# mryab/learning-at-home

Measured on NVIDIA H100. Metric: DMoE training samples/sec (whole job, device-timed, max over ranks), higher is better.
Workload: dtype bf16

## Files before the change

learning-at-home_b200/csrc/adam.cu:

```cuda
#include "sm90.cuh"

namespace lah {

struct AdamArgs {
    float* p; float* g; float* m; float* v; float* vmax; bf16* p_bf16;
    int num_segs; long long seg_start[13]; long long seg_n[12]; long long total;
    const int* step;
    const int* group_rows;
    int step_scalar;
    float lr, beta1, beta2, eps, weight_decay;
    int amsgrad, zero_mask;
    int world; long long peer_grad_off; char* peer_base[8]; float grad_scale;
    int G_active; const int* shadow_of; long long shadow_g_off; int me;
    int num_ranges; long long r_start[6]; long long r_cum[7];
    int dead_mask;
    const int* poison;
    float decay;
    const float* lr_dev;
};

template <bool DECOUPLED, bool DEV_LR>
__global__ void __launch_bounds__(256) adam_kernel(AdamArgs a) {
    if (a.poison && (*a.poison & 1)) return;
    float dev_lr = 0.f, dev_decay = 1.f;
    if constexpr (DEV_LR) {
        dev_lr = a.lr_dev[0];
        if constexpr (DECOUPLED) dev_decay = a.lr_dev[1];
    }
    const long long stride = static_cast<long long>(gridDim.x) * blockDim.x * 4;
    const long long span = a.num_ranges ? a.r_cum[a.num_ranges] : a.total;
    for (long long j = (static_cast<long long>(blockIdx.x) * blockDim.x + threadIdx.x) * 4; j < span; j += stride) {
        long long i = j;
        if (a.num_ranges) {
            int r = 0;
#pragma unroll
            for (int t = 1; t < 6; ++t)
                if (t < a.num_ranges && j >= a.r_cum[t]) r = t;
            i = a.r_start[r] + (j - a.r_cum[r]);
        }
        int sg = 0;
#pragma unroll
        for (int t = 1; t < 12; ++t)
            if (t < a.num_segs && i >= a.seg_start[t]) sg = t;
        const int g = static_cast<int>((i - a.seg_start[sg]) / a.seg_n[sg]);
        if (g >= a.G_active) continue;
        if (a.group_rows && a.group_rows[g] <= 0) continue;
        const int step = a.step ? a.step[g] : a.step_scalar;
        const float bc1 = 1.f - powf(a.beta1, static_cast<float>(step));
        const float bc2 = 1.f - powf(a.beta2, static_cast<float>(step));
        const float step_size = (DEV_LR ? dev_lr : a.lr) / bc1;
        const float inv_sqrt_bc2 = rsqrtf(bc2);
        float4 gr;
        if (a.peer_grad_off >= 0) {
            gr = make_float4(0.f, 0.f, 0.f, 0.f);
            for (int r = 0; r < a.world; ++r) {
                if ((a.dead_mask >> r) & 1) continue;
                const float4 t = *reinterpret_cast<const float4*>(
                    reinterpret_cast<const float*>(a.peer_base[r] + a.peer_grad_off) + i);
                gr.x += t.x; gr.y += t.y; gr.z += t.z; gr.w += t.w;
            }
            gr.x *= a.grad_scale; gr.y *= a.grad_scale; gr.z *= a.grad_scale; gr.w *= a.grad_scale;
        } else if (a.shadow_of && a.shadow_of[2 * g] >= 0) {
            const int slot = a.shadow_of[2 * g], mask = a.shadow_of[2 * g + 1];
            gr = ((mask >> a.me) & 1) ? *reinterpret_cast<const float4*>(a.g + i) : make_float4(0.f, 0.f, 0.f, 0.f);
            const long long pi = i + (a.G_active + slot - g) * a.seg_n[sg];
            for (int r = 0; r < a.world; ++r) {
                if (r == a.me || !((mask >> r) & 1)) continue;
                const float4 t = *reinterpret_cast<const float4*>(
                    reinterpret_cast<const float*>(a.peer_base[r] + a.shadow_g_off) + pi);
                gr.x += t.x; gr.y += t.y; gr.z += t.z; gr.w += t.w;
            }
        } else {
            gr = *reinterpret_cast<const float4*>(a.g + i);
        }
        float4 p = *reinterpret_cast<const float4*>(a.p + i);
        float4 m = *reinterpret_cast<const float4*>(a.m + i);
        float4 v = *reinterpret_cast<const float4*>(a.v + i);
        float4 vm = a.amsgrad ? *reinterpret_cast<const float4*>(a.vmax + i) : make_float4(0.f, 0.f, 0.f, 0.f);
        float* pp = &p.x; float* mp = &m.x; float* vp = &v.x; float* vmp = &vm.x; float* gp = &gr.x;
#pragma unroll
        for (int t = 0; t < 4; ++t) {
            float grad = gp[t];
            if constexpr (DECOUPLED) pp[t] = __fmul_rn(pp[t], DEV_LR ? dev_decay : a.decay);
            else if (a.weight_decay != 0.f) grad += a.weight_decay * pp[t];
            mp[t] = mp[t] + (1.f - a.beta1) * (grad - mp[t]);
            vp[t] = vp[t] * a.beta2 + (1.f - a.beta2) * grad * grad;
            float denom;
            if (a.amsgrad) {
                vmp[t] = fmaxf(vmp[t], vp[t]);
                denom = sqrtf(vmp[t]) * inv_sqrt_bc2 + a.eps;
            } else {
                denom = sqrtf(vp[t]) * inv_sqrt_bc2 + a.eps;
            }
            pp[t] -= step_size * (mp[t] / denom);
        }
        *reinterpret_cast<float4*>(a.p + i) = p;
        *reinterpret_cast<float4*>(a.m + i) = m;
        *reinterpret_cast<float4*>(a.v + i) = v;
        if (a.amsgrad) *reinterpret_cast<float4*>(a.vmax + i) = vm;
        if (a.p_bf16) {
            uint2 q;
            q.x = pack_bf16x2(p.x, p.y);
            q.y = pack_bf16x2(p.z, p.w);
            *reinterpret_cast<uint2*>(a.p_bf16 + i) = q;
        }
        if (((a.zero_mask >> sg) & 1) && a.peer_grad_off < 0)
            *reinterpret_cast<float4*>(a.g + i) = make_float4(0.f, 0.f, 0.f, 0.f);
    }
}

__global__ void bump_steps_kernel(int* step, const int* group_rows, int G) {
    const int g = blockIdx.x * blockDim.x + threadIdx.x;
    if (g < G && group_rows[g] > 0) step[g] += 1;
}

__global__ void cast_bf16_kernel(const float* __restrict__ src, bf16* __restrict__ dst, long long n) {
    const long long stride = static_cast<long long>(gridDim.x) * blockDim.x * 4;
    for (long long i = (static_cast<long long>(blockIdx.x) * blockDim.x + threadIdx.x) * 4; i < n; i += stride) {
        const float4 p = *reinterpret_cast<const float4*>(src + i);
        uint2 q;
        q.x = pack_bf16x2(p.x, p.y);
        q.y = pack_bf16x2(p.z, p.w);
        *reinterpret_cast<uint2*>(dst + i) = q;
    }
}

}

using namespace lah;

extern "C" const int* lah_get_poison_word();

extern "C" {

int lah_adam_step(float* p, float* g, float* m, float* v, float* vmax, void* p_bf16, int num_segs, const long long* seg_n,
                  int G, const int* step, const int* group_rows, int step_scalar, float lr, const float* lr_dev, float beta1,
                  float beta2, float eps, float weight_decay, int amsgrad, int zero_mask, int world, long long peer_grad_off,
                  const unsigned long long* peer_bases, float grad_scale, int G_active, const int* shadow_of,
                  long long shadow_g_off, int me, int seg_mask, int dead_mask, float decay, int decoupled, cudaStream_t st) {
    if (num_segs < 1 || num_segs > 12) return -2;
    if (decoupled && weight_decay != 0.f) return -2;
    AdamArgs a;
    a.num_segs = num_segs;
    long long off = 0;
    for (int s = 0; s < 12; ++s) {
        a.seg_start[s] = off;
        a.seg_n[s] = s < num_segs ? seg_n[s] : 1;
        if (s < num_segs) {
            if (seg_n[s] % 4) return -2;
            off += seg_n[s] * G;
        }
    }
    a.seg_start[12] = off;
    a.p = p; a.g = g; a.m = m; a.v = v; a.vmax = vmax; a.p_bf16 = (bf16*)p_bf16;
    a.total = off; a.step = step; a.group_rows = group_rows; a.step_scalar = step_scalar; a.lr = lr;
    a.beta1 = beta1; a.beta2 = beta2; a.eps = eps; a.weight_decay = weight_decay; a.amsgrad = amsgrad;
    a.zero_mask = zero_mask; a.world = world; a.peer_grad_off = peer_grad_off; a.grad_scale = grad_scale;
    a.G_active = G_active > 0 ? G_active : G; a.shadow_of = shadow_of; a.shadow_g_off = shadow_g_off; a.me = me;
    for (int i = 0; i < 8; ++i) a.peer_base[i] = (peer_bases && i < world) ? (char*)peer_bases[i] : nullptr;
    a.poison = lah_get_poison_word();
    a.dead_mask = dead_mask;
    a.decay = decay;
    a.lr_dev = lr_dev;
    a.num_ranges = 0;
    a.r_cum[0] = 0;
    if (seg_mask) {
        for (int s = 0; s < num_segs; ++s) {
            if (!((seg_mask >> s) & 1)) continue;
            const long long len = seg_n[s] * G;
            if (a.num_ranges && a.r_start[a.num_ranges - 1] + (a.r_cum[a.num_ranges] - a.r_cum[a.num_ranges - 1]) == a.seg_start[s]) {
                a.r_cum[a.num_ranges] += len;
            } else {
                if (a.num_ranges == 6) return -2;
                a.r_start[a.num_ranges] = a.seg_start[s];
                a.r_cum[a.num_ranges + 1] = a.r_cum[a.num_ranges] + len;
                ++a.num_ranges;
            }
        }
        if (!a.num_ranges) return 0;
    }
    const long long span = a.num_ranges ? a.r_cum[a.num_ranges] : a.total;
    if (span <= 0) return 0;
    long long blocks = (span / 4 + 255) / 256;
    if (blocks > 132 * 16) blocks = 132 * 16;
    if (lr_dev) {
        if (decoupled)
            adam_kernel<true, true><<<(int)blocks, 256, 0, st>>>(a);
        else
            adam_kernel<false, true><<<(int)blocks, 256, 0, st>>>(a);
    } else if (decoupled) {
        adam_kernel<true, false><<<(int)blocks, 256, 0, st>>>(a);
    } else {
        adam_kernel<false, false><<<(int)blocks, 256, 0, st>>>(a);
    }
    return -(int)cudaGetLastError();
}

int lah_bump_steps(int* step, const int* group_rows, int G, cudaStream_t st) {
    bump_steps_kernel<<<(G + 255) / 256, 256, 0, st>>>(step, group_rows, G);
    return -(int)cudaGetLastError();
}

int lah_cast_bf16(const float* src, void* dst, long long n, cudaStream_t st) {
    if (n % 4) return -2;
    if (n <= 0) return 0;
    long long blocks = (n / 4 + 255) / 256;
    if (blocks > 132 * 16) blocks = 132 * 16;
    cast_bf16_kernel<<<(int)blocks, 256, 0, st>>>(src, (bf16*)dst, n);
    return -(int)cudaGetLastError();
}

}
```

learning-at-home_b200/csrc/sm90.cuh:

```cuda
#pragma once

#include <cuda.h>
#include <cuda_runtime.h>
#include <cuda_bf16.h>
#include <stdint.h>

namespace lah {

typedef __nv_bfloat16 bf16;

__device__ __forceinline__ uint32_t smem_u32(const void* p) {
    return static_cast<uint32_t>(__cvta_generic_to_shared(p));
}

__device__ __forceinline__ uint32_t elect_one_sync() {
    uint32_t pred = 0;
    asm volatile(
        "{\n"
        ".reg .pred P1;\n"
        "elect.sync _|P1, 0xffffffff;\n"
        "selp.b32 %0, 1, 0, P1;\n"
        "}\n"
        : "=r"(pred));
    return pred;
}

__device__ __forceinline__ void mbar_init(uint64_t* bar, uint32_t count) {
    asm volatile("mbarrier.init.shared::cta.b64 [%0], %1;" ::"r"(smem_u32(bar)), "r"(count) : "memory");
}
__device__ __forceinline__ void fence_mbar_init() {
    asm volatile("fence.mbarrier_init.release.cluster;" ::: "memory");
}
__device__ __forceinline__ void fence_proxy_async_smem() {
    asm volatile("fence.proxy.async.shared::cta;" ::: "memory");
}
__device__ __forceinline__ void mbar_arrive_expect_tx(uint64_t* bar, uint32_t bytes) {
    asm volatile("mbarrier.arrive.expect_tx.shared::cta.b64 _, [%0], %1;" ::"r"(smem_u32(bar)), "r"(bytes)
                 : "memory");
}
__device__ __forceinline__ void mbar_arrive(uint64_t* bar) {
    asm volatile("mbarrier.arrive.shared::cta.b64 _, [%0];" ::"r"(smem_u32(bar)) : "memory");
}
__device__ __forceinline__ uint32_t mbar_try_wait(uint64_t* bar, uint32_t parity) {
    uint32_t ok;
    asm volatile(
        "{\n"
        ".reg .pred p;\n"
        "mbarrier.try_wait.parity.shared::cta.b64 p, [%1], %2;\n"
        "selp.b32 %0, 1, 0, p;\n"
        "}\n"
        : "=r"(ok)
        : "r"(smem_u32(bar)), "r"(parity)
        : "memory");
    return ok;
}
__device__ __forceinline__ void mbar_wait(uint64_t* bar, uint32_t parity) {
    while (!mbar_try_wait(bar, parity)) {
    }
}

__device__ __forceinline__ void tma_prefetch_desc(const CUtensorMap* tm) {
    asm volatile("prefetch.tensormap [%0];" ::"l"(reinterpret_cast<uint64_t>(tm)) : "memory");
}
__device__ __forceinline__ void tma_load_2d(void* smem_dst, const CUtensorMap* tm, uint64_t* bar, int c0, int c1) {
    asm volatile(
        "cp.async.bulk.tensor.2d.shared::cluster.global.mbarrier::complete_tx::bytes [%0], [%1, {%3, %4}], [%2];"
        ::"r"(smem_u32(smem_dst)), "l"(reinterpret_cast<uint64_t>(tm)), "r"(smem_u32(bar)), "r"(c0), "r"(c1)
        : "memory");
}
__device__ __forceinline__ void tma_load_3d(void* smem_dst, const CUtensorMap* tm, uint64_t* bar, int c0, int c1,
                                            int c2) {
    asm volatile(
        "cp.async.bulk.tensor.3d.shared::cluster.global.mbarrier::complete_tx::bytes [%0], [%1, {%3, %4, %5}], [%2];"
        ::"r"(smem_u32(smem_dst)), "l"(reinterpret_cast<uint64_t>(tm)), "r"(smem_u32(bar)), "r"(c0), "r"(c1), "r"(c2)
        : "memory");
}
__device__ __forceinline__ void tma_store_2d(const CUtensorMap* tm, const void* smem_src, int c0, int c1) {
    asm volatile("cp.async.bulk.tensor.2d.global.shared::cta.bulk_group [%0, {%2, %3}], [%1];" ::"l"(
                     reinterpret_cast<uint64_t>(tm)),
                 "r"(smem_u32(smem_src)), "r"(c0), "r"(c1)
                 : "memory");
}
__device__ __forceinline__ void tma_store_3d(const CUtensorMap* tm, const void* smem_src, int c0, int c1, int c2) {
    asm volatile("cp.async.bulk.tensor.3d.global.shared::cta.bulk_group [%0, {%2, %3, %4}], [%1];" ::"l"(
                     reinterpret_cast<uint64_t>(tm)),
                 "r"(smem_u32(smem_src)), "r"(c0), "r"(c1), "r"(c2)
                 : "memory");
}
__device__ __forceinline__ void tma_store_commit() { asm volatile("cp.async.bulk.commit_group;" ::: "memory"); }
template <int N>
__device__ __forceinline__ void tma_store_wait_read() {
    asm volatile("cp.async.bulk.wait_group.read %0;" ::"n"(N) : "memory");
}
template <int N>
__device__ __forceinline__ void tma_store_wait() {
    asm volatile("cp.async.bulk.wait_group %0;" ::"n"(N) : "memory");
}

__device__ __forceinline__ void wgmma_fence() { asm volatile("wgmma.fence.sync.aligned;" ::: "memory"); }
__device__ __forceinline__ void wgmma_commit() { asm volatile("wgmma.commit_group.sync.aligned;" ::: "memory"); }
template <int N>
__device__ __forceinline__ void wgmma_wait() {
    asm volatile("wgmma.wait_group.sync.aligned %0;" ::"n"(N) : "memory");
}
template <int R>
__device__ __forceinline__ void wgmma_fence_regs(float (&d)[R]) {
#pragma unroll
    for (int i = 0; i < R; ++i) asm volatile("" : "+f"(d[i])::"memory");
}

template <int TA, int TB>
__device__ __forceinline__ void wgmma_bf16_n16(float (&d)[8], uint64_t da, uint64_t db, uint32_t accumulate) {
    asm volatile(
        "{\n.reg .pred p;\nsetp.ne.b32 p, %10, 0;\n"
        "wgmma.mma_async.sync.aligned.m64n16k16.f32.bf16.bf16 {%0, %1, %2, %3, %4, %5, %6, %7}, %8, %9, p, 1, 1, %11, %12;\n}\n"
        : "+f"(d[0]), "+f"(d[1]), "+f"(d[2]), "+f"(d[3]), "+f"(d[4]), "+f"(d[5]), "+f"(d[6]), "+f"(d[7])
        : "l"(da), "l"(db), "r"(accumulate), "n"(TA), "n"(TB));
}

template <int TA, int TB>
__device__ __forceinline__ void wgmma_bf16_n32(float (&d)[16], uint64_t da, uint64_t db, uint32_t accumulate) {
    asm volatile(
        "{\n.reg .pred p;\nsetp.ne.b32 p, %18, 0;\n"
        "wgmma.mma_async.sync.aligned.m64n32k16.f32.bf16.bf16 {%0, %1, %2, %3, %4, %5, %6, %7, %8, %9, %10, %11, %12, %13, %14, %15}, %16, %17, p, 1, 1, %19, %20;\n}\n"
        : "+f"(d[0]), "+f"(d[1]), "+f"(d[2]), "+f"(d[3]), "+f"(d[4]), "+f"(d[5]), "+f"(d[6]), "+f"(d[7]), "+f"(d[8]), "+f"(d[9]), "+f"(d[10]), "+f"(d[11]), "+f"(d[12]), "+f"(d[13]), "+f"(d[14]), "+f"(d[15])
        : "l"(da), "l"(db), "r"(accumulate), "n"(TA), "n"(TB));
}

template <int TA, int TB>
__device__ __forceinline__ void wgmma_bf16_n64(float (&d)[32], uint64_t da, uint64_t db, uint32_t accumulate) {
    asm volatile(
        "{\n.reg .pred p;\nsetp.ne.b32 p, %34, 0;\n"
        "wgmma.mma_async.sync.aligned.m64n64k16.f32.bf16.bf16 {%0, %1, %2, %3, %4, %5, %6, %7, %8, %9, %10, %11, %12, %13, %14, %15, %16, %17, %18, %19, %20, %21, %22, %23, %24, %25, %26, %27, %28, %29, %30, %31}, %32, %33, p, 1, 1, %35, %36;\n}\n"
        : "+f"(d[0]), "+f"(d[1]), "+f"(d[2]), "+f"(d[3]), "+f"(d[4]), "+f"(d[5]), "+f"(d[6]), "+f"(d[7]), "+f"(d[8]), "+f"(d[9]), "+f"(d[10]), "+f"(d[11]), "+f"(d[12]), "+f"(d[13]), "+f"(d[14]), "+f"(d[15]), "+f"(d[16]), "+f"(d[17]), "+f"(d[18]), "+f"(d[19]), "+f"(d[20]), "+f"(d[21]), "+f"(d[22]), "+f"(d[23]), "+f"(d[24]), "+f"(d[25]), "+f"(d[26]), "+f"(d[27]), "+f"(d[28]), "+f"(d[29]), "+f"(d[30]), "+f"(d[31])
        : "l"(da), "l"(db), "r"(accumulate), "n"(TA), "n"(TB));
}

template <int TA, int TB>
__device__ __forceinline__ void wgmma_bf16_n128(float (&d)[64], uint64_t da, uint64_t db, uint32_t accumulate) {
    asm volatile(
        "{\n.reg .pred p;\nsetp.ne.b32 p, %66, 0;\n"
        "wgmma.mma_async.sync.aligned.m64n128k16.f32.bf16.bf16 {%0, %1, %2, %3, %4, %5, %6, %7, %8, %9, %10, %11, %12, %13, %14, %15, %16, %17, %18, %19, %20, %21, %22, %23, %24, %25, %26, %27, %28, %29, %30, %31, %32, %33, %34, %35, %36, %37, %38, %39, %40, %41, %42, %43, %44, %45, %46, %47, %48, %49, %50, %51, %52, %53, %54, %55, %56, %57, %58, %59, %60, %61, %62, %63}, %64, %65, p, 1, 1, %67, %68;\n}\n"
        : "+f"(d[0]), "+f"(d[1]), "+f"(d[2]), "+f"(d[3]), "+f"(d[4]), "+f"(d[5]), "+f"(d[6]), "+f"(d[7]), "+f"(d[8]), "+f"(d[9]), "+f"(d[10]), "+f"(d[11]), "+f"(d[12]), "+f"(d[13]), "+f"(d[14]), "+f"(d[15]), "+f"(d[16]), "+f"(d[17]), "+f"(d[18]), "+f"(d[19]), "+f"(d[20]), "+f"(d[21]), "+f"(d[22]), "+f"(d[23]), "+f"(d[24]), "+f"(d[25]), "+f"(d[26]), "+f"(d[27]), "+f"(d[28]), "+f"(d[29]), "+f"(d[30]), "+f"(d[31]), "+f"(d[32]), "+f"(d[33]), "+f"(d[34]), "+f"(d[35]), "+f"(d[36]), "+f"(d[37]), "+f"(d[38]), "+f"(d[39]), "+f"(d[40]), "+f"(d[41]), "+f"(d[42]), "+f"(d[43]), "+f"(d[44]), "+f"(d[45]), "+f"(d[46]), "+f"(d[47]), "+f"(d[48]), "+f"(d[49]), "+f"(d[50]), "+f"(d[51]), "+f"(d[52]), "+f"(d[53]), "+f"(d[54]), "+f"(d[55]), "+f"(d[56]), "+f"(d[57]), "+f"(d[58]), "+f"(d[59]), "+f"(d[60]), "+f"(d[61]), "+f"(d[62]), "+f"(d[63])
        : "l"(da), "l"(db), "r"(accumulate), "n"(TA), "n"(TB));
}

template <int TA, int TB>
__device__ __forceinline__ void wgmma_bf16_n256(float (&d)[128], uint64_t da, uint64_t db, uint32_t accumulate) {
    asm volatile(
        "{\n.reg .pred p;\nsetp.ne.b32 p, %130, 0;\n"
        "wgmma.mma_async.sync.aligned.m64n256k16.f32.bf16.bf16 {%0, %1, %2, %3, %4, %5, %6, %7, %8, %9, %10, %11, %12, %13, %14, %15, %16, %17, %18, %19, %20, %21, %22, %23, %24, %25, %26, %27, %28, %29, %30, %31, %32, %33, %34, %35, %36, %37, %38, %39, %40, %41, %42, %43, %44, %45, %46, %47, %48, %49, %50, %51, %52, %53, %54, %55, %56, %57, %58, %59, %60, %61, %62, %63, %64, %65, %66, %67, %68, %69, %70, %71, %72, %73, %74, %75, %76, %77, %78, %79, %80, %81, %82, %83, %84, %85, %86, %87, %88, %89, %90, %91, %92, %93, %94, %95, %96, %97, %98, %99, %100, %101, %102, %103, %104, %105, %106, %107, %108, %109, %110, %111, %112, %113, %114, %115, %116, %117, %118, %119, %120, %121, %122, %123, %124, %125, %126, %127}, %128, %129, p, 1, 1, %131, %132;\n}\n"
        : "+f"(d[0]), "+f"(d[1]), "+f"(d[2]), "+f"(d[3]), "+f"(d[4]), "+f"(d[5]), "+f"(d[6]), "+f"(d[7]), "+f"(d[8]), "+f"(d[9]), "+f"(d[10]), "+f"(d[11]), "+f"(d[12]), "+f"(d[13]), "+f"(d[14]), "+f"(d[15]), "+f"(d[16]), "+f"(d[17]), "+f"(d[18]), "+f"(d[19]), "+f"(d[20]), "+f"(d[21]), "+f"(d[22]), "+f"(d[23]), "+f"(d[24]), "+f"(d[25]), "+f"(d[26]), "+f"(d[27]), "+f"(d[28]), "+f"(d[29]), "+f"(d[30]), "+f"(d[31]), "+f"(d[32]), "+f"(d[33]), "+f"(d[34]), "+f"(d[35]), "+f"(d[36]), "+f"(d[37]), "+f"(d[38]), "+f"(d[39]), "+f"(d[40]), "+f"(d[41]), "+f"(d[42]), "+f"(d[43]), "+f"(d[44]), "+f"(d[45]), "+f"(d[46]), "+f"(d[47]), "+f"(d[48]), "+f"(d[49]), "+f"(d[50]), "+f"(d[51]), "+f"(d[52]), "+f"(d[53]), "+f"(d[54]), "+f"(d[55]), "+f"(d[56]), "+f"(d[57]), "+f"(d[58]), "+f"(d[59]), "+f"(d[60]), "+f"(d[61]), "+f"(d[62]), "+f"(d[63]), "+f"(d[64]), "+f"(d[65]), "+f"(d[66]), "+f"(d[67]), "+f"(d[68]), "+f"(d[69]), "+f"(d[70]), "+f"(d[71]), "+f"(d[72]), "+f"(d[73]), "+f"(d[74]), "+f"(d[75]), "+f"(d[76]), "+f"(d[77]), "+f"(d[78]), "+f"(d[79]), "+f"(d[80]), "+f"(d[81]), "+f"(d[82]), "+f"(d[83]), "+f"(d[84]), "+f"(d[85]), "+f"(d[86]), "+f"(d[87]), "+f"(d[88]), "+f"(d[89]), "+f"(d[90]), "+f"(d[91]), "+f"(d[92]), "+f"(d[93]), "+f"(d[94]), "+f"(d[95]), "+f"(d[96]), "+f"(d[97]), "+f"(d[98]), "+f"(d[99]), "+f"(d[100]), "+f"(d[101]), "+f"(d[102]), "+f"(d[103]), "+f"(d[104]), "+f"(d[105]), "+f"(d[106]), "+f"(d[107]), "+f"(d[108]), "+f"(d[109]), "+f"(d[110]), "+f"(d[111]), "+f"(d[112]), "+f"(d[113]), "+f"(d[114]), "+f"(d[115]), "+f"(d[116]), "+f"(d[117]), "+f"(d[118]), "+f"(d[119]), "+f"(d[120]), "+f"(d[121]), "+f"(d[122]), "+f"(d[123]), "+f"(d[124]), "+f"(d[125]), "+f"(d[126]), "+f"(d[127])
        : "l"(da), "l"(db), "r"(accumulate), "n"(TA), "n"(TB));
}

template <int TB>
__device__ __forceinline__ void wgmma_bf16_rs_n32(float (&d)[16], const uint32_t (&a)[4], uint64_t db, uint32_t accumulate) {
    asm volatile(
        "{\n.reg .pred p;\nsetp.ne.b32 p, %21, 0;\n"
        "wgmma.mma_async.sync.aligned.m64n32k16.f32.bf16.bf16 {%0, %1, %2, %3, %4, %5, %6, %7, %8, %9, %10, %11, %12, %13, %14, %15}, {%16, %17, %18, %19}, %20, p, 1, 1, %22;\n}\n"
        : "+f"(d[0]), "+f"(d[1]), "+f"(d[2]), "+f"(d[3]), "+f"(d[4]), "+f"(d[5]), "+f"(d[6]), "+f"(d[7]), "+f"(d[8]), "+f"(d[9]), "+f"(d[10]), "+f"(d[11]), "+f"(d[12]), "+f"(d[13]), "+f"(d[14]), "+f"(d[15])
        : "r"(a[0]), "r"(a[1]), "r"(a[2]), "r"(a[3]), "l"(db), "r"(accumulate), "n"(TB));
}

template <int TB>
__device__ __forceinline__ void wgmma_bf16_rs_n64(float (&d)[32], const uint32_t (&a)[4], uint64_t db, uint32_t accumulate) {
    asm volatile(
        "{\n.reg .pred p;\nsetp.ne.b32 p, %37, 0;\n"
        "wgmma.mma_async.sync.aligned.m64n64k16.f32.bf16.bf16 {%0, %1, %2, %3, %4, %5, %6, %7, %8, %9, %10, %11, %12, %13, %14, %15, %16, %17, %18, %19, %20, %21, %22, %23, %24, %25, %26, %27, %28, %29, %30, %31}, {%32, %33, %34, %35}, %36, p, 1, 1, %38;\n}\n"
        : "+f"(d[0]), "+f"(d[1]), "+f"(d[2]), "+f"(d[3]), "+f"(d[4]), "+f"(d[5]), "+f"(d[6]), "+f"(d[7]), "+f"(d[8]), "+f"(d[9]), "+f"(d[10]), "+f"(d[11]), "+f"(d[12]), "+f"(d[13]), "+f"(d[14]), "+f"(d[15]), "+f"(d[16]), "+f"(d[17]), "+f"(d[18]), "+f"(d[19]), "+f"(d[20]), "+f"(d[21]), "+f"(d[22]), "+f"(d[23]), "+f"(d[24]), "+f"(d[25]), "+f"(d[26]), "+f"(d[27]), "+f"(d[28]), "+f"(d[29]), "+f"(d[30]), "+f"(d[31])
        : "r"(a[0]), "r"(a[1]), "r"(a[2]), "r"(a[3]), "l"(db), "r"(accumulate), "n"(TB));
}

template <int TB>
__device__ __forceinline__ void wgmma_bf16_rs_n128(float (&d)[64], const uint32_t (&a)[4], uint64_t db, uint32_t accumulate) {
    asm volatile(
        "{\n.reg .pred p;\nsetp.ne.b32 p, %69, 0;\n"
        "wgmma.mma_async.sync.aligned.m64n128k16.f32.bf16.bf16 {%0, %1, %2, %3, %4, %5, %6, %7, %8, %9, %10, %11, %12, %13, %14, %15, %16, %17, %18, %19, %20, %21, %22, %23, %24, %25, %26, %27, %28, %29, %30, %31, %32, %33, %34, %35, %36, %37, %38, %39, %40, %41, %42, %43, %44, %45, %46, %47, %48, %49, %50, %51, %52, %53, %54, %55, %56, %57, %58, %59, %60, %61, %62, %63}, {%64, %65, %66, %67}, %68, p, 1, 1, %70;\n}\n"
        : "+f"(d[0]), "+f"(d[1]), "+f"(d[2]), "+f"(d[3]), "+f"(d[4]), "+f"(d[5]), "+f"(d[6]), "+f"(d[7]), "+f"(d[8]), "+f"(d[9]), "+f"(d[10]), "+f"(d[11]), "+f"(d[12]), "+f"(d[13]), "+f"(d[14]), "+f"(d[15]), "+f"(d[16]), "+f"(d[17]), "+f"(d[18]), "+f"(d[19]), "+f"(d[20]), "+f"(d[21]), "+f"(d[22]), "+f"(d[23]), "+f"(d[24]), "+f"(d[25]), "+f"(d[26]), "+f"(d[27]), "+f"(d[28]), "+f"(d[29]), "+f"(d[30]), "+f"(d[31]), "+f"(d[32]), "+f"(d[33]), "+f"(d[34]), "+f"(d[35]), "+f"(d[36]), "+f"(d[37]), "+f"(d[38]), "+f"(d[39]), "+f"(d[40]), "+f"(d[41]), "+f"(d[42]), "+f"(d[43]), "+f"(d[44]), "+f"(d[45]), "+f"(d[46]), "+f"(d[47]), "+f"(d[48]), "+f"(d[49]), "+f"(d[50]), "+f"(d[51]), "+f"(d[52]), "+f"(d[53]), "+f"(d[54]), "+f"(d[55]), "+f"(d[56]), "+f"(d[57]), "+f"(d[58]), "+f"(d[59]), "+f"(d[60]), "+f"(d[61]), "+f"(d[62]), "+f"(d[63])
        : "r"(a[0]), "r"(a[1]), "r"(a[2]), "r"(a[3]), "l"(db), "r"(accumulate), "n"(TB));
}

template <int N, int TA, int TB>
__device__ __forceinline__ void wgmma_bf16_ss(float (&d)[N / 2], uint64_t da, uint64_t db, uint32_t accumulate) {
    static_assert(N == 32 || N == 64 || N == 128, "N");
    if constexpr (N == 32) wgmma_bf16_n32<TA, TB>(d, da, db, accumulate);
    else if constexpr (N == 64) wgmma_bf16_n64<TA, TB>(d, da, db, accumulate);
    else wgmma_bf16_n128<TA, TB>(d, da, db, accumulate);
}
template <int N, int TB>
__device__ __forceinline__ void wgmma_bf16_rs(float (&d)[N / 2], const uint32_t (&a)[4], uint64_t db, uint32_t accumulate) {
    static_assert(N == 32 || N == 64 || N == 128, "N");
    if constexpr (N == 32) wgmma_bf16_rs_n32<TB>(d, a, db, accumulate);
    else if constexpr (N == 64) wgmma_bf16_rs_n64<TB>(d, a, db, accumulate);
    else wgmma_bf16_rs_n128<TB>(d, a, db, accumulate);
}

__device__ __forceinline__ uint64_t make_smem_desc_sw128(uint32_t saddr, uint32_t lbo_bytes, uint32_t sbo_bytes) {
    uint64_t d = 0;
    d |= static_cast<uint64_t>((saddr & 0x3FFFFu) >> 4);
    d |= static_cast<uint64_t>((lbo_bytes >> 4) & 0x3FFFu) << 16;
    d |= static_cast<uint64_t>((sbo_bytes >> 4) & 0x3FFFu) << 32;
    d |= static_cast<uint64_t>(1) << 62;
    return d;
}

__device__ __forceinline__ uint64_t make_smem_desc_sw64(uint32_t saddr, uint32_t lbo_bytes, uint32_t sbo_bytes) {
    uint64_t d = 0;
    d |= static_cast<uint64_t>((saddr & 0x3FFFFu) >> 4);
    d |= static_cast<uint64_t>((lbo_bytes >> 4) & 0x3FFFu) << 16;
    d |= static_cast<uint64_t>((sbo_bytes >> 4) & 0x3FFFu) << 32;
    d |= static_cast<uint64_t>(2) << 62;
    return d;
}

template <int COLS>
__device__ __forceinline__ uint64_t make_smem_desc_cols(uint32_t saddr, uint32_t lbo_bytes) {
    static_assert(COLS == 32 || COLS == 64, "atoms are 32 or 64 bf16 columns wide");
    if constexpr (COLS == 32) return make_smem_desc_sw64(saddr, lbo_bytes, 512);
    else return make_smem_desc_sw128(saddr, lbo_bytes, 1024);
}

__device__ __forceinline__ void named_bar_sync(int id, int threads) {
    asm volatile("bar.sync %0, %1;" ::"r"(id), "r"(threads) : "memory");
}

__device__ __forceinline__ void st_release_sys(int* p, int v) {
    asm volatile("st.release.sys.global.s32 [%0], %1;" ::"l"(p), "r"(v) : "memory");
}
__device__ __forceinline__ int ld_acquire_sys(const int* p) {
    int v;
    asm volatile("ld.acquire.sys.global.s32 %0, [%1];" : "=r"(v) : "l"(p) : "memory");
    return v;
}
__device__ __forceinline__ void red_add_release_sys(int* p, int v) {
    asm volatile("red.release.sys.global.add.s32 [%0], %1;" ::"l"(p), "r"(v) : "memory");
}
__device__ __forceinline__ int ld_acquire_gpu(const int* p) {
    int v;
    asm volatile("ld.acquire.gpu.global.s32 %0, [%1];" : "=r"(v) : "l"(p) : "memory");
    return v;
}
__device__ __forceinline__ int4 ld_nc_v4(const int4* p) {
    int4 r;
    asm volatile("ld.global.nc.L1::no_allocate.v4.s32 {%0, %1, %2, %3}, [%4];"
                 : "=r"(r.x), "=r"(r.y), "=r"(r.z), "=r"(r.w)
                 : "l"(p));
    return r;
}
__device__ __forceinline__ int4 ld_v4(const int4* p) {
    int4 r;
    asm volatile("ld.global.v4.s32 {%0, %1, %2, %3}, [%4];" : "=r"(r.x), "=r"(r.y), "=r"(r.z), "=r"(r.w) : "l"(p));
    return r;
}
__device__ __forceinline__ void st_v4(int4* p, const int4& v) {
    asm volatile("st.global.v4.s32 [%0], {%1, %2, %3, %4};" ::"l"(p), "r"(v.x), "r"(v.y), "r"(v.z), "r"(v.w)
                 : "memory");
}

__device__ __forceinline__ bool spin_flag_ge(const int* flag, int epoch) {
    const long long t0 = clock64();
    while (ld_acquire_sys(flag) < epoch) {
        if (clock64() - t0 > 20000000000ll) return false;
    }
    return true;
}
__device__ __forceinline__ bool spin_flag_ft(const int* flag, int epoch, int* status, int rank, int timeout_ms) {
    if (status) {
        const volatile int* vs = status;
        if ((vs[1] >> rank) & 1) return false;
        if (vs[0] & 1) return false;
    }
    const long long t0 = clock64();
    const long long limit = timeout_ms > 0 ? static_cast<long long>(timeout_ms) * 2000000ll : 20000000000ll;
    while (ld_acquire_sys(flag) < epoch) {
        if (clock64() - t0 > limit) {
            if (status) atomicOr(status, 1);
            return false;
        }
    }
    return true;
}
__device__ __forceinline__ unsigned long long globaltimer_ns() {
    unsigned long long t;
    asm volatile("mov.u64 %0, %%globaltimer;" : "=l"(t));
    return t;
}
__device__ __forceinline__ void fence_proxy_async_global() { asm volatile("fence.proxy.async.global;" ::: "memory"); }

__device__ __forceinline__ uint32_t pack_bf16x2(float lo, float hi) {
    __nv_bfloat162 v = __floats2bfloat162_rn(lo, hi);
    return *reinterpret_cast<uint32_t*>(&v);
}
__device__ __forceinline__ float2 unpack_bf16x2(uint32_t u) {
    __nv_bfloat162 v = *reinterpret_cast<__nv_bfloat162*>(&u);
    return __bfloat1622float2(v);
}
__device__ __forceinline__ float warp_sum(float v) {
#pragma unroll
    for (int o = 16; o > 0; o >>= 1) v += __shfl_xor_sync(0xffffffffu, v, o);
    return v;
}
__device__ __forceinline__ float warp_max(float v) {
#pragma unroll
    for (int o = 16; o > 0; o >>= 1) v = fmaxf(v, __shfl_xor_sync(0xffffffffu, v, o));
    return v;
}

inline int make_tmap(CUtensorMap* tm, CUtensorMapDataType dtype, int rank, const void* ptr, const uint64_t* dims,
                     const uint64_t* strides_bytes, const uint32_t* box,
                     CUtensorMapSwizzle swizzle = CU_TENSOR_MAP_SWIZZLE_128B) {
    typedef CUresult (*EncodeTiled)(CUtensorMap*, CUtensorMapDataType, cuuint32_t, void*, const cuuint64_t*,
                                    const cuuint64_t*, const cuuint32_t*, const cuuint32_t*, CUtensorMapInterleave,
                                    CUtensorMapSwizzle, CUtensorMapL2promotion, CUtensorMapFloatOOBfill);
    static const EncodeTiled encode = [] {
        void* fn = nullptr;
        cudaDriverEntryPointQueryResult qres;
        if (cudaGetDriverEntryPoint("cuTensorMapEncodeTiled", &fn, cudaEnableDefault, &qres) != cudaSuccess) fn = nullptr;
        return reinterpret_cast<EncodeTiled>(fn);
    }();
    if (!encode) return -100;
    cuuint64_t gdims[3], gstr[2];
    cuuint32_t gbox[3], estr[3] = {1, 1, 1};
    for (int i = 0; i < rank; ++i) {
        gdims[i] = dims[i];
        gbox[i] = box[i];
    }
    for (int i = 0; i < rank - 1; ++i) gstr[i] = strides_bytes[i];
    const CUresult r = encode(tm, dtype, rank, const_cast<void*>(ptr), gdims, gstr, gbox, estr, CU_TENSOR_MAP_INTERLEAVE_NONE,
                              swizzle, CU_TENSOR_MAP_L2_PROMOTION_L2_256B, CU_TENSOR_MAP_FLOAT_OOB_FILL_NONE);
    return r == CUDA_SUCCESS ? 0 : -1000 - static_cast<int>(r);
}

inline int num_sms() {
    static const int sms = [] {
        int dev = 0, n = 0;
        cudaGetDevice(&dev);
        cudaDeviceGetAttribute(&n, cudaDevAttrMultiProcessorCount, dev);
        return n;
    }();
    return sms;
}

inline int persistent_grid(long long total_tiles, int max_ctas) {
    int grid = num_sms();
    if (max_ctas > 0 && max_ctas < grid) grid = max_ctas;
    if (total_tiles < grid) grid = static_cast<int>(total_tiles);
    return grid;
}

template <auto Kernel>
inline int set_max_dynamic_smem(int bytes) {
    static bool done = false;
    if (!done) {
        const cudaError_t e = cudaFuncSetAttribute(Kernel, cudaFuncAttributeMaxDynamicSharedMemorySize, bytes);
        if (e != cudaSuccess) return -static_cast<int>(e);
        done = true;
    }
    return 0;
}

}
```

learning-at-home_b200/csrc/small_m.cu:

```cuda
#include "sm90.cuh"
#include <climits>

namespace lah {
namespace smallm {

constexpr int BM = 128;
constexpr int BK = 64;
constexpr int MMA_K = 16;
constexpr int BN_MAX = 128;
constexpr int NUM_THREADS = 288;

namespace sab {

constexpr int STAGES = 6;
constexpr int A_BYTES = BM * BK * 2;
constexpr int B_BYTES = BN_MAX * BK * 2;
constexpr int STAGE_BYTES = A_BYTES + B_BYTES;
constexpr int BAR_OFFSET = STAGES * STAGE_BYTES;
constexpr int QD = 4;
constexpr int MAX_G = 1023;
constexpr int CUM_OFFSET = BAR_OFFSET + (2 * STAGES + 2 * QD) * 8 + QD * 4 + 16;
constexpr int SMEM_TOTAL = CUM_OFFSET + (MAX_G + 1) * 4 + 1024;
static_assert(SMEM_TOTAL <= 232448, "shared memory budget");

struct Params {
    int G, M_out, K;
    const int* group_off;
    const int* group_rows;
    bf16* out;
    long long ldo;
    const float* bias;
    const bf16* residual;
    long long ldr;
    const int* wait_flags;
    int wait_count, wait_epoch;
    const int* epoch_base;
    int* status;
    int* tile_counter;
};

__device__ __forceinline__ int box_rows_of(int nn) { return nn <= 16 ? 16 : (nn <= 32 ? 32 : (nn <= 64 ? 64 : 128)); }

__device__ __forceinline__ int find_group(const int* cum, int G, int gc) {
    int lo = 0, hi = G - 1;
    while (lo < hi) {
        const int mid = (lo + hi + 1) >> 1;
        if (cum[mid] <= gc) lo = mid; else hi = mid - 1;
    }
    return lo;
}

template <int NB, bool A_MN>
__device__ __forceinline__ void sab_tile(const Params& p, uint8_t* smem, uint64_t* full_bar, uint64_t* empty_bar, int& stage,
                                         uint32_t& phase, int num_kb, int wg, int warp, int lane, int g, int ms, int row0,
                                         int nn) {
    float acc[NB / 2];
    constexpr uint32_t A_KSTEP = A_MN ? MMA_K * 128 : MMA_K * 2;
    int prev_stage = -1;
    for (int kb = 0; kb < num_kb; ++kb) {
        mbar_wait(&full_bar[stage], phase);
        const uint32_t sa = smem_u32(smem + stage * STAGE_BYTES) + wg * (A_MN ? BK * 128 : 64 * 128);
        const uint32_t sb = smem_u32(smem + stage * STAGE_BYTES + A_BYTES);
        wgmma_fence();
#pragma unroll
        for (int k = 0; k < BK / MMA_K; ++k) {
            const uint64_t da = make_smem_desc_sw128(sa + k * A_KSTEP, BK * 128, 1024);
            const uint64_t db = make_smem_desc_sw128(sb + k * (MMA_K * 2), 0, 1024);
            const uint32_t accum = (kb > 0 || k > 0) ? 1u : 0u;
            if constexpr (NB == 16) wgmma_bf16_n16<A_MN, 0>(acc, da, db, accum);
            if constexpr (NB == 32) wgmma_bf16_n32<A_MN, 0>(acc, da, db, accum);
            if constexpr (NB == 64) wgmma_bf16_n64<A_MN, 0>(acc, da, db, accum);
            if constexpr (NB == 128) wgmma_bf16_n128<A_MN, 0>(acc, da, db, accum);
        }
        wgmma_commit();
        wgmma_wait<1>();
        if (prev_stage >= 0) {
            __syncwarp();
            if (lane == 0) mbar_arrive(&empty_bar[prev_stage]);
        }
        prev_stage = stage;
        if (++stage == STAGES) {
            stage = 0;
            phase ^= 1;
        }
    }
    wgmma_wait<0>();
    wgmma_fence_regs(acc);
    __syncwarp();
    if (lane == 0 && prev_stage >= 0) mbar_arrive(&empty_bar[prev_stage]);

    const int n16 = (nn + 15) & ~15;
#pragma unroll
    for (int h = 0; h < 2; ++h) {
        const int feat = ms * BM + wg * 64 + (warp & 3) * 16 + (lane >> 2) + 8 * h;
        const float bias = p.bias ? __ldg(p.bias + static_cast<long long>(g) * p.M_out + feat) : 0.f;
#pragma unroll
        for (int j = 0; j < NB / 8; ++j) {
#pragma unroll
            for (int e = 0; e < 2; ++e) {
                const int n = 8 * j + 2 * (lane & 3) + e;
                if (n < n16) {
                    const long long row = row0 + n;
                    float v = acc[4 * j + 2 * h + e] + bias;
                    if (p.residual) v += __bfloat162float(p.residual[row * p.ldr + feat]);
                    p.out[row * p.ldo + feat] = __float2bfloat16(v);
                }
            }
        }
    }
}

template <bool A_MN>
__global__ void __launch_bounds__(NUM_THREADS, 1)
swapab_kernel(const Params p, const __grid_constant__ CUtensorMap tmA, const __grid_constant__ CUtensorMap tmB16,
              const __grid_constant__ CUtensorMap tmB32, const __grid_constant__ CUtensorMap tmB64,
              const __grid_constant__ CUtensorMap tmB128) {
    extern __shared__ uint8_t smem_raw[];
    uint8_t* smem = reinterpret_cast<uint8_t*>((reinterpret_cast<uintptr_t>(smem_raw) + 1023) & ~uintptr_t(1023));
    uint64_t* full_bar = reinterpret_cast<uint64_t*>(smem + BAR_OFFSET);
    uint64_t* empty_bar = full_bar + STAGES;
    uint64_t* q_full = empty_bar + STAGES;
    uint64_t* q_empty = q_full + QD;
    volatile int* q_tile = reinterpret_cast<volatile int*>(q_empty + QD);
    int* cum = reinterpret_cast<int*>(smem + CUM_OFFSET);

    const int warp = threadIdx.x >> 5;
    const int lane = threadIdx.x & 31;

    if (warp == 0) {
        int carry = 0;
        for (int base = 0; base < p.G; base += 32) {
            const int g = base + lane;
            int x = g < p.G ? (__ldg(p.group_rows + g) + BN_MAX - 1) / BN_MAX : 0;
#pragma unroll
            for (int d = 1; d < 32; d <<= 1) {
                const int y = __shfl_up_sync(0xffffffffu, x, d);
                if (lane >= d) x += y;
            }
            if (g < p.G) cum[g + 1] = carry + x;
            carry += __shfl_sync(0xffffffffu, x, 31);
        }
        if (lane == 0) cum[0] = 0;
    }
    if (warp == 8 && lane == 0) {
        tma_prefetch_desc(&tmA);
        tma_prefetch_desc(&tmB16);
        tma_prefetch_desc(&tmB32);
        tma_prefetch_desc(&tmB64);
        tma_prefetch_desc(&tmB128);
        for (int i = 0; i < STAGES; ++i) {
            mbar_init(&full_bar[i], 1);
            mbar_init(&empty_bar[i], 8);
        }
        for (int i = 0; i < QD; ++i) {
            mbar_init(&q_full[i], 1);
            mbar_init(&q_empty[i], 8);
        }
        fence_mbar_init();
    }
    __syncthreads();

    const int m_slices = p.M_out / BM;
    const int total = cum[p.G] * m_slices;
    const int num_kb = p.K / BK;

    if (warp == 8) {
        if (lane != 0) return;
        if (p.wait_flags) {
            const int epoch = p.wait_epoch + (p.epoch_base ? *p.epoch_base : 0);
            const unsigned long long t_wait = globaltimer_ns();
            for (int sidx = 0; sidx < p.wait_count; ++sidx)
                spin_flag_ft(p.wait_flags + sidx, epoch, p.status, sidx, p.epoch_base ? p.epoch_base[1] : 0);
            if (blockIdx.x == 0) atomicAdd(reinterpret_cast<unsigned long long*>(p.status + 2), globaltimer_ns() - t_wait);
            fence_proxy_async_global();
        }
        int stage = 0, qi = 0;
        uint32_t phase = 0, qphase = 0;
        while (true) {
            const int tile = atomicAdd(p.tile_counter, 1);
            mbar_wait(&q_empty[qi], qphase ^ 1);
            q_tile[qi] = tile;
            mbar_arrive(&q_full[qi]);
            if (++qi == QD) {
                qi = 0;
                qphase ^= 1;
            }
            if (tile >= total) break;
            const int gc = tile / m_slices, ms = tile - gc * m_slices;
            const int g = find_group(cum, p.G, gc);
            const int n0 = (gc - cum[g]) * BN_MAX;
            const int rows = __ldg(p.group_rows + g);
            const int off = __ldg(p.group_off + g);
            const int box = box_rows_of(min(rows - n0, BN_MAX));
            const CUtensorMap* tmB = box == 16 ? &tmB16 : (box == 32 ? &tmB32 : (box == 64 ? &tmB64 : &tmB128));
            for (int kb = 0; kb < num_kb; ++kb) {
                mbar_wait(&empty_bar[stage], phase ^ 1);
                uint8_t* sa = smem + stage * STAGE_BYTES;
                uint8_t* sb = sa + A_BYTES;
                const int k = kb * BK;
                mbar_arrive_expect_tx(&full_bar[stage], A_BYTES + box * 128);
                if (!A_MN) {
                    tma_load_3d(sa, &tmA, &full_bar[stage], k, ms * BM, g);
                } else {
#pragma unroll
                    for (int i = 0; i < BM / 64; ++i)
                        tma_load_3d(sa + i * (BK * 128), &tmA, &full_bar[stage], ms * BM + i * 64, k, g);
                }
                tma_load_2d(sb, tmB, &full_bar[stage], k, off + n0);
                if (++stage == STAGES) {
                    stage = 0;
                    phase ^= 1;
                }
            }
        }
        return;
    }

    const int wg = warp >> 2;
    int stage = 0, qi = 0;
    uint32_t phase = 0, qphase = 0;
    while (true) {
        mbar_wait(&q_full[qi], qphase);
        const int tile = q_tile[qi];
        __syncwarp();
        if (lane == 0) mbar_arrive(&q_empty[qi]);
        if (++qi == QD) {
            qi = 0;
            qphase ^= 1;
        }
        if (tile >= total) break;
        const int gc = tile / m_slices, ms = tile - gc * m_slices;
        const int g = find_group(cum, p.G, gc);
        const int n0 = (gc - cum[g]) * BN_MAX;
        const int nn = min(__ldg(p.group_rows + g) - n0, BN_MAX);
        const int row0 = __ldg(p.group_off + g) + n0;
        switch (box_rows_of(nn)) {
            case 16: sab_tile<16, A_MN>(p, smem, full_bar, empty_bar, stage, phase, num_kb, wg, warp, lane, g, ms, row0, nn); break;
            case 32: sab_tile<32, A_MN>(p, smem, full_bar, empty_bar, stage, phase, num_kb, wg, warp, lane, g, ms, row0, nn); break;
            case 64: sab_tile<64, A_MN>(p, smem, full_bar, empty_bar, stage, phase, num_kb, wg, warp, lane, g, ms, row0, nn); break;
            default: sab_tile<128, A_MN>(p, smem, full_bar, empty_bar, stage, phase, num_kb, wg, warp, lane, g, ms, row0, nn); break;
        }
    }
}

}

namespace wa {

constexpr int WBK = 32;
constexpr int OP_STAGES = 2;
constexpr int OP_STAGE_BYTES = 2 * (WBK * BM * 2);
constexpr int OP_BYTES = OP_STAGES * OP_STAGE_BYTES;
constexpr int BAND_ROWS = 4;
constexpr int CHUNKS = 16 / BAND_ROWS;
constexpr int SUB_COLS = 32;
constexpr int SUB_BYTES = BM / CHUNKS * SUB_COLS * 4;
constexpr int ARR_BYTES = (BN_MAX / SUB_COLS) * SUB_BYTES;
constexpr int ST_STAGES = 3;
constexpr int ST_STAGE_BYTES = 4 * ARR_BYTES;
constexpr int ST_OFFSET = OP_BYTES;
constexpr int BAR_OFFSET = ST_OFFSET + ST_STAGES * ST_STAGE_BYTES;
constexpr int QD = 4;
constexpr int SMEM_TOTAL = BAR_OFFSET + (2 * OP_STAGES + 2 * ST_STAGES + 2 * QD) * 8 + QD * 4 + 16 + 1024;
static_assert(ST_STAGES <= CHUNKS, "the producer issues a tile's first ST_STAGES chunks before its remaining k-blocks");
static_assert(OP_STAGE_BYTES % 1024 == 0 && SUB_BYTES % 1024 == 0, "128-B swizzle atoms need 1 KB alignment");
static_assert(SMEM_TOTAL <= 232448, "shared memory budget");

struct Params {
    int G, N, K;
    const int* group_off;
    const int* group_rows;
    const int* skip;
    const int* step;
    float* p;
    float* m;
    float* v;
    float* vmax;
    bf16* p_bf16;
    float lr, beta1, beta2, eps;
    int amsgrad;
    float wd;
    int* tile_counter;
    const int* poison;
};
static_assert(sizeof(Params) == 128 && sizeof(Params) % alignof(CUtensorMap) == 0, "Params layout");

constexpr int WD_NONE = 0, WD_L2 = 1, WD_DECOUPLED = 2;

struct Tile {
    int g, mt, nt;
};

struct StateMaps {
    CUtensorMap a[4];
};

__device__ __forceinline__ void state_chunk_tma(const StateMaps& tm, int n_arr, uint8_t* ss, uint64_t* bar, int col0, int srow,
                                                int c) {
    for (int a = 0; a < n_arr; ++a)
#pragma unroll
        for (int q = 0; q < BN_MAX / SUB_COLS; ++q) {
            uint8_t* s = ss + a * ARR_BYTES + q * SUB_BYTES;
            if (bar) tma_load_3d(s, &tm.a[a], bar, col0 + q * SUB_COLS, BAND_ROWS * c, srow / 16);
            else tma_store_3d(&tm.a[a], s, col0 + q * SUB_COLS, BAND_ROWS * c, srow / 16);
        }
}

template <int WD, bool DEV_LR>
__global__ void __launch_bounds__(NUM_THREADS, 1)
wgrad_adam_kernel(const Params p, const __grid_constant__ CUtensorMap tmDY, const __grid_constant__ CUtensorMap tmX,
                  const __grid_constant__ StateMaps tmS, const float* __restrict__ lr_dev) {
    extern __shared__ uint8_t smem_raw[];
    uint8_t* smem = reinterpret_cast<uint8_t*>((reinterpret_cast<uintptr_t>(smem_raw) + 1023) & ~uintptr_t(1023));
    uint8_t* st_smem = smem + ST_OFFSET;
    uint64_t* op_full = reinterpret_cast<uint64_t*>(smem + BAR_OFFSET);
    uint64_t* op_empty = op_full + OP_STAGES;
    uint64_t* st_full = op_empty + OP_STAGES;
    uint64_t* st_empty = st_full + ST_STAGES;
    uint64_t* q_full = st_empty + ST_STAGES;
    uint64_t* q_empty = q_full + QD;
    volatile int* q_tile = reinterpret_cast<volatile int*>(q_empty + QD);

    const int warp = threadIdx.x >> 5;
    const int lane = threadIdx.x & 31;
    if (p.poison && (*p.poison & 1)) return;
    const int n_arr = p.amsgrad ? 4 : 3;

    if (warp == 8 && lane == 0) {
        tma_prefetch_desc(&tmDY);
        tma_prefetch_desc(&tmX);
        for (int a = 0; a < n_arr; ++a) tma_prefetch_desc(&tmS.a[a]);
        for (int i = 0; i < OP_STAGES; ++i) {
            mbar_init(&op_full[i], 1);
            mbar_init(&op_empty[i], 8);
        }
        for (int i = 0; i < ST_STAGES; ++i) {
            mbar_init(&st_full[i], 1);
            mbar_init(&st_empty[i], 1);
        }
        for (int i = 0; i < QD; ++i) {
            mbar_init(&q_full[i], 1);
            mbar_init(&q_empty[i], 8);
        }
        fence_mbar_init();
    }
    __syncthreads();

    const int n_tiles = p.K / BN_MAX;
    const int tiles_per_group = (p.N / BM) * n_tiles;
    const int total = p.G * tiles_per_group;
    auto decode = [&](int tile) {
        Tile t;
        t.g = tile / tiles_per_group;
        const int r = tile - t.g * tiles_per_group;
        t.mt = r / n_tiles;
        t.nt = r - t.mt * n_tiles;
        return t;
    };

    if (warp == 8) {
        if (lane != 0) return;
        uint32_t phase = 0, qphase = 0, sphase = 0;
        int qi = 0, stage = 0, sstage = 0;
        while (true) {
            int tile;
            while (true) {
                tile = atomicAdd(p.tile_counter, 1);
                if (tile >= total) break;
                const int g = tile / tiles_per_group;
                if (__ldg(p.group_rows + g) > 0 && !(p.skip && __ldg(p.skip + 2 * g) >= 0)) break;
                atomicMax(p.tile_counter, (g + 1) * tiles_per_group);
            }
            mbar_wait(&q_empty[qi], qphase ^ 1);
            q_tile[qi] = tile;
            mbar_arrive(&q_full[qi]);
            if (++qi == QD) {
                qi = 0;
                qphase ^= 1;
            }
            if (tile >= total) break;
            const Tile t = decode(tile);
            const int off = __ldg(p.group_off + t.g), rows = __ldg(p.group_rows + t.g);
            const int srow = t.g * p.N + t.mt * BM;
            auto load_chunk = [&](int c) {
                mbar_wait(&st_empty[sstage], sphase ^ 1);
                mbar_arrive_expect_tx(&st_full[sstage], n_arr * ARR_BYTES);
                state_chunk_tma(tmS, n_arr, st_smem + sstage * ST_STAGE_BYTES, &st_full[sstage], t.nt * BN_MAX, srow, c);
                if (++sstage == ST_STAGES) {
                    sstage = 0;
                    sphase ^= 1;
                }
            };
            for (int t0 = 0; t0 < rows; t0 += WBK) {
                mbar_wait(&op_empty[stage], phase ^ 1);
                mbar_arrive_expect_tx(&op_full[stage], OP_STAGE_BYTES);
                uint8_t* sa = smem + stage * OP_STAGE_BYTES;
                uint8_t* sb = sa + WBK * BM * 2;
#pragma unroll
                for (int i = 0; i < BM / 64; ++i)
                    tma_load_2d(sa + i * (WBK * 128), &tmDY, &op_full[stage], t.mt * BM + i * 64, off + t0);
#pragma unroll
                for (int i = 0; i < BN_MAX / 64; ++i)
                    tma_load_2d(sb + i * (WBK * 128), &tmX, &op_full[stage], t.nt * BN_MAX + i * 64, off + t0);
                if (++stage == OP_STAGES) {
                    stage = 0;
                    phase ^= 1;
                }
                if (t0 == 0)
                    for (int c = 0; c < ST_STAGES; ++c) load_chunk(c);
            }
            for (int c = ST_STAGES; c < CHUNKS; ++c) load_chunk(c);
        }
        return;
    }

    float lr = p.lr, wd = p.wd;
    if constexpr (DEV_LR) {
        lr = lr_dev[0];
        if constexpr (WD == WD_DECOUPLED) wd = lr_dev[1];
    }
    const int wg = warp >> 2;
    int qi = 0, stage = 0, sstage = 0;
    uint32_t phase = 0, qphase = 0, sphase = 0;
    float acc[BN_MAX / 2];
    float xg[BN_MAX / 8];
    const int lrow = wg * 64 + (warp & 3) * 16 + (lane >> 2);
    const int brow = (lane >> 2) & 3;
    const int R = warp * BAND_ROWS + brow;
    const int jflip = 2 * (brow & 1);
    while (true) {
        mbar_wait(&q_full[qi], qphase);
        const int tile = q_tile[qi];
        __syncwarp();
        if (lane == 0) mbar_arrive(&q_empty[qi]);
        if (++qi == QD) {
            qi = 0;
            qphase ^= 1;
        }
        if (tile >= total) break;
        const Tile t = decode(tile);
        const int rows = __ldg(p.group_rows + t.g);
        int prev_stage = -1;
        for (int t0 = 0; t0 < rows; t0 += WBK) {
            mbar_wait(&op_full[stage], phase);
            const uint32_t sa = smem_u32(smem + stage * OP_STAGE_BYTES) + wg * (WBK * 128);
            const uint32_t sb = smem_u32(smem + stage * OP_STAGE_BYTES + WBK * BM * 2);
            const int ksteps = min(WBK / MMA_K, (rows - t0 + MMA_K - 1) / MMA_K);
            wgmma_fence();
            for (int k = 0; k < ksteps; ++k) {
                const uint64_t da = make_smem_desc_sw128(sa + k * (MMA_K * 128), WBK * 128, 1024);
                const uint64_t db = make_smem_desc_sw128(sb + k * (MMA_K * 128), WBK * 128, 1024);
                wgmma_bf16_n128<1, 1>(acc, da, db, (t0 > 0 || k > 0) ? 1u : 0u);
            }
            wgmma_commit();
            wgmma_wait<1>();
            if (prev_stage >= 0) {
                __syncwarp();
                if (lane == 0) mbar_arrive(&op_empty[prev_stage]);
            }
            prev_stage = stage;
            if (++stage == OP_STAGES) {
                stage = 0;
                phase ^= 1;
            }
        }
        wgmma_wait<0>();
        wgmma_fence_regs(acc);
        __syncwarp();
        if (lane == 0 && prev_stage >= 0) mbar_arrive(&op_empty[prev_stage]);

        const float st = static_cast<float>(__ldg(p.step + t.g));
        const float step_size = lr / (1.f - powf(p.beta1, st));
        const float inv_sqrt_bc2 = rsqrtf(1.f - powf(p.beta2, st));
        const int srow = t.g * p.N + t.mt * BM;
        const int col_base = t.nt * BN_MAX + 2 * (lane & 3);
#pragma unroll
        for (int c = 0; c < CHUNKS; ++c) {
            mbar_wait(&st_full[sstage], sphase);
            uint8_t* ss = st_smem + sstage * ST_STAGE_BYTES;
            if ((c & 1) == 0) {
#pragma unroll
                for (int i = 0; i < BN_MAX / 8; ++i) xg[i] = __shfl_xor_sync(0xffffffffu, acc[4 * (BN_MAX / 16 + i / 2) + i % 2], 16);
            }
            const bool own = (lane >> 4) == (c & 1);
            const long long o_row = (static_cast<long long>(srow) + (own ? lrow : lrow ^ 4) + 8 * (c >> 1)) * p.K + col_base;
            const int jbase = own ? 0 : BN_MAX / 16;
#pragma unroll
            for (int k = 0; k < BN_MAX / 16; ++k) {
                const int j = jbase + (k ^ jflip);
                const int so = (j >> 2) * SUB_BYTES + R * 128 + (((2 * (j & 3) + ((lane & 3) >> 1)) ^ (R & 7)) << 4) +
                               8 * (lane & 1);
                float2* sp = reinterpret_cast<float2*>(ss + so);
                float2* sm = reinterpret_cast<float2*>(ss + ARR_BYTES + so);
                float2* sv = reinterpret_cast<float2*>(ss + 2 * ARR_BYTES + so);
                float2* svm = reinterpret_cast<float2*>(ss + 3 * ARR_BYTES + so);
                float2 pw = *sp, m = *sm, v = *sv;
                float2 vm = p.amsgrad ? *svm : make_float2(0.f, 0.f);
                float* pp = &pw.x; float* mp = &m.x; float* vp = &v.x; float* vmp = &vm.x;
#pragma unroll
                for (int e = 0; e < 2; ++e) {
                    float grad = own ? (jflip ? acc[4 * (k ^ 2) + e] : acc[4 * k + e])
                                     : (jflip ? xg[2 * (k ^ 2) + e] : xg[2 * k + e]);
                    if constexpr (WD == WD_L2) grad += wd * pp[e];
                    if constexpr (WD == WD_DECOUPLED) pp[e] = __fmul_rn(pp[e], wd);
                    mp[e] = mp[e] + (1.f - p.beta1) * (grad - mp[e]);
                    vp[e] = vp[e] * p.beta2 + (1.f - p.beta2) * grad * grad;
                    float denom;
                    if (p.amsgrad) {
                        vmp[e] = fmaxf(vmp[e], vp[e]);
                        denom = sqrtf(vmp[e]) * inv_sqrt_bc2 + p.eps;
                    } else {
                        denom = sqrtf(vp[e]) * inv_sqrt_bc2 + p.eps;
                    }
                    pp[e] -= step_size * (mp[e] / denom);
                }
                *sp = pw;
                *sm = m;
                *sv = v;
                if (p.amsgrad) *svm = vm;
                *reinterpret_cast<uint32_t*>(p.p_bf16 + o_row + 8 * j) = pack_bf16x2(pw.x, pw.y);
            }
            fence_proxy_async_smem();
            named_bar_sync(1, 256);
            if (threadIdx.x == 0) {
                state_chunk_tma(tmS, n_arr, ss, nullptr, t.nt * BN_MAX, srow, c);
                tma_store_commit();
                tma_store_wait_read<0>();
                mbar_arrive(&st_empty[sstage]);
            }
            if (++sstage == ST_STAGES) {
                sstage = 0;
                sphase ^= 1;
            }
            if (c == 1) {
#pragma unroll
                for (int j = 0; j < BN_MAX / 8; ++j) {
                    acc[4 * j] = acc[4 * j + 2];
                    acc[4 * j + 1] = acc[4 * j + 3];
                }
            }
        }
    }
    if (threadIdx.x == 0) tma_store_wait<0>();
}

}
}
}

using namespace lah;
using namespace lah::smallm;

extern "C" const int* lah_get_epoch_base();

static int* tile_counter() {
    static int* ctr = nullptr;
    if (!ctr) {
        if (cudaMalloc(&ctr, 256) != cudaSuccess) return nullptr;
        cudaMemset(ctr, 0, 256);
    }
    return ctr;
}
static const int* g_poison = nullptr;

extern "C" {

int lah_set_poison_word(const int* status) {
    g_poison = status;
    return 0;
}
const int* lah_get_poison_word() { return g_poison; }

int lah_swapab_linear(const void* x, long long ldx, int x_rows, const void* W, int G, int M_out, int K, int a_mn,
                      void* out, long long ldo, const int* group_off, const int* group_rows, const float* bias,
                      const void* residual, long long ldr, const int* wait_flags, int wait_count, int wait_epoch,
                      int* status, int max_ctas, cudaStream_t st) {
    if ((K % BK) || (M_out % BM) || (ldx % 8) || G > sab::MAX_G) return -2;
    CUtensorMap tmA, tmB[4];
    if (!a_mn) {
        uint64_t dims[3] = {(uint64_t)K, (uint64_t)M_out, (uint64_t)G};
        uint64_t str[2] = {(uint64_t)K * 2, (uint64_t)M_out * K * 2};
        uint32_t box[3] = {BK, BM, 1};
        int r = make_tmap(&tmA, CU_TENSOR_MAP_DATA_TYPE_BFLOAT16, 3, W, dims, str, box);
        if (r) return r;
    } else {
        uint64_t dims[3] = {(uint64_t)M_out, (uint64_t)K, (uint64_t)G};
        uint64_t str[2] = {(uint64_t)M_out * 2, (uint64_t)M_out * K * 2};
        uint32_t box[3] = {64, BK, 1};
        int r = make_tmap(&tmA, CU_TENSOR_MAP_DATA_TYPE_BFLOAT16, 3, W, dims, str, box);
        if (r) return r;
    }
    const uint32_t boxes[4] = {16, 32, 64, 128};
    for (int i = 0; i < 4; ++i) {
        uint64_t dims[2] = {(uint64_t)K, (uint64_t)x_rows};
        uint64_t str[1] = {(uint64_t)ldx * 2};
        uint32_t box[2] = {BK, boxes[i]};
        int r = make_tmap(&tmB[i], CU_TENSOR_MAP_DATA_TYPE_BFLOAT16, 2, x, dims, str, box);
        if (r) return r;
    }
    sab::Params p;
    p.G = G; p.M_out = M_out; p.K = K; p.group_off = group_off; p.group_rows = group_rows; p.out = (bf16*)out; p.ldo = ldo;
    p.bias = bias; p.residual = (const bf16*)residual; p.ldr = ldr; p.wait_flags = wait_flags; p.wait_count = wait_count;
    p.wait_epoch = wait_epoch; p.epoch_base = lah_get_epoch_base(); p.status = status;
    p.tile_counter = tile_counter();
    if (!p.tile_counter) return -3;
    const long long total = 1ll * (M_out / BM) * (G + x_rows / BN_MAX);
    if (total <= 0 || G <= 0) return 0;
    if (cudaMemsetAsync(p.tile_counter, 0, sizeof(int), st) != cudaSuccess) return -4;
    const int ctas = persistent_grid(total, max_ctas);
    if (!a_mn) {
        if (int e = set_max_dynamic_smem<sab::swapab_kernel<false>>(sab::SMEM_TOTAL)) return e;
        sab::swapab_kernel<false><<<ctas, NUM_THREADS, sab::SMEM_TOTAL, st>>>(p, tmA, tmB[0], tmB[1], tmB[2], tmB[3]);
    } else {
        if (int e = set_max_dynamic_smem<sab::swapab_kernel<true>>(sab::SMEM_TOTAL)) return e;
        sab::swapab_kernel<true><<<ctas, NUM_THREADS, sab::SMEM_TOTAL, st>>>(p, tmA, tmB[0], tmB[1], tmB[2], tmB[3]);
    }
    return -(int)cudaGetLastError();
}

}

template <int WD, bool DEV_LR>
static int launch_wgrad_adam(const wa::Params& a, const CUtensorMap& tmDY, const CUtensorMap& tmX, const wa::StateMaps& tmS,
                             const float* lr_dev, int ctas, cudaStream_t st) {
    if (int e = set_max_dynamic_smem<wa::wgrad_adam_kernel<WD, DEV_LR>>(wa::SMEM_TOTAL)) return e;
    wa::wgrad_adam_kernel<WD, DEV_LR><<<ctas, NUM_THREADS, wa::SMEM_TOTAL, st>>>(a, tmDY, tmX, tmS, lr_dev);
    return -(int)cudaGetLastError();
}

extern "C" {

int lah_wgrad_adam(const void* dy, long long lddy, const void* x, long long ldx, int total_rows, int G, int N, int K,
                   const int* group_off, const int* group_rows, const int* skip, const int* step, float* p, float* m,
                   float* v, float* vmax, void* p_bf16, float lr, const float* lr_dev, float beta1, float beta2, float eps,
                   int amsgrad, float weight_decay, float decay, int decoupled, int max_ctas, cudaStream_t st) {
    if ((N % BM) || (K % BN_MAX) || (lddy % 8) || (ldx % 8) || 1ll * G * N > INT_MAX) return -2;
    if (decoupled && weight_decay != 0.f) return -2;
    if (amsgrad && !vmax) return -2;
    CUtensorMap tmDY, tmX;
    wa::StateMaps tmS;
    {
        float* arrs[4] = {p, m, v, amsgrad ? vmax : p};
        uint64_t dims[3] = {(uint64_t)K, 16, (uint64_t)G * N / 16};
        uint64_t str[2] = {(uint64_t)K * 4, (uint64_t)K * 64};
        uint32_t box[3] = {wa::SUB_COLS, wa::BAND_ROWS, BM / 16};
        for (int a = 0; a < 4; ++a) {
            int r = make_tmap(&tmS.a[a], CU_TENSOR_MAP_DATA_TYPE_FLOAT32, 3, arrs[a], dims, str, box);
            if (r) return r;
        }
    }
    {
        uint64_t dims[2] = {(uint64_t)N, (uint64_t)total_rows};
        uint64_t str[1] = {(uint64_t)lddy * 2};
        uint32_t box[2] = {64, wa::WBK};
        int r = make_tmap(&tmDY, CU_TENSOR_MAP_DATA_TYPE_BFLOAT16, 2, dy, dims, str, box);
        if (r) return r;
    }
    {
        uint64_t dims[2] = {(uint64_t)K, (uint64_t)total_rows};
        uint64_t str[1] = {(uint64_t)ldx * 2};
        uint32_t box[2] = {64, wa::WBK};
        int r = make_tmap(&tmX, CU_TENSOR_MAP_DATA_TYPE_BFLOAT16, 2, x, dims, str, box);
        if (r) return r;
    }
    wa::Params a;
    a.G = G; a.N = N; a.K = K; a.group_off = group_off; a.group_rows = group_rows; a.skip = skip; a.step = step;
    a.p = p; a.m = m; a.v = v; a.vmax = vmax; a.p_bf16 = (bf16*)p_bf16; a.lr = lr; a.beta1 = beta1; a.beta2 = beta2; a.eps = eps; a.amsgrad = amsgrad;
    a.wd = decoupled ? decay : weight_decay;
    a.tile_counter = tile_counter() ? tile_counter() + 16 : nullptr;
    a.poison = g_poison;
    if (!a.tile_counter) return -3;
    const long long total = 1ll * G * (N / BM) * (K / BN_MAX);
    if (total <= 0) return 0;
    if (cudaMemsetAsync(a.tile_counter, 0, sizeof(int), st) != cudaSuccess) return -4;
    const int ctas = persistent_grid(total, max_ctas);
    if (lr_dev) {
        if (decoupled) return launch_wgrad_adam<wa::WD_DECOUPLED, true>(a, tmDY, tmX, tmS, lr_dev, ctas, st);
        if (weight_decay != 0.f) return launch_wgrad_adam<wa::WD_L2, true>(a, tmDY, tmX, tmS, lr_dev, ctas, st);
        return launch_wgrad_adam<wa::WD_NONE, true>(a, tmDY, tmX, tmS, lr_dev, ctas, st);
    }
    if (decoupled) return launch_wgrad_adam<wa::WD_DECOUPLED, false>(a, tmDY, tmX, tmS, nullptr, ctas, st);
    if (weight_decay != 0.f) return launch_wgrad_adam<wa::WD_L2, false>(a, tmDY, tmX, tmS, nullptr, ctas, st);
    return launch_wgrad_adam<wa::WD_NONE, false>(a, tmDY, tmX, tmS, nullptr, ctas, st);
}

}
```

learning-at-home_b200/ops/kernels.py:

```python
import ctypes
import math

import torch
import torch.nn.functional as F

from . import native
from .native import c_void_p, c_int, c_ll, c_float, ptr, stream_ptr

c_ull = ctypes.c_ulonglong
_configured = False

SLOT_COUNTS, SLOT_DISPATCH, SLOT_OUTPUT, SLOT_GRAD, SLOT_DINPUT, SLOT_TRAINER, SLOT_BARRIER, SLOT_SHADOW = range(8)
NUM_SLOTS = 8
MAX_WORLD = 8
STATUS_TIMEOUT, STATUS_OVERFLOW = 1, 2


def _lib():
    global _configured
    lib = native.cuda_lib()
    if _configured:
        return lib
    P, I, L, Fl = c_void_p, c_int, c_ll, c_float
    sigs = {
        "lah_ln_relu_fwd": [P, P, P, P, P, P, P, I, I, I, I, P],
        "lah_ln_relu_bwd": [P, P, P, P, P, P, P, P, P, P, P, P, I, I, I, I, P, P],
        "lah_grouped_colsum": [P, L, P, P, I, P, I, I, P],
        "lah_set_step_counters": [P],
        "lah_set_multicast": [c_ull],
        "lah_set_poison_word": [P],
        "lah_nvls_allreduce": [L, L, Fl, P],
        "lah_heartbeat": [L, I, I, L, P],
        "lah_alive_from_heartbeats": [P, P, I, L, L, P],
        "lah_set_spin_timeout_ms": [I],
        "lah_step_begin": [I, L, P],
        "lah_swapab_linear": [P, L, I, P, I, I, I, I, P, L, P, P, P, P, L, P, I, I, P, I, P],
        "lah_wgrad_adam": [P, L, P, L, I, I, I, I, P, P, P, P, P, P, P, P, P, Fl, P, Fl, Fl, Fl, I, Fl, Fl, I, I, P],
        "lah_ln_relu_fwd_q": [P, P, P, P, P, P, P, I, I, I, P, P, P],
        "lah_set_peers": [P, I, I],
        "lah_set_wait_counter": [P],
        "lah_gate_topk": [P, I, P, I, I, P, Fl, c_ull, L, P, P, P, P, P],
        "lah_layout_exchange": [L, L, I, I, I, I, I, I, I, P, P, P, P, P, P, P, I, Fl, I, P, P, P, P, P],
        "lah_scatter_rows": [P, P, P, P, P, P, L, L, I, I, I, I, I, I, I, I, P, P, P, P, P, I, P],
        "lah_pull_shadow": [P, I, I, L, L, I, P, I, P],
        "lah_zero_slots": [P, I, P, I, I, I, I, P],
        "lah_signal_wait": [L, I, I, I, I, P, P],
        "lah_combine_rows": [L, P, P, P, P, I, I, I, I, L, I, I, I, I, P, P, P],
        "lah_gate_bwd": [L, P, P, P, P, P, I, I, I, I, P, I, P, P],
        "lah_router_loss_fwd": [P, I, P, I, P, P, I, P, P, P, P, P, P, P],
        "lah_router_loss_bwd": [P, I, P, I, P, P, P, P, Fl, Fl, P, P],
        "lah_adam_step": [P, P, P, P, P, P, I, P, I, P, P, I, Fl, P, Fl, Fl, Fl, Fl, I, I, I, L, P, Fl, I, P, L, I, I, I, Fl,
                          I, P],
        "lah_bump_steps": [P, P, I, P],
        "lah_cast_bf16": [P, P, L, P],
        "lah_attention_fwd": [P, P, P, L, I, I, I, c_ull, I, Fl, P, P],
        "lah_attention_bwd": [P, P, P, P, P, P, P, L, I, I, I, c_ull, I, Fl, P, P],
        "lah_attention_fwd_causal": [P, P, P, L, I, I, I, c_ull, I, Fl, P],
        "lah_attention_bwd_causal": [P, P, P, P, P, P, P, L, I, I, I, c_ull, I, Fl, P],
        "lah_pack_key_mask": [P, P, L, I, P],
        "lah_dropout_mask": [P, I, I, I, I, I, c_ull, I, P],
        "lah_dropout_ew": [I, P, P, P, L, I, c_ull, I, I, Fl, P],
        "lah_rms_norm_fwd": [P, P, P, P, I, I, Fl, P, I, P],
        "lah_rms_norm_bwd": [P, P, P, P, P, P, P, I, I, I, P, P, P],
        "lah_swiglu_fwd": [P, P, L, I, P],
        "lah_swiglu_bwd": [P, P, P, L, I, P],
        "lah_symm_alloc": [c_ull, ctypes.POINTER(c_void_p)],
        "lah_symm_free": [P],
        "lah_symm_get_handle": [P, ctypes.c_char_p],
        "lah_symm_open_handle": [ctypes.c_char_p, ctypes.POINTER(c_void_p)],
        "lah_symm_close_handle": [P],
        "lah_device_sync": [],
    }
    for name, argtypes in sigs.items():
        fn = getattr(lib, name)
        fn.restype = c_int
        fn.argtypes = argtypes
    _configured = True
    return lib


def _grid_array(grid_size):
    return (c_int * len(grid_size))(*[int(g) for g in grid_size])


def _check_ln_width(C, what, max_width=None):
    if max_width is None and not ln_width_ok(C):
        raise ValueError(f"{what}: width {C} is not a multiple of {LN_WIDTH_STEP} in [{LN_WIDTH_STEP}, {LN_MAX_WIDTH}]")
    if max_width is not None and (C <= 0 or C % LN_WIDTH_STEP):
        raise ValueError(f"{what}: width {C} is not a positive multiple of {LN_WIDTH_STEP}")


def ln_relu_fwd(h, gamma, beta, tile_group, *, out, mean, rstd, relu=True, quant=None, tile_rows=128):
    rows, C = h.shape
    _check_ln_width(C, "ln_relu_fwd")
    assert h.is_contiguous() and gamma.dtype == torch.float32 and (out is None or out.is_contiguous())
    if quant is not None:
        assert quant.K == C and quant.groups == 1 and quant.rows_per_group >= rows and quant.tile_rows == 128
        native.check(_lib().lah_ln_relu_fwd_q(ptr(h), ptr(out), ptr(mean), ptr(rstd), ptr(gamma), ptr(beta),
                                              ptr(tile_group), rows, C, int(relu), ptr(quant.q), ptr(quant.sf),
                                              stream_ptr()), "lah_ln_relu_fwd_q")
    else:
        native.check(_lib().lah_ln_relu_fwd(ptr(h), ptr(out), ptr(mean), ptr(rstd), ptr(gamma), ptr(beta),
                                            ptr(tile_group), rows, C, int(relu), int(tile_rows), stream_ptr()),
                     "lah_ln_relu_fwd")
    native.count_launch()
    return out


def ln_relu_bwd(da, h, mean, rstd, gamma, beta, tile_group, *, dh, dgamma, dbeta, dbias, relu=True, tile_rows=128,
                dres=None):
    rows, C = h.shape
    _check_ln_width(C, "ln_relu_bwd")
    assert da.is_contiguous() and h.is_contiguous() and dh.is_contiguous()
    assert dres is None or (dres.shape == h.shape and dres.dtype == torch.bfloat16 and dres.is_contiguous())
    part = torch.empty((rows + tile_rows - 1) // tile_rows, 3, C, device=h.device, dtype=torch.float32)
    native.check(_lib().lah_ln_relu_bwd(ptr(da), ptr(h), ptr(mean), ptr(rstd), ptr(gamma), ptr(beta), ptr(dh),
                                        ptr(dgamma), ptr(dbeta), ptr(dbias), ptr(part), ptr(tile_group), rows, C,
                                        int(relu), int(tile_rows), ptr(dres), stream_ptr()), "lah_ln_relu_bwd")
    native.count_launch(2)
    return dh


def _bf16_rows(t, what, shape):
    if t.dtype != torch.bfloat16 or not t.is_contiguous() or tuple(t.shape) != tuple(shape):
        raise ValueError(f"{what}: expected a contiguous bf16 tensor of shape {tuple(shape)}, got {t.dtype} "
                         f"{tuple(t.shape)}{'' if t.is_contiguous() else ' (not contiguous)'}")


def _f32_vec(t, what, n):
    if t.dtype != torch.float32 or not t.is_contiguous() or t.numel() != n:
        raise ValueError(f"{what}: expected a contiguous float32 tensor of {n} elements, got {t.dtype} {tuple(t.shape)}")


def _check_rms_groups(what, gamma, tile_group, tile_rows, rows, C):
    if tile_rows < 8 or tile_rows & (tile_rows - 1):
        raise ValueError(f"{what}: tile_rows must be a power of two >= 8, got {tile_rows}")
    if tile_group is None:
        return 1
    tiles = (rows + tile_rows - 1) // tile_rows
    if tile_group.dtype != torch.int32 or not tile_group.is_contiguous() or tile_group.numel() < tiles:
        raise ValueError(f"{what}: tile_group must be a contiguous int32 tensor of >= {tiles} entries, got "
                         f"{tile_group.dtype} {tuple(tile_group.shape)}")
    if gamma.numel() % C or gamma.numel() == 0:
        raise ValueError(f"{what}: grouped gamma must be [G, {C}], got {tuple(gamma.shape)}")
    return gamma.numel() // C


def rms_norm_fwd(x, gamma, eps, *, out, rstd, tile_group=None, tile_rows=16):
    if x.dim() != 2:
        raise ValueError(f"rms_norm_fwd: x must be [rows, C], got {tuple(x.shape)}")
    rows, C = x.shape
    _check_ln_width(C, "rms_norm_fwd")
    _bf16_rows(x, "rms_norm_fwd x", (rows, C))
    _bf16_rows(out, "rms_norm_fwd out", (rows, C))
    G = _check_rms_groups("rms_norm_fwd", gamma, tile_group, tile_rows, rows, C)
    _f32_vec(gamma, "rms_norm_fwd gamma", G * C)
    _f32_vec(rstd, "rms_norm_fwd rstd", rows)
    if not eps > 0:
        raise ValueError(f"rms_norm_fwd: eps must be > 0, got {eps}")
    native.check(_lib().lah_rms_norm_fwd(ptr(x), ptr(out), ptr(rstd), ptr(gamma), rows, C, float(eps), ptr(tile_group),
                                         int(tile_rows), stream_ptr()), "lah_rms_norm_fwd")
    native.count_launch()
    return out


def rms_norm_bwd(dn, x, rstd, gamma, *, dx, dgamma, dres=None, tile_rows=16, tile_group=None):
    if x.dim() != 2:
        raise ValueError(f"rms_norm_bwd: x must be [rows, C], got {tuple(x.shape)}")
    rows, C = x.shape
    _check_ln_width(C, "rms_norm_bwd")
    for t, what in ((dn, "dn"), (x, "x"), (dx, "dx")) + (((dres, "dres"),) if dres is not None else ()):
        _bf16_rows(t, f"rms_norm_bwd {what}", (rows, C))
    G = _check_rms_groups("rms_norm_bwd", gamma, tile_group, tile_rows, rows, C)
    _f32_vec(gamma, "rms_norm_bwd gamma", G * C)
    _f32_vec(dgamma, "rms_norm_bwd dgamma", G * C)
    _f32_vec(rstd, "rms_norm_bwd rstd", rows)
    part = torch.empty((rows + tile_rows - 1) // tile_rows, C, device=x.device, dtype=torch.float32)
    native.check(_lib().lah_rms_norm_bwd(ptr(dn), ptr(x), ptr(rstd), ptr(gamma), ptr(dx), ptr(dgamma), ptr(part), rows, C,
                                         int(tile_rows), ptr(dres), ptr(tile_group), stream_ptr()), "lah_rms_norm_bwd")
    native.count_launch(2)
    return dx


def _tile_rows_of(tile_group, tile_rows, rows):
    return tile_group.long().repeat_interleave(tile_rows)[:rows]


def rms_norm_grouped_fwd_ref(x, gamma, eps, tile_group, tile_rows):
    xf = x if x.dtype == torch.float64 else x.float()
    g = _tile_rows_of(tile_group.cpu(), tile_rows, x.shape[0]).to(x.device)
    live = (g >= 0)[:, None]
    gam = gamma.reshape(-1, x.shape[1]).to(xf.dtype)[g.clamp(min=0)]
    n, rstd = rms_norm_fwd_ref(xf, torch.ones(x.shape[1], dtype=xf.dtype, device=x.device), eps)
    return torch.where(live, n * gam, torch.zeros_like(n)), rstd


def rms_norm_grouped_bwd_ref(dn, x, gamma, eps, tile_group, tile_rows, dres=None):
    xf = x if x.dtype == torch.float64 else x.float()
    C = x.shape[1]
    gam = gamma.reshape(-1, C).to(xf.dtype)
    g = _tile_rows_of(tile_group.cpu(), tile_rows, x.shape[0]).to(x.device)
    live = g >= 0
    d = dn.to(xf.dtype) * live[:, None]
    gr = gam[g.clamp(min=0)]
    rstd = torch.rsqrt(xf.pow(2).mean(-1, keepdim=True) + eps)
    dx = rstd * (gr * d - xf * (gr * d * xf).mean(-1, keepdim=True) * rstd * rstd)
    if dres is not None:
        dx = dx + dres.to(xf.dtype)
    dx = dx * live[:, None]
    dgamma = torch.zeros_like(gam).index_add_(0, g[live], (d * xf * rstd)[live])
    return dx, dgamma


def rms_norm_fwd_ref(x, gamma, eps):
    xf = x if x.dtype == torch.float64 else x.float()
    rstd = torch.rsqrt(xf.pow(2).mean(-1) + eps)
    return xf * rstd[:, None] * gamma.to(xf.dtype), rstd


def rms_norm_bwd_ref(dn, x, gamma, eps, dres=None):
    xf = x if x.dtype == torch.float64 else x.float()
    d, g = dn.to(xf.dtype), gamma.to(xf.dtype)
    rstd = torch.rsqrt(xf.pow(2).mean(-1, keepdim=True) + eps)
    dx = rstd * (g * d - xf * (g * d * xf).mean(-1, keepdim=True) * rstd * rstd)
    if dres is not None:
        dx = dx + dres.to(xf.dtype)
    return dx, (d * xf * rstd).sum(0)


def grouped_colsum(x, tile_group, *, out, tile_rows=128):
    rows, C = x.shape
    _check_ln_width(C, "grouped_colsum", max_width=0)
    part = torch.empty((rows + tile_rows - 1) // tile_rows, C, device=x.device, dtype=torch.float32)
    native.check(_lib().lah_grouped_colsum(ptr(x), x.stride(0), ptr(out), ptr(part), C, ptr(tile_group), rows,
                                           int(tile_rows), stream_ptr()), "lah_grouped_colsum")
    native.count_launch(2)
    return out


def set_peers(bases, me):
    arr = (c_ull * len(bases))(*[int(b) for b in bases])
    native.check(_lib().lah_set_peers(ctypes.cast(arr, c_void_p), len(bases), me), "lah_set_peers")


def set_wait_counter(counter):
    native.check(_lib().lah_set_wait_counter(ptr(counter)), "lah_set_wait_counter")


def set_multicast(mc_base):
    native.check(_lib().lah_set_multicast(int(mc_base)), "lah_set_multicast")


def nvls_allreduce(off, n, scale=1.0):
    native.check(_lib().lah_nvls_allreduce(int(off), int(n), float(scale), stream_ptr()), "lah_nvls_allreduce")
    native.count_launch()


def heartbeat(hb_off, first, count, now_ms):
    native.check(_lib().lah_heartbeat(int(hb_off), int(first), int(count), int(now_ms), stream_ptr()), "lah_heartbeat")
    native.count_launch()


def alive_from_heartbeats(hb, alive, now_ms, max_age_ms):
    native.check(_lib().lah_alive_from_heartbeats(ptr(hb), ptr(alive), alive.numel(), int(now_ms), int(max_age_ms),
                                                  stream_ptr()), "lah_alive_from_heartbeats")
    native.count_launch()


def set_poison_word(status):
    native.check(_lib().lah_set_poison_word(ptr(status)), "lah_set_poison_word")


def set_step_counters(ctr):
    native.check(_lib().lah_set_step_counters(ptr(ctr)), "lah_set_step_counters")


def step_begin(epoch_delta, token_delta=0):
    native.check(_lib().lah_step_begin(int(epoch_delta), int(token_delta), stream_ptr()), "lah_step_begin")
    native.count_launch()


def set_spin_timeout_ms(ms):
    native.check(_lib().lah_set_spin_timeout_ms(int(ms)), "lah_set_spin_timeout_ms")


def gate_topk(logits, grid_size, k, *, alive=None, failure_rate=0.0, seed=0, token_offset=0, idx, w, pos, counts):
    B = logits.shape[0]
    assert logits.dtype == torch.float32 and logits.is_contiguous() and logits.shape[1] == sum(grid_size)
    native.check(_lib().lah_gate_topk(ptr(logits), B, ctypes.cast(_grid_array(grid_size), c_void_p), len(grid_size), k,
                                      ptr(alive), float(failure_rate), int(seed) & (2 ** 64 - 1), int(token_offset),
                                      ptr(idx), ptr(w), ptr(pos), ptr(counts), stream_ptr()), "lah_gate_topk")
    native.count_launch(2)


def layout_exchange(cnt_all_off, flags_off, slot, epoch, E, E_loc, max_rows, *, align=128, tile_rows=None, counts, dst_row, group_off, group_rows,
                    tile_group, total_rows, status, shadow_slots=0, shadow_tol=1.1, min_shadow_rows=512, route_owner=None,
                    step_rows=None, shadow_info=None, owned_shadow=None):
    native.check(_lib().lah_layout_exchange(cnt_all_off, flags_off, slot, epoch, E, E_loc, max_rows, align,
                                            int(tile_rows or min(align, 128)), ptr(counts),
                                            ptr(dst_row), ptr(group_off), ptr(group_rows), ptr(tile_group),
                                            ptr(total_rows), ptr(status), int(shadow_slots), float(shadow_tol),
                                            int(min_shadow_rows), ptr(route_owner), ptr(step_rows), ptr(shadow_info),
                                            ptr(owned_shadow), stream_ptr()), "lah_layout_exchange")
    native.count_launch()


def pull_shadow(shadow_info, shadow_slots, E_loc, p_off, pbf16_off, seg_sizes, small_mask):
    segs = (c_ll * len(seg_sizes))(*[int(s) for s in seg_sizes])
    native.check(_lib().lah_pull_shadow(ptr(shadow_info), int(shadow_slots), E_loc, p_off, pbf16_off, len(seg_sizes),
                                        ctypes.cast(segs, c_void_p), int(small_mask), stream_ptr()), "lah_pull_shadow")
    native.count_launch()


def zero_slots(g, seg_sizes, slots, first_slot, num_slots, seg_mask):
    segs = (c_ll * len(seg_sizes))(*[int(s) for s in seg_sizes])
    native.check(_lib().lah_zero_slots(ptr(g), len(seg_sizes), ctypes.cast(segs, c_void_p), slots, first_slot, num_slots,
                                       int(seg_mask), stream_ptr()), "lah_zero_slots")
    native.count_launch()


def scatter_rows(src, scale, idx, pos, dst_row, pair_row, dst_off, flags_off, slot, epoch, k, E_loc, max_rows,
                 group_off, group_rows, done_counter, status, align=128, route_owner=None, num_groups=0):
    num_pairs = idx.numel()
    H = src.shape[1]
    assert src.is_contiguous() and src.dtype == torch.bfloat16
    native.check(_lib().lah_scatter_rows(ptr(src), ptr(scale), ptr(idx), ptr(pos), ptr(dst_row), ptr(pair_row), dst_off,
                                         flags_off, slot, epoch, num_pairs, k, H, E_loc, max_rows, align, ptr(group_off),
                                         ptr(group_rows), ptr(done_counter), ptr(status), ptr(route_owner),
                                         int(num_groups), stream_ptr()),
                 "lah_scatter_rows")
    native.count_launch()


def signal_wait(flags_off, slot, epoch, status, *, signal=True, wait=True):
    native.check(_lib().lah_signal_wait(flags_off, slot, epoch, int(signal), int(wait), ptr(status), stream_ptr()),
                 "lah_signal_wait")
    native.count_launch()


def combine_rows(src_off, idx, pair_row, w, out, k, E_loc, *, flags_off=0, slot=0, epoch=0, signal=False, wait=False,
                 status=None, route_owner=None):
    B, H = out.shape
    native.check(_lib().lah_combine_rows(src_off, ptr(idx), ptr(pair_row), ptr(w), ptr(out), B, k, H, E_loc, flags_off,
                                         slot, epoch, int(signal), int(wait), ptr(status), ptr(route_owner),
                                         stream_ptr()),
                 "lah_combine_rows")
    native.count_launch()
    return out


def gate_bwd(yo_off, grad, idx, pair_row, w, dlogits, k, E_loc, grid_size, route_owner=None):
    B, H = grad.shape
    assert grad.is_contiguous() and grad.dtype == torch.bfloat16 and dlogits.dtype == torch.float32
    native.check(_lib().lah_gate_bwd(yo_off, ptr(grad), ptr(idx), ptr(pair_row), ptr(w), ptr(dlogits), B, k, H, E_loc,
                                     ctypes.cast(_grid_array(grid_size), c_void_p), len(grid_size), ptr(route_owner),
                                     stream_ptr()),
                 "lah_gate_bwd")
    native.count_launch()
    return dlogits


MAX_GRID_DIMS = 4
LAYOUT_MAX_E = 4096
ROUTER_WARPS = 4


def check_router_grid(grid_size):
    grid = tuple(int(g) for g in grid_size)
    if not 1 <= len(grid) <= MAX_GRID_DIMS or min(grid) < 1 or sum(grid) > LAYOUT_MAX_E or math.prod(grid) > LAYOUT_MAX_E:
        raise ValueError(f"router losses: grid_size must have 1..{MAX_GRID_DIMS} positive sizes with at most "
                         f"{LAYOUT_MAX_E} experts, got {grid_size}")
    return grid


def _router_args(what, logits, grid_size, alive):
    grid = check_router_grid(grid_size)
    if logits.dtype != torch.float32 or logits.dim() != 2 or logits.shape[1] != sum(grid) or not logits.is_contiguous():
        raise ValueError(f"{what}: logits must be a contiguous float32 [B, {sum(grid)}] tensor, got {logits.dtype} "
                         f"{tuple(logits.shape)}")
    E = math.prod(grid)
    if alive is not None and (alive.dtype != torch.uint8 or alive.numel() != E or not alive.is_contiguous()):
        raise ValueError(f"{what}: alive must be a contiguous uint8 tensor of {E} entries, got {alive.dtype} "
                         f"{tuple(alive.shape)}")
    return grid, logits.shape[0], E


def router_loss_fwd(logits, grid_size, counts, *, alive=None, f, z, Fb, loss, partials=None, ticket=None):
    grid, B, E = _router_args("router_loss_fwd", logits, grid_size, alive)
    if counts.dtype != torch.int32 or counts.dim() != 2 or counts.shape[1] != E or not counts.is_contiguous() \
            or not 1 <= counts.shape[0] <= MAX_WORLD:
        raise ValueError(f"router_loss_fwd: counts must be a contiguous int32 [R <= {MAX_WORLD}, {E}] tensor, got "
                         f"{counts.dtype} {tuple(counts.shape)}")
    nblk = (B + ROUTER_WARPS - 1) // ROUTER_WARPS
    if partials is None:
        partials = torch.empty(max(1, 2 * nblk), dtype=torch.float32, device=logits.device)
    if ticket is None:
        ticket = torch.zeros(1, dtype=torch.int32, device=logits.device)
    _f32_vec(f, "router_loss_fwd: f", E + 1)
    _f32_vec(loss, "router_loss_fwd: loss", 2)
    for t, name, n in ((z, "z", B), (Fb, "Fb", B), (partials, "partials", 2 * nblk)):
        if t.dtype != torch.float32 or not t.is_contiguous() or t.numel() < n:
            raise ValueError(f"router_loss_fwd: {name} must be a contiguous float32 tensor of >= {n} entries, got "
                             f"{t.dtype} {tuple(t.shape)}")
    if ticket.dtype != torch.int32 or ticket.numel() < 1:
        raise ValueError("router_loss_fwd: ticket must be an int32 tensor")
    native.check(_lib().lah_router_loss_fwd(ptr(logits), B, ctypes.cast(_grid_array(grid), c_void_p), len(grid),
                                            ptr(alive), ptr(counts), counts.shape[0], ptr(f), ptr(z), ptr(Fb), ptr(loss),
                                            ptr(partials), ptr(ticket), stream_ptr()), "lah_router_loss_fwd")
    native.count_launch(2 if B > 0 else 1)
    return loss


def router_loss_bwd(logits, grid_size, *, alive=None, f, z, Fb, aux_coef, z_coef, dlogits):
    grid, B, E = _router_args("router_loss_bwd", logits, grid_size, alive)
    _f32_vec(f, "router_loss_bwd: f", E + 1)
    for t, name in ((z, "z"), (Fb, "Fb")):
        if t.dtype != torch.float32 or not t.is_contiguous() or t.numel() < B:
            raise ValueError(f"router_loss_bwd: {name} must be a contiguous float32 tensor of >= {B} entries")
    if dlogits.dtype != torch.float32 or tuple(dlogits.shape) != tuple(logits.shape) or not dlogits.is_contiguous():
        raise ValueError(f"router_loss_bwd: dlogits must be a contiguous float32 {tuple(logits.shape)} tensor, got "
                         f"{dlogits.dtype} {tuple(dlogits.shape)}")
    if not (math.isfinite(aux_coef) and math.isfinite(z_coef)):
        raise ValueError("router_loss_bwd: the coefficients must be finite")
    native.check(_lib().lah_router_loss_bwd(ptr(logits), B, ctypes.cast(_grid_array(grid), c_void_p), len(grid),
                                            ptr(alive), ptr(f), ptr(z), ptr(Fb), float(aux_coef), float(z_coef),
                                            ptr(dlogits), stream_ptr()), "lah_router_loss_bwd")
    if B > 0:
        native.count_launch()
    return dlogits


MAX_SEQ = 65536
HEAD_DIMS = (32, 64, 128)
LN_WIDTH_STEP = 128
LN_MAX_WIDTH = 4096
LN_WIDTHS = tuple(range(LN_WIDTH_STEP, LN_MAX_WIDTH + 1, LN_WIDTH_STEP))


def ln_width_ok(C) -> bool:
    return 0 < C <= LN_MAX_WIDTH and C % LN_WIDTH_STEP == 0


def pack_key_mask(pad):
    assert pad.is_cuda and pad.dtype == torch.bool and pad.dim() == 2 and pad.is_contiguous(), (pad.dtype, tuple(pad.shape))
    batch, seq_len = pad.shape
    assert 1 <= seq_len <= MAX_SEQ, seq_len
    words = torch.empty(batch, (seq_len + 31) // 32, dtype=torch.int32, device=pad.device)
    native.check(_lib().lah_pack_key_mask(ptr(pad), ptr(words), batch, seq_len, stream_ptr()), "lah_pack_key_mask")
    native.count_launch()
    return words


def pack_key_mask_ref(pad):
    batch, seq_len = pad.shape
    n = (seq_len + 31) // 32
    valid = torch.zeros(batch, n * 32, dtype=torch.int64)
    valid[:, :seq_len] = (~pad.cpu()).long()
    bits = (valid.view(batch, n, 32) << torch.arange(32)).sum(-1)
    return torch.where(bits >= 2 ** 31, bits - 2 ** 32, bits).to(torch.int32)


def _check_key_mask(key_mask, tokens, seq_len, device, causal):
    assert not (causal and key_mask is not None), "causal attention takes no key padding mask"
    if key_mask is not None:
        assert key_mask.dtype == torch.int32 and key_mask.is_contiguous() and key_mask.device == device
        assert key_mask.shape == (tokens // seq_len, (seq_len + 31) // 32), (tuple(key_mask.shape), tokens, seq_len)


def attention_fwd(qkv, num_heads, *, out=None, lse=None, dropout=None, seq_len=512, key_mask=None, causal=False):
    tokens, three_d = qkv.shape
    d_model = three_d // 3
    assert 1 <= seq_len <= MAX_SEQ and tokens % seq_len == 0, (tokens, seq_len)
    assert qkv.is_cuda and qkv.dtype == torch.bfloat16 and qkv.is_contiguous()
    assert num_heads > 0 and d_model % num_heads == 0 and d_model // num_heads in HEAD_DIMS, (d_model, num_heads)
    if out is None:
        out = torch.empty(tokens, d_model, dtype=torch.bfloat16, device=qkv.device)
    assert out.dtype == torch.bfloat16 and out.is_contiguous() and out.shape == (tokens, d_model)
    if lse is not None:
        assert lse.dtype == torch.float32 and lse.is_contiguous() and lse.numel() == tokens * num_heads
    _check_key_mask(key_mask, tokens, seq_len, qkv.device, causal)
    seed, thr, rescale = _dropout_args(dropout)
    args = (ptr(qkv), ptr(out), ptr(lse), tokens, int(seq_len), num_heads, d_model, seed, thr, rescale, stream_ptr())
    if causal:
        native.check(_lib().lah_attention_fwd_causal(*args), "lah_attention_fwd_causal")
    else:
        native.check(_lib().lah_attention_fwd(*args, ptr(key_mask)), "lah_attention_fwd")
    native.count_launch()
    return out


def attention_bwd(qkv, out, dout, lse, num_heads, *, dropout=None, seq_len=512, dqkv=None, key_mask=None, causal=False):
    tokens, three_d = qkv.shape
    d_model = three_d // 3
    assert 1 <= seq_len <= MAX_SEQ and tokens % seq_len == 0, (tokens, seq_len)
    assert dout.dtype == torch.bfloat16 and dout.is_contiguous() and out.is_contiguous() and lse.dtype == torch.float32
    assert out.dtype == torch.bfloat16 and qkv.is_contiguous()
    assert num_heads > 0 and d_model % num_heads == 0 and d_model // num_heads in HEAD_DIMS, (d_model, num_heads)
    delta = torch.empty(tokens, num_heads, dtype=torch.float32, device=qkv.device)
    if dqkv is None:
        dqkv = torch.empty_like(qkv)
    assert dqkv.dtype == torch.bfloat16 and dqkv.is_contiguous() and dqkv.shape == qkv.shape
    blocks = (seq_len + 127) // 128
    dq_part = torch.empty(blocks, tokens, d_model, dtype=torch.bfloat16, device=qkv.device)
    _check_key_mask(key_mask, tokens, seq_len, qkv.device, causal)
    args = (ptr(qkv), ptr(out), ptr(dout), ptr(lse), ptr(delta), ptr(dqkv), ptr(dq_part), tokens, int(seq_len), num_heads,
            d_model, *_dropout_args(dropout), stream_ptr())
    if causal:
        native.check(_lib().lah_attention_bwd_causal(*args), "lah_attention_bwd_causal")
    else:
        native.check(_lib().lah_attention_bwd(*args, ptr(key_mask)), "lah_attention_bwd")
    native.count_launch(3)
    return dqkv


def attention_ref(qkv, num_heads, seq_len=512, key_mask=None, causal=False):
    tokens, three_d = qkv.shape
    d = three_d // 3
    x = qkv if qkv.dtype == torch.float64 else qkv.float()
    q, k, v = x.view(tokens // seq_len, seq_len, 3, num_heads, d // num_heads).unbind(2)
    q, k, v = (t.transpose(1, 2) for t in (q, k, v))
    s = q @ k.transpose(-1, -2) / (d // num_heads) ** 0.5
    if causal:
        s = s.masked_fill(torch.ones(seq_len, seq_len, dtype=torch.bool, device=s.device).triu(1), float("-inf"))
    if key_mask is None:
        att = torch.softmax(s, dim=-1) @ v
    else:
        s = s.masked_fill(key_mask.to(s.device).view(tokens // seq_len, 1, 1, seq_len), float("-inf"))
        att = torch.softmax(s, dim=-1).nan_to_num(0.0) @ v
    return att.transpose(1, 2).reshape(tokens, d)


SITE_ATTN, SITE_OUT_PROJ, SITE_FF, SITE_LINEAR2 = range(4)


def dropout_threshold(p):
    assert 0.0 <= p < 1.0, p
    return min(65535, int(math.floor(p * 65536 + 0.5)))


def _dropout_args(dropout):
    if dropout is None or dropout[0] == 0:
        return 0, -1, 1.0
    p, seed = dropout[0], dropout[1]
    return int(seed) & (2 ** 64 - 1), dropout_threshold(p), 1.0 / (1.0 - p)


def dropout_mask(shape, p, seed, site, device=None):
    if site == SITE_ATTN:
        batch, heads, rows, cols = shape
    else:
        (rows, cols), batch, heads = shape, 1, 1
    out = torch.empty(*shape, dtype=torch.uint8, device=device or "cuda")
    native.check(_lib().lah_dropout_mask(ptr(out), int(site), batch, heads, rows, cols, int(seed) & (2 ** 64 - 1),
                                         dropout_threshold(p), stream_ptr()), "lah_dropout_mask")
    native.count_launch()
    return out.bool()


def _dropout_ew(op, x, f, p, seed, site, out):
    assert x.dtype == torch.bfloat16 and x.is_contiguous() and x.dim() == 2 and 1 <= site <= 3
    assert f is None or (f.shape == x.shape and f.dtype == torch.bfloat16 and f.is_contiguous())
    out = torch.empty_like(x) if out is None else out
    assert out.shape == x.shape and out.is_contiguous()
    rows, cols = x.shape
    native.check(_lib().lah_dropout_ew(op, ptr(x), ptr(f), ptr(out), rows, cols, int(seed) & (2 ** 64 - 1), int(site),
                                       dropout_threshold(p), 1.0 / (1.0 - p), stream_ptr()), "lah_dropout_ew")
    native.count_launch()
    return out


def dropout_apply(x, p, seed, site, *, out=None):
    return _dropout_ew(0, x, None, p, seed, site, out)


def gelu_dropout(f, p, seed, site, *, out=None):
    return _dropout_ew(1, f, None, p, seed, site, out)


def gelu_dropout_bwd(dg, f, p, seed, site, *, out=None):
    return _dropout_ew(2, dg, f, p, seed, site, out)


def relu_dropout(f, p, seed, site, *, out=None):
    return _dropout_ew(3, f, None, p, seed, site, out)


def relu_dropout_bwd(dg, f, p, seed, site, *, out=None):
    return _dropout_ew(4, dg, f, p, seed, site, out)


def relu_dropout_ref(f, mask, p):
    return mask.float() * F.relu(f.float()) / (1 - p)


def relu_dropout_bwd_ref(dg, f, mask, p):
    return (f.float() > 0).float() * mask.float() * dg.float() / (1 - p)


def _check_swiglu(h, what):
    if h.dim() != 2 or h.shape[1] % 256:
        raise ValueError(f"{what}: h must be [rows, 2 * inner] with inner a multiple of 128, got {tuple(h.shape)}")
    rows, inner = h.shape[0], h.shape[1] // 2
    _bf16_rows(h, f"{what} h", (rows, 2 * inner))
    return rows, inner


def swiglu_fwd(h, *, out=None):
    rows, inner = _check_swiglu(h, "swiglu_fwd")
    out = torch.empty(rows, inner, dtype=torch.bfloat16, device=h.device) if out is None else out
    _bf16_rows(out, "swiglu_fwd out", (rows, inner))
    native.check(_lib().lah_swiglu_fwd(ptr(h), ptr(out), rows, inner, stream_ptr()), "lah_swiglu_fwd")
    native.count_launch()
    return out


def swiglu_bwd(da, h, *, out=None):
    rows, inner = _check_swiglu(h, "swiglu_bwd")
    _bf16_rows(da, "swiglu_bwd da", (rows, inner))
    out = torch.empty_like(h) if out is None else out
    _bf16_rows(out, "swiglu_bwd out", (rows, 2 * inner))
    native.check(_lib().lah_swiglu_bwd(ptr(da), ptr(h), ptr(out), rows, inner, stream_ptr()), "lah_swiglu_bwd")
    native.count_launch()
    return out


def swiglu_ref(h):
    hf = h if h.dtype == torch.float64 else h.float()
    g, u = hf.chunk(2, dim=-1)
    return F.silu(g) * u


def swiglu_bwd_ref(da, h):
    hf = h if h.dtype == torch.float64 else h.float()
    g, u = hf.chunk(2, dim=-1)
    d = da.to(hf.dtype)
    s = torch.sigmoid(g)
    return torch.cat([d * u * s * (1 + g * (1 - s)), d * g * s], dim=-1)


_PHILOX_M0, _PHILOX_M1, _PHILOX_W0, _PHILOX_W1 = 0xD2511F53, 0xCD9E8D57, 0x9E3779B9, 0xBB67AE85
_U32 = 0xFFFFFFFF


def _mulhilo32(a, m):
    t1, t2 = (a & 0xFFFF) * m, (a >> 16) * m
    return (t2 + (t1 >> 16)) >> 16, (((t2 & 0xFFFF) << 16) + t1) & _U32


def philox4x32_10_ref(ctr, key):
    c = [torch.as_tensor(w, dtype=torch.int64) for w in ctr]
    c = list(torch.broadcast_tensors(*c))
    k0, k1 = int(key[0]) & _U32, int(key[1]) & _U32
    for _ in range(10):
        hi0, lo0 = _mulhilo32(c[0], _PHILOX_M0)
        hi1, lo1 = _mulhilo32(c[2], _PHILOX_M1)
        c = [hi1 ^ c[1] ^ k0, lo1, hi0 ^ c[3] ^ k1, lo0]
        k0, k1 = (k0 + _PHILOX_W0) & _U32, (k1 + _PHILOX_W1) & _U32
    return c


def dropout_counter_ref(site, *index):
    idx = torch.broadcast_tensors(*[torch.as_tensor(t, dtype=torch.int64) for t in index])
    zero = torch.zeros_like(idx[0])
    if site == SITE_ATTN:
        b, h, q, k = idx
        gq, gk = (q >> 4) * 4 + ((q >> 1) & 3), (k >> 4) * 4 + ((k >> 1) & 3)
        ctr = ((((gq & 127) * 128) + (gk & 127)) | ((q & 1) << 14), h, b, ((gq >> 7) << 8) | ((gk >> 7) << 20) | SITE_ATTN)
        lane = ((q >> 3) & 1) * 4 + ((k & 1) | (((k >> 3) & 1) << 1))
    else:
        r, n = idx
        gr, gn = (r >> 4) * 8 + (r & 7), (n >> 4) * 4 + ((n >> 1) & 3)
        ctr = (gn, gr, zero, zero + site)
        lane = ((r >> 3) & 1) * 4 + ((n & 1) | (((n >> 3) & 1) << 1))
    return ctr, lane


def dropout_keep_ref(p, seed, site, *index):
    ctr, lane = dropout_counter_ref(site, *index)
    seed = int(seed) & (2 ** 64 - 1)
    words = torch.stack(philox4x32_10_ref(ctr, (seed & _U32, seed >> 32)), dim=-1)
    w = words.gather(-1, (lane >> 1).unsqueeze(-1)).squeeze(-1)
    u16 = torch.where((lane & 1) == 1, w >> 16, w & 0xFFFF)
    return u16 >= dropout_threshold(p)


def dropout_mask_ref(shape, p, seed, site):
    grids = [torch.arange(n).view(*([1] * i), n, *([1] * (len(shape) - i - 1))) for i, n in enumerate(shape)]
    return dropout_keep_ref(p, seed, site, *grids)


def weight_decay_args(lr, weight_decay, decoupled):
    if decoupled:
        return 0.0, 1.0 - float(lr) * float(weight_decay)
    return float(weight_decay), 1.0


def lr_block_values(lr, weight_decay, decoupled):
    return float(lr), weight_decay_args(lr, weight_decay, decoupled)[1]


def _check_lr_dev(lr_dev):
    assert (lr_dev.is_cuda and lr_dev.dtype == torch.float32 and lr_dev.numel() == 2 and lr_dev.is_contiguous()), \
        "lr_dev: a contiguous float32 CUDA tensor [lr, decay] (lr_block_values)"


def segment_views(flat, shapes, slots=1):
    views, off = {}, 0
    for name, shape in shapes.items():
        n = slots * math.prod(shape)
        views[name] = flat[off: off + n].view(slots, *shape)
        off += n
    assert off == flat.numel(), (off, flat.numel())
    return views


def adam_step(p, g, m, v, vmax, p_bf16, seg_sizes, G, *, step=None, group_rows=None, step_scalar=0, lr=1e-3,
              betas=(0.9, 0.999), eps=1e-8, weight_decay=0.0, decoupled=False, amsgrad=True, zero_mask=0, world=1,
              peer_grad_off=-1, peer_bases=None, grad_scale=1.0, G_active=0, shadow_of=None, shadow_g_off=-1, me=0,
              seg_mask=0, dead_mask=0, lr_dev=None):
    arr = None
    if peer_bases is not None:
        arr = (c_ull * len(peer_bases))(*[int(b) for b in peer_bases])
    if isinstance(seg_sizes, int):
        seg_sizes = [seg_sizes]
    segs = (c_ll * len(seg_sizes))(*[int(s) for s in seg_sizes])
    if lr_dev is not None:
        _check_lr_dev(lr_dev)
    l2, decay = weight_decay_args(lr, weight_decay, decoupled)
    native.check(_lib().lah_adam_step(ptr(p), ptr(g), ptr(m), ptr(v), ptr(vmax), ptr(p_bf16), len(seg_sizes),
                                      ctypes.cast(segs, c_void_p), G, ptr(step), ptr(group_rows), int(step_scalar), lr,
                                      ptr(lr_dev), betas[0], betas[1], eps, l2, int(amsgrad), int(zero_mask), world,
                                      peer_grad_off, ctypes.cast(arr, c_void_p) if arr is not None else c_void_p(0),
                                      grad_scale, int(G_active), ptr(shadow_of), int(shadow_g_off), int(me), int(seg_mask),
                                      int(dead_mask), decay, int(bool(decoupled and weight_decay)), stream_ptr()),
                 "lah_adam_step")
    native.count_launch()


def swapab_linear(x, w, group_off, group_rows, *, out, bias=None, residual=None, w_is_kn=False, wait=None, max_ctas=0):
    assert x.dtype == torch.bfloat16 and w.dtype == torch.bfloat16 and out.dtype == torch.bfloat16 and w.is_contiguous()
    rows, K = x.shape
    G = w.shape[0]
    M_out = w.shape[2] if w_is_kn else w.shape[1]
    assert (w.shape[1] if w_is_kn else w.shape[2]) == K and x.stride(1) == 1 and out.stride(1) == 1
    wait_flags, wait_count, wait_epoch, wait_status = (wait[0], wait[0].numel(), wait[1], wait[2]) if wait else (None, 0, 0, None)
    native.check(_lib().lah_swapab_linear(ptr(x), x.stride(0), rows, ptr(w), G, M_out, K, int(w_is_kn), ptr(out),
                                          out.stride(0), ptr(group_off), ptr(group_rows), ptr(bias), ptr(residual),
                                          residual.stride(0) if residual is not None else 0, ptr(wait_flags), wait_count,
                                          wait_epoch, ptr(wait_status), int(max_ctas), stream_ptr()),
                 "lah_swapab_linear")
    native.count_launch()
    return out


def swapab_linear_ref(x, w, group_off, group_rows, *, bias=None, residual=None, w_is_kn=False):
    off, rows = group_off.tolist(), group_rows.tolist()
    M_out = w.shape[2] if w_is_kn else w.shape[1]
    out = torch.zeros(x.shape[0], M_out, dtype=torch.float32, device=x.device)
    for g, (o, r) in enumerate(zip(off, rows)):
        if r <= 0:
            continue
        wg = w[g].float()
        y = x[o:o + r].float() @ (wg if w_is_kn else wg.t())
        if bias is not None:
            y = y + bias.view(w.shape[0], M_out)[g]
        if residual is not None:
            y = y + residual[o:o + r].float()
        out[o:o + r] = y
    return out


def wgrad_adam(dy, x, group_off, group_rows, *, p, m, v, vmax, p_bf16, step, skip=None, lr=1e-3, betas=(0.9, 0.999),
               eps=1e-8, amsgrad=True, weight_decay=0.0, decoupled=False, max_ctas=0, lr_dev=None):
    G, N, Kd = p.shape
    assert dy.shape[1] == N and x.shape[1] == Kd and dy.shape[0] == x.shape[0] and p.is_contiguous()
    assert dy.dtype == torch.bfloat16 and x.dtype == torch.bfloat16 and p.dtype == torch.float32
    if amsgrad and vmax is None:
        raise ValueError("wgrad_adam: amsgrad needs a vmax tensor (vmax=None only with amsgrad=False)")
    if lr_dev is not None:
        _check_lr_dev(lr_dev)
    l2, decay = weight_decay_args(lr, weight_decay, decoupled)
    native.check(_lib().lah_wgrad_adam(ptr(dy), dy.stride(0), ptr(x), x.stride(0), dy.shape[0], G, N, Kd, ptr(group_off),
                                       ptr(group_rows), ptr(skip), ptr(step), ptr(p), ptr(m), ptr(v), ptr(vmax), ptr(p_bf16),
                                       lr, ptr(lr_dev), betas[0], betas[1], eps, int(amsgrad), l2, decay,
                                       int(bool(decoupled and weight_decay)), int(max_ctas), stream_ptr()),
                 "lah_wgrad_adam")
    native.count_launch()


def bump_steps(step, group_rows):
    native.check(_lib().lah_bump_steps(ptr(step), ptr(group_rows), step.numel(), stream_ptr()), "lah_bump_steps")
    native.count_launch()


def cast_bf16(src, dst):
    assert src.dtype == torch.float32 and dst.dtype == torch.bfloat16 and src.numel() == dst.numel()
    native.check(_lib().lah_cast_bf16(ptr(src), ptr(dst), src.numel(), stream_ptr()), "lah_cast_bf16")
    native.count_launch()


def product_key_scores(logits, grid_size):
    parts = torch.split(logits, list(grid_size), dim=-1)
    scores = parts[0]
    for part in parts[1:]:
        scores = (scores.unsqueeze(-1) + part.unsqueeze(-2)).flatten(-2)
    return scores


def gate_topk_ref(logits, grid_size, k, alive=None, fail_mask=None):
    scores = product_key_scores(logits.float(), grid_size)
    dead = torch.zeros_like(scores, dtype=torch.bool)
    if alive is not None:
        dead |= ~alive.bool().view(1, -1)
    if fail_mask is not None:
        dead |= fail_mask
    scores = scores.masked_fill(dead, float("-inf"))
    if scores.shape[-1] < k:
        scores = F.pad(scores, (0, k - scores.shape[-1]), value=float("-inf"))
    top_v, top_i = torch.sort(scores, dim=-1, descending=True, stable=True)
    top_v, top_i = top_v[..., :k], top_i[..., :k]
    valid = torch.isfinite(top_v)
    w = torch.softmax(top_v.masked_fill(~valid, float("-inf")), dim=-1)
    w = torch.where(valid, w, torch.zeros_like(w)).nan_to_num(0.0)
    return torch.where(valid, top_i, torch.full_like(top_i, -1)), w


def router_loss_ref(logits, grid_size, counts, alive=None):
    scores = product_key_scores(logits, grid_size)
    B, E = scores.shape
    live = torch.ones(E, dtype=torch.bool, device=scores.device) if alive is None else alive.bool().reshape(-1).to(scores.device)
    c = counts.reshape(-1, E).sum(0).to(scores.dtype).to(scores.device)
    f = (c / c.sum() if float(c.sum()) > 0 else torch.zeros_like(c)).detach()
    N = int(live.sum())
    masked = scores.masked_fill(~live.view(1, -1), float("-inf"))
    ok = torch.isfinite(masked).any(-1, keepdim=True)
    masked = torch.where(ok, masked, torch.zeros_like(masked))
    if N == 0 or B == 0:
        zero = scores.sum() * 0
        return zero, zero
    z = torch.logsumexp(masked, -1, keepdim=True)
    p = torch.where(live.view(1, -1) & ok, torch.exp(masked - z), torch.zeros_like(masked))
    z = torch.where(ok, z, torch.zeros_like(z)).squeeze(-1)
    return N * (p * f).sum() / B, (z * z).sum() / B


_SPLITMIX_GAMMA = 0x9E3779B97F4A7C15


def splitmix64_ref(x):
    import numpy as np
    x = np.array(x, dtype=np.uint64, ndmin=1) + np.uint64(_SPLITMIX_GAMMA)
    x = (x ^ (x >> np.uint64(30))) * np.uint64(0xBF58476D1CE4E5B9)
    x = (x ^ (x >> np.uint64(27))) * np.uint64(0x94D049BB133111EB)
    return x ^ (x >> np.uint64(31))


def gate_fail_mask_ref(B, E, rate, seed, token_offset):
    import numpy as np
    mask64 = 2 ** 64 - 1
    tok = (np.arange(B, dtype=np.uint64) + np.uint64(int(token_offset) & mask64)) * np.uint64(0x100000001B3)
    key = np.uint64(int(seed) & mask64) ^ (tok[:, None] + np.arange(E, dtype=np.uint64)[None, :])
    u = (splitmix64_ref(key) >> np.uint64(40)).astype(np.float64) / 2.0 ** 24
    return torch.from_numpy(u < float(np.float32(rate)))


def ln_relu_ref(h, gamma, beta, relu=True):
    y = F.layer_norm(h.float(), (h.shape[-1],), gamma.float(), beta.float(), 1e-5)
    return F.relu(y) if relu else y


def ln_relu_bwd_ref(da, h, gamma, beta, relu=True, dres=None):
    hf = h.float()
    mu = hf.mean(-1, keepdim=True)
    rstd = torch.rsqrt(hf.var(-1, unbiased=False, keepdim=True) + 1e-5)
    xhat = (hf - mu) * rstd
    g = da.float()
    if relu:
        g = g * (xhat * gamma.float() + beta.float() > 0)
    dxh = g * gamma.float()
    dh = rstd * (dxh - dxh.mean(-1, keepdim=True) - xhat * (dxh * xhat).mean(-1, keepdim=True))
    if dres is not None:
        dh = dh + dres.float()
    return dh, (g * xhat).sum(0), g.sum(0), dh.sum(0)


@torch.no_grad()
def adam_step_ref(p, g, m, v, vmax, seg_sizes, G, *, step, group_rows=None, lr=1e-3, betas=(0.9, 0.999), eps=1e-8,
                  amsgrad=True, zero_mask=0, weight_decay=0.0, decoupled=False):
    if isinstance(seg_sizes, int):
        seg_sizes = [seg_sizes]
    off = 0
    active = torch.ones(G, dtype=torch.bool, device=p.device) if group_rows is None else (group_rows > 0)
    idx = active.nonzero().squeeze(1)
    stepf = step.to(torch.float32).clamp(min=1)[idx]
    bc1 = (1 - betas[0] ** stepf).view(-1, 1)
    bc2 = (1 - betas[1] ** stepf).view(-1, 1)
    for s, size in enumerate(seg_sizes):
        sl = slice(off, off + size * G)
        off += size * G
        if idx.numel() == 0:
            continue
        P, Gr, M, V = p[sl].view(G, size), g[sl].view(G, size), m[sl].view(G, size), v[sl].view(G, size)
        grad = Gr[idx]
        if weight_decay and decoupled:
            P[idx] = P[idx] * (1 - lr * weight_decay)
        elif weight_decay:
            grad = grad + weight_decay * P[idx]
        m_new = M[idx] + (1 - betas[0]) * (grad - M[idx])
        v_new = V[idx] * betas[1] + (1 - betas[1]) * grad * grad
        if amsgrad:
            VM = vmax[sl].view(G, size)
            vm_new = torch.maximum(VM[idx], v_new)
            denom = vm_new.sqrt() / bc2.sqrt() + eps
            VM[idx] = vm_new
        else:
            denom = v_new.sqrt() / bc2.sqrt() + eps
        P[idx] = P[idx] - (lr / bc1) * (m_new / denom)
        M[idx] = m_new
        V[idx] = v_new
        if (zero_mask >> s) & 1:
            Gr[idx] = 0.0
```

learning-at-home_b200/parallel/engine.py:

```python
import math
from dataclasses import dataclass, field
from typing import Dict, List, Optional, Sequence, Tuple

import torch
import torch.nn as nn
import torch.nn.functional as F

from ..models.layers import FFN_SEG_KEYS as REF_KEYS, FFN_SEG_NAMES as SEG_NAMES, FFN_SMALL_SEG_MASK as SMALL_SEG_MASK
from ..models.layers import EXPERT_LAYOUTS, gated_inner_dim
from ..ops import fp8, gemm, kernels as K, native

GATED_EPS = 1e-6


@dataclass
class DMoEConfig:
    hidden: int = 512
    grid_size: Tuple[int, ...] = (8, 8)
    k: int = 4
    num_layers: int = 4
    in_features: int = 784
    num_classes: int = 10
    tokens_per_rank: int = 1024
    capacity_factor: float = 2.0
    failure_rate: float = 0.0
    lr: float = 1e-3
    betas: Tuple[float, float] = (0.9, 0.999)
    eps: float = 1e-8
    amsgrad: bool = True
    weight_decay: float = 0.0
    decoupled_weight_decay: bool = False
    seed: int = 1337
    uid_prefix: str = "expert"
    gate_mode: str = "product_key"
    shadow_experts: int = 8
    shadow_tol: float = 1.1
    shadow_min_rows: int = 1024
    expert_dtype: str = "bf16"
    expert_path: str = "auto"
    optimizer_ctas: int = -1
    update_every_inputs: int = 0
    update_every_steps: int = 0
    trainer_staleness: int = 0
    trainer_microbatches: int = 1
    peer_timeout_ms: int = 0
    expert: str = "ffn"
    inner_dim: int = 0
    router_aux_loss_coef: float = 0.0
    router_z_loss_coef: float = 0.0

    def __post_init__(self):
        if self.expert not in EXPERT_LAYOUTS:
            raise ValueError(f"DMoEConfig.expert must be one of {sorted(EXPERT_LAYOUTS)}, got {self.expert!r}")
        if self.expert == "ffn" and self.inner_dim:
            raise ValueError("DMoEConfig.inner_dim: FeedforwardBlock experts are 4 * hidden wide; inner_dim is for "
                             "expert='swiglu' only")
        if self.inner_dim < 0:
            raise ValueError(f"DMoEConfig.inner_dim must be >= 0, got {self.inner_dim}")
        if self.expert == "swiglu" and self.expert_dtype != "bf16":
            raise ValueError("expert='swiglu' runs bf16 expert GEMMs only (its RMSNorm and SwiGLU kernels do not emit "
                             f"MXFP8 operands); got expert_dtype={self.expert_dtype!r}")
        for name in ("router_aux_loss_coef", "router_z_loss_coef"):
            v = float(getattr(self, name))
            if not math.isfinite(v) or v < 0.0:
                raise ValueError(f"DMoEConfig.{name} must be a finite value >= 0, got {v}")
            if v > 0.0 and self.gate_mode == "emulator":
                raise ValueError(f"DMoEConfig.{name}: the emulator gate is frozen (not trained), so a router loss would "
                                 "train nothing; use gate_mode='product_key'")

    @property
    def router_losses(self) -> bool:
        return self.router_aux_loss_coef > 0.0 or self.router_z_loss_coef > 0.0

    def check_native_sizes(self):
        if self.expert == "swiglu" and (self.hidden % 128 or not 128 <= self.hidden <= K.LN_MAX_WIDTH or self.inner % 128):
            raise ValueError(f"expert='swiglu' on the GPU needs hidden a multiple of 128 in [128, {K.LN_MAX_WIDTH}] and "
                             f"an inner width that is a multiple of 128; got hidden={self.hidden}, inner={self.inner}")

    @property
    def layout(self):
        return EXPERT_LAYOUTS[self.expert]

    def gemm_widths(self) -> Tuple[int, ...]:
        H, I = self.hidden, self.inner
        return (2 * I, H, I) if self.expert == "swiglu" else (I, H)

    def resolved_path(self, world: int = 1) -> str:
        if self.accumulate:
            return "big"
        if self.expert_path != "auto":
            return self.expert_path
        rows_per_expert = self.tokens_per_rank * world * self.k / max(1, self.num_experts)
        experts_per_rank = -(-self.num_experts // max(1, world))
        return "small" if (rows_per_expert < 512 and self.expert_dtype == "bf16"
                           and all(n % 128 == 0 for n in self.gemm_widths())
                           and experts_per_rank <= 1023) else "big"

    @property
    def accumulate(self) -> bool:
        return self.update_every_inputs > 1 or self.update_every_steps > 1

    def update_thresholds(self) -> Tuple[int, int]:
        never = 2 ** 31 - 1
        return (self.update_every_inputs if self.update_every_inputs > 0 else never,
                self.update_every_steps if self.update_every_steps > 0 else never)

    @property
    def num_experts(self) -> int:
        return int(math.prod(self.grid_size))

    @property
    def inner(self) -> int:
        if self.expert == "swiglu":
            return self.inner_dim or gated_inner_dim(self.hidden)
        return 4 * self.hidden

    def adam_kwargs(self) -> Dict:
        return dict(lr=self.lr, betas=self.betas, eps=self.eps, amsgrad=self.amsgrad, weight_decay=self.weight_decay,
                    decoupled=self.decoupled_weight_decay)

    def seg_shapes(self) -> Dict[str, Tuple[int, ...]]:
        return self.layout.shapes(self.hidden, self.inner)


def refuse_router_losses(cfg: DMoEConfig, arm: str):
    if cfg.router_losses:
        raise ValueError(f"{arm} does not train router losses; set router_aux_loss_coef and router_z_loss_coef to 0 "
                         "(FusedDMoE / DMoETrainer train them)")


def expert_uid(cfg: DMoEConfig, e: int) -> str:
    parts = []
    for size in reversed(cfg.grid_size):
        parts.append(str(e % size))
        e //= size
    return ".".join([cfg.uid_prefix] + parts[::-1])


class EngineContext:

    def __init__(self, cfg: DMoEConfig, group=None, device=None, heap_bytes: Optional[int] = None):
        from .symmetric import SymmetricHeap
        import torch.distributed as dist
        cfg.check_native_sizes()
        self.cfg = cfg
        self.device = device or torch.device("cuda", torch.cuda.current_device())
        distributed = dist.is_available() and dist.is_initialized()
        self.world = dist.get_world_size(group) if distributed else 1
        self.rank = dist.get_rank(group) if distributed else 0
        assert cfg.num_experts % self.world == 0, "experts must divide evenly over ranks"
        self.E = cfg.num_experts
        self.E_loc = self.E // self.world
        pairs = cfg.tokens_per_rank * cfg.k
        cap = pairs if self.world == 1 else int(math.ceil(pairs * cfg.capacity_factor))
        self.small = cfg.resolved_path(self.world) == "small"
        if self.small:
            self.align = self.tile_rows = 16
            self.S = 0
        else:
            self.align = 256 if all(n % 256 == 0 for n in cfg.gemm_widths()) else 128
            self.tile_rows = 128
            self.S = min(int(cfg.shadow_experts), 2 * K.MAX_WORLD) if self.world > 1 else 0
        self.G_tot = self.E_loc + self.S
        self.max_rows = ((cap + self.align - 1) // self.align + self.G_tot) * self.align
        self.max_rows = (self.max_rows + 127) // 128 * 128
        self.max_tiles = self.max_rows // self.tile_rows
        H = cfg.hidden
        sym_rows_bytes = self.max_rows * H * 2
        need = (3 * cfg.num_layers + 2) * (sym_rows_bytes + 4096) + K.MAX_WORLD * self.E * 4 + (32 << 20)
        if self.S:
            rec = sum(int(math.prod(shape)) for shape in cfg.seg_shapes().values())
            need += cfg.num_layers * (self.G_tot * rec * 10 + (1 << 20))
        self.heap = SymmetricHeap(heap_bytes or need, group=group, device=self.device)
        self.flags, self.flags_off = self.heap.alloc((K.NUM_SLOTS, K.MAX_WORLD), torch.int32)
        self.cnt_all, self.cnt_all_off = self.heap.alloc((K.MAX_WORLD, self.E), torch.int32)
        i32 = dict(dtype=torch.int32, device=self.device)
        self.counts = torch.zeros(self.E, **i32)
        self.done_counter = torch.zeros(1, **i32)
        self._status_buf = torch.zeros(4, **i32)
        self.status = self._status_buf[:1]
        self.wait_ns = self._status_buf[2:4].view(torch.int64)
        K.set_wait_counter(self.wait_ns)
        self.step_ctr = torch.zeros(4, **i32)
        K.set_step_counters(self.step_ctr)
        K.set_spin_timeout_ms(cfg.peer_timeout_ms)
        self.step_ctr[1] = int(cfg.peer_timeout_ms)
        self.dead_mask = 0
        import os as _os
        octas = int(_os.environ.get("LAH_OPTIMIZER_CTAS", cfg.optimizer_ctas))
        sms = torch.cuda.get_device_properties(self.device).multi_processor_count
        if octas < 0:
            octas = sms * (17 if self.world == 1 else 18) // 28
        self.opt_ctas = octas if (self.small and 0 < octas < sms - 8) else 0
        self.chain_ctas = sms - self.opt_ctas if self.opt_ctas else 0
        self.opt_stream = torch.cuda.Stream(self.device) if self.opt_ctas else None
        self._opt_pending = False
        self.defer_join = False
        K.set_poison_word(self.status)
        self._lr_written = K.lr_block_values(cfg.lr, cfg.weight_decay, cfg.decoupled_weight_decay)
        self.lr_dev = torch.tensor(self._lr_written, dtype=torch.float32, device=self.device)
        assert 2 * cfg.num_layers + 4 < self.EPOCH_STRIDE
        self.alive = torch.ones(self.E, dtype=torch.uint8, device=self.device)
        self.hb, self.hb_off = self.heap.alloc((self.E,), torch.int64)
        self.hb.zero_()
        self._hb_stream = None
        self.epoch = 0
        self.token_counter = 0
        from .profiler import StageTimer
        self.timer = StageTimer(enabled=False)
        self.gyd, self.gyd_off = self.heap.alloc((self.max_rows, H), torch.bfloat16)
        self.dxd, self.dxd_off = self.heap.alloc((self.max_rows, H), torch.bfloat16)
        if cfg.router_losses:
            blocks = -(-cfg.tokens_per_rank // K.ROUTER_WARPS)
            self.router_partials = torch.zeros(2 * blocks, dtype=torch.float32, device=self.device)
            self.router_ticket = torch.zeros(1, dtype=torch.int32, device=self.device)
        bf = dict(dtype=torch.bfloat16, device=self.device)
        for name, width in cfg.layout.buffers(H, cfg.inner)["scratch"].items():
            setattr(self, name, torch.empty(self.max_rows, width, **bf))
        self.heap.barrier()

    EPOCH_STRIDE = 64

    def adam_kwargs(self) -> Dict:
        return dict(self.cfg.adam_kwargs(), lr_dev=self.lr_dev)

    def refresh_lr(self):
        cfg = self.cfg
        vals = K.lr_block_values(cfg.lr, cfg.weight_decay, cfg.decoupled_weight_decay)
        if vals == self._lr_written or torch.cuda.is_current_stream_capturing():
            return
        self.lr_dev[0].fill_(vals[0])
        self.lr_dev[1].fill_(vals[1])
        self._lr_written = vals

    def close(self):
        K.set_wait_counter(None)
        K.set_step_counters(None)
        K.set_poison_word(None)
        self.heap.close()

    def heartbeat(self, experts=None, now: Optional[float] = None):
        import time
        first, count = experts if experts is not None else (self.rank * self.E_loc, self.E_loc)
        now_ms = int((time.time() if now is None else now) * 1000)
        if self._hb_stream is None:
            self._hb_stream = torch.cuda.Stream(self.device)
        with torch.cuda.stream(self._hb_stream):
            K.heartbeat(self.hb_off, first, count, now_ms)

    def refresh_alive(self, heartbeat_expiration: float = 120.0, now: Optional[float] = None):
        import time
        now_ms = int((time.time() if now is None else now) * 1000)
        if self._hb_stream is None:
            self._hb_stream = torch.cuda.Stream(self.device)
        with torch.cuda.stream(self._hb_stream):
            K.alive_from_heartbeats(self.hb, self.alive, now_ms, int(heartbeat_expiration * 1000))
            self._apply_dead_mask()

    def step_failed(self) -> bool:
        return bool(int(self.status.item()) & K.STATUS_TIMEOUT)

    def clear_failure(self):
        self._status_buf[0] = 0

    def detect_dead_ranks(self, max_age: float, now: Optional[float] = None):
        ages = self.heartbeat_ages(now).view(self.world, self.E_loc)
        return [r for r in range(self.world) if r != self.rank and float(ages[r].min()) > max_age]

    def exclude_ranks(self, ranks):
        for r in ranks:
            self.dead_mask |= 1 << int(r)
        self._status_buf[1] = self.dead_mask
        self._apply_dead_mask()
        self.clear_failure()

    def readmit_ranks(self, ranks):
        for r in ranks:
            self.dead_mask &= ~(1 << int(r))
        self._status_buf[1] = self.dead_mask

    def _apply_dead_mask(self):
        if self.dead_mask:
            view = self.alive.view(self.world, self.E_loc)
            for r in range(self.world):
                if (self.dead_mask >> r) & 1:
                    view[r] = 0

    def heartbeat_ages(self, now: Optional[float] = None) -> torch.Tensor:
        import time
        if self._hb_stream is not None:
            self._hb_stream.synchronize()
        hb = self.hb.cpu().double()
        now_ms = (time.time() if now is None else now) * 1000
        return torch.where(hb > 0, (now_ms - hb) / 1000.0, torch.full_like(hb, float("inf")))

    def join_optimizer_stream(self):
        if self.opt_stream is not None and self._opt_pending:
            torch.cuda.current_stream(self.device).wait_stream(self.opt_stream)
            self._opt_pending = False

    def begin_step(self):
        K.step_begin(self.EPOCH_STRIDE, self.cfg.num_layers * self.cfg.tokens_per_rank)
        self.epoch = 0
        self.token_counter = 0

    def next_epoch(self) -> int:
        if self.epoch + 1 >= self.EPOCH_STRIDE:
            self.begin_step()
        self.epoch += 1
        return self.epoch

    def exposed_wait_ms(self, reset: bool = True) -> float:
        ms = float(self.wait_ns.item()) * 1e-6
        if reset:
            self.wait_ns.zero_()
        return ms

    def check_status(self):
        code = int(self.status.item())
        if code & K.STATUS_TIMEOUT:
            raise RuntimeError("DMoE engine: timed out waiting for a peer GPU (dead rank?)")
        if code & K.STATUS_OVERFLOW:
            raise RuntimeError("DMoE engine: expert receive buffer overflow; raise DMoEConfig.capacity_factor")


class ExpertShard:

    def __init__(self, cfg: DMoEConfig, E_loc: int, first_expert: int, device, layer_index: int = 0, ctx=None):
        self.cfg, self.E_loc, self.first_expert = cfg, E_loc, first_expert
        self.slots = slots = E_loc + (ctx.S if ctx is not None else 0)
        self.layout = cfg.layout
        shapes = cfg.seg_shapes()
        shapes = {n: shapes[n] for n in self.layout.names}
        self.seg_sizes = [int(math.prod(shape)) for shape in shapes.values()]
        total = sum(self.seg_sizes) * slots
        f32 = dict(dtype=torch.float32, device=device)
        self.p_off = self.g_off = self.pbf16_off = -1
        if ctx is not None and ctx.S > 0:
            self.p, self.p_off = ctx.heap.alloc((total,), torch.float32)
            self.g, self.g_off = ctx.heap.alloc((total,), torch.float32)
            self.p_bf16, self.pbf16_off = ctx.heap.alloc((total,), torch.bfloat16)
            self.p.zero_(), self.g.zero_(), self.p_bf16.zero_()
        else:
            self.p = torch.zeros(total, **f32)
            self.g = torch.zeros(total, **f32)
            self.p_bf16 = torch.zeros(total, dtype=torch.bfloat16, device=device)
        self.m = torch.zeros(total, **f32)
        self.v = torch.zeros(total, **f32)
        self.vmax = torch.zeros(total, **f32) if cfg.amsgrad else None
        self.step = torch.zeros(E_loc, dtype=torch.int32, device=device)
        self.views, self.grads, self.bf16, self.m_views, self.v_views = (
            K.segment_views(flat, shapes, slots) for flat in (self.p, self.g, self.p_bf16, self.m, self.v))
        self.vmax_views = K.segment_views(self.vmax, shapes, slots) if self.vmax is not None else {}
        self.pending_rows = torch.zeros(E_loc, dtype=torch.int32, device=device)
        self.pending_steps = torch.zeros(E_loc, dtype=torch.int32, device=device)
        self.fire = torch.zeros(E_loc, dtype=torch.int32, device=device)
        self.w8 = None
        self.w8_dirty = True
        if cfg.expert_dtype == "fp8" and ctx is not None:
            self.w8 = {n: fp8.MXFP8Tensor(shapes[n][0], slots, shapes[n][1], fp8.WEIGHT_TILE, device)
                       for n in ("w1", "w2", "w3")}
        self.reset_parameters(layer_index)

    @torch.no_grad()
    def reset_parameters(self, layer_index: int = 0):
        cfg = self.cfg
        dev = self.p.device
        for le in range(self.E_loc):
            gen = torch.Generator(device=dev)
            gen.manual_seed(cfg.seed * 1000003 + layer_index * 10007 + self.first_expert + le)
            for n in self.layout.names:
                t = self.views[n][le]
                if n.startswith("be"):
                    t.zero_()
                elif n.startswith("g"):
                    t.fill_(1.0)
                else:
                    fan_in = self.views["w" + n[1:]].shape[-1]
                    bound = 1.0 / math.sqrt(fan_in)
                    t.uniform_(-bound, bound, generator=gen)
        self.sync_bf16()

    def fp8_weights(self):
        if self.w8_dirty:
            for n, t in self.w8.items():
                fp8.quantize(self.bf16[n].view(-1, t.K), tile_rows=fp8.WEIGHT_TILE, groups=self.slots, out=t)
            self.w8_dirty = False
        return self.w8

    def sync_bf16(self):
        self.w8_dirty = True
        if self.p.is_cuda:
            K.cast_bf16(self.p, self.p_bf16)
        else:
            self.p_bf16.copy_(self.p)

    def _expert_tensors(self, views, le: int) -> Dict[str, torch.Tensor]:
        return self.layout.module_state({n: views[n][le] for n in self.layout.names})

    def expert_state_dict(self, le: int, prefix: str = "expert.") -> Dict[str, torch.Tensor]:
        return {prefix + k: t.detach().clone().cpu() for k, t in self._expert_tensors(self.views, le).items()}

    def expert_optimizer_state(self, le: int) -> Dict:
        step = torch.tensor(float(self.step[le].item()))
        moments = [("exp_avg", self.m_views), ("exp_avg_sq", self.v_views)]
        if self.vmax is not None:
            moments.append(("max_exp_avg_sq", self.vmax_views))
        per_key = {name: self._expert_tensors(views, le) for name, views in moments}
        state = {i: dict(step=step.clone(), **{name: per_key[name][k].clone().cpu() for name, _ in moments})
                 for i, k in enumerate(self.layout.params)}
        cfg = self.cfg
        group = dict(lr=cfg.lr, betas=cfg.betas, eps=cfg.eps, weight_decay=cfg.weight_decay, amsgrad=cfg.amsgrad,
                     decoupled_weight_decay=cfg.decoupled_weight_decay, params=list(range(len(self.layout.params))))
        return dict(state=state, param_groups=[group])

    def load_expert_state_dict(self, le: int, state: Dict[str, torch.Tensor], prefix: str = "expert."):
        with torch.no_grad():
            for n, t in self.layout.segment_state(state, prefix).items():
                self.views[n][le].copy_(t)
        self.sync_bf16()

    def load_expert_optimizer_state(self, le: int, opt_state: Dict):
        with torch.no_grad():
            for i, k in enumerate(self.layout.params):
                entry = opt_state["state"].get(i)
                if entry is None:
                    continue
                n, block, parts = self.layout.slices[k]
                for name, views in (("exp_avg", self.m_views), ("exp_avg_sq", self.v_views),
                                    ("max_exp_avg_sq", self.vmax_views if self.vmax is not None else None)):
                    if views is None or name not in entry:
                        continue
                    dst = views[n][le]
                    dst = dst.chunk(parts, 0)[block] if parts > 1 else dst
                    dst.copy_(entry[name].reshape(dst.shape))
                self.step[le] = int(entry["step"])


class LayerWorkspace:
    def __init__(self, ctx: EngineContext):
        cfg, dev, R = ctx.cfg, ctx.device, ctx.max_rows
        H, I = cfg.hidden, cfg.inner
        bf = dict(dtype=torch.bfloat16, device=dev)
        i32 = dict(dtype=torch.int32, device=dev)
        f32 = dict(dtype=torch.float32, device=dev)
        self.xd, self.xd_off = ctx.heap.alloc((R, H), torch.bfloat16)
        self.yo, self.yo_off = ctx.heap.alloc((R, H), torch.bfloat16)
        buffers = cfg.layout.buffers(H, I)
        for name, width in buffers["rows"].items():
            setattr(self, name, torch.empty(R, width, **bf))
        for name in buffers["stats"]:
            setattr(self, name, torch.empty(R, **f32))
        self.xq = self.aq = None
        if cfg.expert_dtype == "fp8":
            self.xq = fp8.MXFP8Tensor(R, 1, H, fp8.ACT_TILE, dev)
            self.aq = fp8.MXFP8Tensor(R, 1, I, fp8.ACT_TILE, dev)
        P = cfg.tokens_per_rank * cfg.k
        self.idx, self.pos, self.pair_row = torch.empty(P, **i32), torch.empty(P, **i32), torch.empty(P, **i32)
        self.w = torch.empty(P, **f32)
        self.dst_row = torch.empty(ctx.E, **i32)
        self.route_owner = torch.zeros(ctx.E, **i32)
        self.group_off = torch.zeros(ctx.G_tot + 1, **i32)
        self.group_rows = torch.zeros(ctx.G_tot, **i32)
        self.step_rows = torch.zeros(ctx.E_loc, **i32)
        self.shadow_info = torch.full((max(ctx.S, 1) * 4,), -1, **i32)
        self.owned_shadow = torch.full((ctx.E_loc * 2,), -1, **i32)
        self.tile_group = torch.full((ctx.max_tiles,), -1, **i32)
        self.total_rows = torch.zeros(1, **i32)
        self.router_loss = None
        if cfg.router_losses:
            self.router_f = torch.zeros(ctx.E + 1, **f32)
            self.router_z = torch.zeros(cfg.tokens_per_rank, **f32)
            self.router_F = torch.zeros(cfg.tokens_per_rank, **f32)
            self.router_loss = torch.zeros(2, **f32)
        self.outstanding = False
        if ctx.small and ctx.opt_stream is not None:
            self.gyd, self.gyd_off = ctx.heap.alloc((R, H), torch.bfloat16)
            for name, shared in buffers["per_layer"].items():
                setattr(self, name, torch.zeros_like(getattr(ctx, shared)))
        else:
            self.gyd, self.gyd_off = ctx.gyd, ctx.gyd_off
            for name, shared in buffers["per_layer"].items():
                setattr(self, name, getattr(ctx, shared))


class _FusedDMoEFunction(torch.autograd.Function):
    @staticmethod
    def forward(ctx, x, logits, layer):
        ctx.layer = layer
        ctx.B = x.shape[0]
        ws = layer.ws
        if ws.outstanding:
            raise RuntimeError("FusedDMoE: forward() called again before the backward of the previous training-mode forward "
                               "(activations of a layer are single-buffered; run evaluate() / the next micro-batch after "
                               "backward, or call layer.release_workspace() to drop the pending forward)")
        ctx.tracked = bool(x.requires_grad or logits.requires_grad)
        ws.outstanding = ctx.tracked
        ctx.router = layer.training and layer.router_on
        if ctx.router:
            ctx.save_for_backward(logits)
        return layer._forward_cuda(x, logits)

    @staticmethod
    def backward(ctx, grad_out):
        if not ctx.layer.ws.outstanding:
            raise RuntimeError("FusedDMoE: backward() without a pending forward (the workspace was released or reused)")
        logits = ctx.saved_tensors[0] if ctx.router else None
        dx, dlogits = ctx.layer._backward_cuda(grad_out.contiguous(), ctx.B, logits)
        ctx.layer.ws.outstanding = False
        ec = ctx.layer.ctx
        if ec._opt_pending and not ec.defer_join:
            torch.autograd.Variable._execution_engine.queue_callback(ec.join_optimizer_stream)
        return dx, dlogits, None


class _AddRouterLoss(torch.autograd.Function):

    @staticmethod
    def forward(ctx, out, aux):
        ctx.aux_dtype = aux.dtype
        return out.view_as(out)

    @staticmethod
    def backward(ctx, grad_out):
        return grad_out, torch.ones((), dtype=ctx.aux_dtype, device=grad_out.device)


class FusedDMoE(nn.Module):

    def __init__(self, cfg: DMoEConfig, ctx: Optional[EngineContext] = None, layer_index: int = 0, device=None):
        super().__init__()
        if ctx is not None and cfg.router_losses and not ctx.cfg.router_losses:
            raise ValueError("FusedDMoE: router losses need an EngineContext built from a DMoEConfig with a nonzero "
                             "router_aux_loss_coef or router_z_loss_coef (the context allocates their buffers)")
        self.cfg, self.ctx, self.layer_index = cfg, ctx, layer_index
        self.grid_size = tuple(cfg.grid_size)
        if cfg.gate_mode == "emulator":
            assert len(self.grid_size) == 1, "gate_mode='emulator' scores experts densely: use grid_size=(num_experts,)"
            self.gating_pre_normalize = nn.LayerNorm(cfg.hidden)
            self.expert_keys = nn.Parameter(torch.randn(cfg.hidden, cfg.num_experts), requires_grad=False)
            self.gating_pre_normalize.requires_grad_(False)
            self.proj = None
        else:
            self.proj = nn.Linear(cfg.hidden, sum(cfg.grid_size))
        if ctx is not None:
            self.E_loc, self.first_expert, dev = ctx.E_loc, ctx.rank * ctx.E_loc, ctx.device
            self.ws = LayerWorkspace(ctx)
        else:
            self.E_loc, self.first_expert, dev = cfg.num_experts, 0, device or torch.device("cpu")
            self.ws = None
        self.shard = ExpertShard(cfg, self.E_loc, self.first_expert, dev, layer_index, ctx=ctx)
        self.ref_fail_mask = None
        self.ref_emulate_bf16 = False
        self._ref_rows = None
        self._ref_leaves = {}
        self.router_aux_coef = float(cfg.router_aux_loss_coef)
        self.router_z_coef = float(cfg.router_z_loss_coef)
        self.router_on = self.router_aux_coef > 0.0 or self.router_z_coef > 0.0
        self.router_grad_scale = 1.0
        if self.ws is not None:
            self.router_loss = self.ws.router_loss if self.router_on else None
        else:
            self.register_buffer("router_loss", torch.zeros(2, device=dev) if self.router_on else None, persistent=False)

    def forward(self, x):
        return self.forward_with_gate(x, self.proj)

    def gate_logits(self, x, proj=None):
        if self.cfg.gate_mode == "emulator" and proj is None:
            if x.is_cuda and x.dtype == torch.bfloat16:
                ln = self.gating_pre_normalize
                key = (self.expert_keys._version, ln.weight._version, ln.bias._version, self.expert_keys.data_ptr())
                if getattr(self, "_gate_cache_key", None) != key:
                    with torch.no_grad():
                        self._gate_cache = (ln.weight.to(x.dtype), ln.bias.to(x.dtype),
                                            F.normalize(self.expert_keys, dim=-1).to(x.dtype).contiguous())
                    self._gate_cache_key = key
                w_ln, b_ln, keys = self._gate_cache
                xn = F.layer_norm(x, (x.shape[-1],), w_ln, b_ln, ln.eps)
                return (xn @ keys).float()
            return self.gating_pre_normalize(x.float()) @ F.normalize(self.expert_keys, dim=-1)
        return F.linear(x.float(), proj.weight, proj.bias)

    def forward_with_gate(self, x, proj: Optional[nn.Linear]):
        assert x.dim() == 2 and x.shape[1] == self.cfg.hidden
        logits = self.gate_logits(x, proj)
        if self.ctx is None:
            return self._forward_ref(x, logits, emulate_bf16=self.ref_emulate_bf16)
        assert x.shape[0] <= self.cfg.tokens_per_rank, "batch exceeds DMoEConfig.tokens_per_rank"
        return _FusedDMoEFunction.apply(x.to(torch.bfloat16).contiguous(), logits.contiguous(), self)

    def release_workspace(self):
        if self.ws is not None:
            self.ws.outstanding = False

    def _forward_cuda(self, x, logits):
        c, ws, sh, cfg = self.ctx, self.ws, self.shard, self.cfg
        B, k = x.shape[0], cfg.k
        P = B * k
        c.join_optimizer_stream()
        c.refresh_lr()
        epoch = c.next_epoch()
        idx, w, pos, pair_row = ws.idx[:P], ws.w[:P], ws.pos[:P], ws.pair_row[:P]
        K.gate_topk(logits, self.grid_size, k, alive=c.alive, failure_rate=cfg.failure_rate if self.training else 0.0,
                    seed=cfg.seed * 7919 + self.layer_index, token_offset=c.token_counter, idx=idx, w=w, pos=pos,
                    counts=c.counts)
        c.token_counter += B
        c.timer.mark("gate_topk")
        K.layout_exchange(c.cnt_all_off, c.flags_off, K.SLOT_COUNTS, epoch, c.E, c.E_loc, c.max_rows, align=c.align,
                          tile_rows=c.tile_rows, counts=c.counts,
                          dst_row=ws.dst_row, group_off=ws.group_off, group_rows=ws.group_rows,
                          tile_group=ws.tile_group, total_rows=ws.total_rows, status=c.status, shadow_slots=c.S,
                          shadow_tol=cfg.shadow_tol, min_shadow_rows=cfg.shadow_min_rows, route_owner=ws.route_owner,
                          step_rows=ws.step_rows, shadow_info=ws.shadow_info, owned_shadow=ws.owned_shadow)
        if self.training and self.router_on:
            K.router_loss_fwd(logits, self.grid_size, c.cnt_all[:c.world], alive=c.alive, f=ws.router_f, z=ws.router_z,
                              Fb=ws.router_F, loss=ws.router_loss, partials=c.router_partials, ticket=c.router_ticket)
        if c.S:
            K.pull_shadow(ws.shadow_info, c.S, c.E_loc, sh.p_off, sh.pbf16_off, sh.seg_sizes, sh.layout.small_mask)
            sh.w8_dirty = True
        K.scatter_rows(x, None, idx, pos, ws.dst_row, pair_row, ws.xd_off, c.flags_off, K.SLOT_DISPATCH, epoch, k,
                       c.E_loc, c.max_rows, ws.group_off, ws.group_rows, c.done_counter, c.status, align=c.align,
                       route_owner=ws.route_owner, num_groups=c.G_tot)
        c.timer.mark("dispatch(layout+pull+scatter)")
        tg = ws.tile_group
        wait = (c.flags[K.SLOT_DISPATCH, :c.world], epoch, c.status) if c.world > 1 else None
        if cfg.expert == "swiglu":
            self._expert_gated_fwd(wait, epoch)
        elif c.small:
            go, gr_, T = ws.group_off, ws.group_rows, c.tile_rows
            K.swapab_linear(ws.xd, sh.bf16["w1"], go, gr_, out=ws.h1, bias=sh.views["b1"], wait=wait)
            K.ln_relu_fwd(ws.h1, sh.views["g1"], sh.views["be1"], tg, out=ws.a1, mean=ws.mean1, rstd=ws.rstd1, tile_rows=T)
            K.swapab_linear(ws.a1, sh.bf16["w2"], go, gr_, out=ws.h2, bias=sh.views["b2"])
            K.ln_relu_fwd(ws.h2, sh.views["g2"], sh.views["be2"], tg, out=ws.a2, mean=ws.mean2, rstd=ws.rstd2, tile_rows=T)
            K.swapab_linear(ws.a2, sh.bf16["w3"], go, gr_, out=ws.yo, bias=sh.views["b3"], residual=ws.xd)
        elif cfg.expert_dtype == "fp8":
            self._expert_ffn_fp8(wait, epoch)
        else:
            gemm.grouped_linear(ws.xd, sh.bf16["w1"], tile_group=tg, bias=sh.views["b1"], out=ws.h1, wait=wait)
            K.ln_relu_fwd(ws.h1, sh.views["g1"], sh.views["be1"], tg, out=ws.a1, mean=ws.mean1, rstd=ws.rstd1)
            gemm.grouped_linear(ws.a1, sh.bf16["w2"], tile_group=tg, bias=sh.views["b2"], out=ws.h2)
            K.ln_relu_fwd(ws.h2, sh.views["g2"], sh.views["be2"], tg, out=ws.a2, mean=ws.mean2, rstd=ws.rstd2)
            gemm.grouped_linear(ws.a2, sh.bf16["w3"], tile_group=tg, bias=sh.views["b3"], residual=ws.xd, out=ws.yo)
        c.timer.mark("expert_ffn_fwd")
        y = torch.empty(B, cfg.hidden, dtype=torch.bfloat16, device=x.device)
        K.combine_rows(ws.yo_off, idx, pair_row, w, y, k, c.E_loc, flags_off=c.flags_off, slot=K.SLOT_OUTPUT, epoch=epoch,
                       signal=c.world > 1, wait=c.world > 1, status=c.status, route_owner=ws.route_owner)
        c.timer.mark("combine")
        return y

    def _expert_gated_fwd(self, wait, epoch):
        c, ws, sh = self.ctx, self.ws, self.shard
        tg, T = ws.tile_group, c.tile_rows
        if wait is not None:
            K.signal_wait(c.flags_off, K.SLOT_DISPATCH, epoch, c.status, signal=False, wait=True)
        K.rms_norm_fwd(ws.xd, sh.views["g"], GATED_EPS, out=ws.n, rstd=ws.rstd, tile_group=tg, tile_rows=T)
        if c.small:
            go, gr_ = ws.group_off, ws.group_rows
            K.swapab_linear(ws.n, sh.bf16["w13"], go, gr_, out=ws.h)
            K.swiglu_fwd(ws.h, out=ws.a)
            K.swapab_linear(ws.a, sh.bf16["w2"], go, gr_, out=ws.yo, residual=ws.xd)
        else:
            gemm.grouped_linear(ws.n, sh.bf16["w13"], tile_group=tg, out=ws.h)
            K.swiglu_fwd(ws.h, out=ws.a)
            gemm.grouped_linear(ws.a, sh.bf16["w2"], tile_group=tg, residual=ws.xd, out=ws.yo)

    def _expert_ffn_fp8(self, wait, epoch):
        c, ws, sh = self.ctx, self.ws, self.shard
        assert c.align == 256, "the FP8 path needs 256-row expert groups (hidden and 4*hidden multiples of 256)"
        tg = ws.tile_group
        if wait is not None:
            K.signal_wait(c.flags_off, K.SLOT_DISPATCH, epoch, c.status, signal=False, wait=True)
        w8 = sh.fp8_weights()
        fp8.quantize(ws.xd, tile_group=tg, out=ws.xq)
        fp8.grouped_linear_fp8(ws.xq, w8["w1"], tile_group=tg, bias=sh.views["b1"], out=ws.h1)
        K.ln_relu_fwd(ws.h1, sh.views["g1"], sh.views["be1"], tg, out=ws.a1, mean=ws.mean1, rstd=ws.rstd1, quant=ws.aq)
        fp8.grouped_linear_fp8(ws.aq, w8["w2"], tile_group=tg, bias=sh.views["b2"], out=ws.h2)
        K.ln_relu_fwd(ws.h2, sh.views["g2"], sh.views["be2"], tg, out=ws.a2, mean=ws.mean2, rstd=ws.rstd2, quant=ws.aq)
        fp8.grouped_linear_fp8(ws.aq, w8["w3"], tile_group=tg, bias=sh.views["b3"], residual=ws.xd, out=ws.yo)

    def _backward_cuda(self, gy, B, logits=None):
        c, ws, sh, cfg = self.ctx, self.ws, self.shard, self.cfg
        k = cfg.k
        P = B * k
        epoch = c.next_epoch()
        idx, w, pos, pair_row = ws.idx[:P], ws.w[:P], ws.pos[:P], ws.pair_row[:P]
        gy = gy.to(torch.bfloat16)
        dlogits = torch.empty(B, sum(self.grid_size), dtype=torch.float32, device=gy.device)
        K.gate_bwd(ws.yo_off, gy, idx, pair_row, w, dlogits, k, c.E_loc, self.grid_size, route_owner=ws.route_owner)
        if logits is not None:
            K.router_loss_bwd(logits, self.grid_size, alive=c.alive, f=ws.router_f, z=ws.router_z, Fb=ws.router_F,
                              aux_coef=self.router_aux_coef * self.router_grad_scale,
                              z_coef=self.router_z_coef * self.router_grad_scale, dlogits=dlogits)
        K.scatter_rows(gy, w, idx, pos, None, pair_row, ws.gyd_off, c.flags_off, K.SLOT_GRAD, epoch, k, c.E_loc,
                       c.max_rows, ws.group_off, ws.group_rows, c.done_counter, c.status, align=c.align,
                       route_owner=ws.route_owner, num_groups=c.G_tot)
        if c.S:
            K.zero_slots(sh.g, sh.seg_sizes, c.G_tot, c.E_loc, c.S, sh.layout.small_mask)
        if c.world > 1:
            K.signal_wait(c.flags_off, K.SLOT_GRAD, epoch, c.status, signal=False, wait=True)
        c.timer.mark("bwd_gate+dispatch_grad")
        tg, go, G = ws.tile_group, ws.group_off, c.G_tot
        gr = sh.grads
        if c.small:
            self._backward_small(epoch)
            c.timer.mark("expert_ffn_bwd(dgrad+ln+fused wgrad/AMSGrad)")
            dx = torch.empty(B, cfg.hidden, dtype=torch.bfloat16, device=gy.device)
            K.combine_rows(c.dxd_off, idx, pair_row, None, dx, k, c.E_loc, flags_off=c.flags_off, slot=K.SLOT_DINPUT,
                           epoch=epoch, signal=c.world > 1, wait=c.world > 1, status=c.status, route_owner=ws.route_owner)
            c.timer.mark("bwd_combine")
            return dx, dlogits
        if cfg.expert == "swiglu":
            gemm.grouped_wgrad(c.gyd, ws.a, go, G, out=gr["w2"], accumulate=cfg.accumulate)
            gemm.grouped_linear(c.gyd, sh.bf16["w2"], tile_group=tg, w_is_kn=True, out=c.da)
            K.swiglu_bwd(c.da, ws.h, out=c.dh)
            gemm.grouped_wgrad(c.dh, ws.n, go, G, out=gr["w13"], accumulate=cfg.accumulate)
            gemm.grouped_linear(c.dh, sh.bf16["w13"], tile_group=tg, w_is_kn=True, out=c.dn)
            K.rms_norm_bwd(c.dn, ws.xd, ws.rstd, sh.views["g"], dx=c.dxd, dgamma=gr["g"], dres=c.gyd,
                           tile_rows=c.tile_rows, tile_group=tg)
        else:
            K.grouped_colsum(c.gyd, tg, out=gr["b3"])
            gemm.grouped_wgrad(c.gyd, ws.a2, go, G, out=gr["w3"], accumulate=cfg.accumulate)
            gemm.grouped_linear(c.gyd, sh.bf16["w3"], tile_group=tg, w_is_kn=True, out=c.da)
            K.ln_relu_bwd(c.da, ws.h2, ws.mean2, ws.rstd2, sh.views["g2"], sh.views["be2"], tg, dh=c.dh, dgamma=gr["g2"],
                          dbeta=gr["be2"], dbias=gr["b2"])
            gemm.grouped_wgrad(c.dh, ws.a1, go, G, out=gr["w2"], accumulate=cfg.accumulate)
            gemm.grouped_linear(c.dh, sh.bf16["w2"], tile_group=tg, w_is_kn=True, out=c.da)
            K.ln_relu_bwd(c.da, ws.h1, ws.mean1, ws.rstd1, sh.views["g1"], sh.views["be1"], tg, dh=c.dh, dgamma=gr["g1"],
                          dbeta=gr["be1"], dbias=gr["b1"])
            gemm.grouped_wgrad(c.dh, ws.xd, go, G, out=gr["w1"], accumulate=cfg.accumulate)
            gemm.grouped_linear(c.dh, sh.bf16["w1"], tile_group=tg, w_is_kn=True, residual=c.gyd, out=c.dxd)
        c.timer.mark("expert_ffn_bwd(wgrad+dgrad+ln)")
        if c.S:
            K.signal_wait(c.flags_off, K.SLOT_SHADOW, epoch, c.status, signal=True, wait=True)
        self.apply_expert_gradients()
        c.timer.mark("expert_adam")
        dx = torch.empty(B, cfg.hidden, dtype=torch.bfloat16, device=gy.device)
        K.combine_rows(c.dxd_off, idx, pair_row, None, dx, k, c.E_loc, flags_off=c.flags_off, slot=K.SLOT_DINPUT,
                       epoch=epoch, signal=c.world > 1, wait=c.world > 1, status=c.status, route_owner=ws.route_owner)
        c.timer.mark("bwd_combine")
        return dx, dlogits

    def _backward_small(self, epoch):
        c, ws, sh, cfg = self.ctx, self.ws, self.shard, self.cfg
        tg, go, rows, T = ws.tile_group, ws.group_off, ws.group_rows, c.tile_rows
        gr = sh.grads
        opt = c.adam_kwargs()
        main = torch.cuda.current_stream(c.device)
        side, chain_ctas = c.opt_stream, c.chain_ctas

        def wgrad(name, dy, x):
            kw = dict(p=sh.views[name][:self.E_loc], m=sh.m_views[name][:self.E_loc], v=sh.v_views[name][:self.E_loc],
                      vmax=sh.vmax_views[name][:self.E_loc] if cfg.amsgrad else None, p_bf16=sh.bf16[name], step=sh.step, **opt)
            if side is None:
                K.wgrad_adam(dy, x, go, rows, **kw)
                return
            side.wait_stream(main)
            with torch.cuda.stream(side):
                K.wgrad_adam(dy, x, go, rows, max_ctas=c.opt_ctas, **kw)
            c._opt_pending = True

        gyd = ws.gyd
        K.bump_steps(sh.step, ws.step_rows)
        if cfg.expert == "swiglu":
            dh13 = ws.dh13
            K.swapab_linear(gyd, sh.bf16["w2"], go, rows, out=c.da, w_is_kn=True, max_ctas=chain_ctas)
            wgrad("w2", gyd, ws.a)
            K.swiglu_bwd(c.da, ws.h, out=dh13)
            K.swapab_linear(dh13, sh.bf16["w13"], go, rows, out=c.dn, w_is_kn=True, max_ctas=chain_ctas)
            wgrad("w13", dh13, ws.n)
            K.rms_norm_bwd(c.dn, ws.xd, ws.rstd, sh.views["g"], dx=c.dxd, dgamma=gr["g"], dres=gyd, tile_rows=T,
                           tile_group=tg)
        else:
            dh2, dh1 = ws.dh2, ws.dh1
            K.grouped_colsum(gyd, tg, out=gr["b3"], tile_rows=T)
            K.swapab_linear(gyd, sh.bf16["w3"], go, rows, out=c.da, w_is_kn=True, max_ctas=chain_ctas)
            wgrad("w3", gyd, ws.a2)
            K.ln_relu_bwd(c.da, ws.h2, ws.mean2, ws.rstd2, sh.views["g2"], sh.views["be2"], tg, dh=dh2, dgamma=gr["g2"],
                          dbeta=gr["be2"], dbias=gr["b2"], tile_rows=T)
            K.swapab_linear(dh2, sh.bf16["w2"], go, rows, out=c.da, w_is_kn=True, max_ctas=chain_ctas)
            wgrad("w2", dh2, ws.a1)
            K.ln_relu_bwd(c.da, ws.h1, ws.mean1, ws.rstd1, sh.views["g1"], sh.views["be1"], tg, dh=dh1, dgamma=gr["g1"],
                          dbeta=gr["be1"], dbias=gr["b1"], tile_rows=T)
            K.swapab_linear(dh1, sh.bf16["w1"], go, rows, out=c.dxd, w_is_kn=True, residual=gyd, max_ctas=chain_ctas)
            wgrad("w1", dh1, ws.xd)
        small = sh.layout.small_mask
        K.adam_step(sh.p, sh.g, sh.m, sh.v, sh.vmax, sh.p_bf16, sh.seg_sizes, sh.slots, step=sh.step,
                    group_rows=ws.step_rows, zero_mask=small, G_active=self.E_loc, seg_mask=small, **opt)
        sh.w8_dirty = True

    def apply_expert_gradients(self):
        sh, cfg, ws, c = self.shard, self.cfg, self.ws, self.ctx
        rows, zero_mask = ws.step_rows, sh.layout.small_mask
        if cfg.accumulate:
            sh.pending_rows += ws.step_rows
            sh.pending_steps += (sh.pending_rows > 0).to(torch.int32)
            thr_rows, thr_steps = cfg.update_thresholds()
            due = (sh.pending_rows > 0) & ((sh.pending_rows >= thr_rows) | (sh.pending_steps >= thr_steps))
            sh.fire.copy_(due.to(torch.int32))
            sh.pending_rows.mul_(1 - sh.fire)
            sh.pending_steps.mul_(1 - sh.fire)
            rows, zero_mask = sh.fire, (1 << len(sh.layout.names)) - 1
        K.bump_steps(sh.step, rows)
        K.adam_step(sh.p, sh.g, sh.m, sh.v, sh.vmax, sh.p_bf16, sh.seg_sizes, sh.slots, step=sh.step,
                    group_rows=rows, **c.adam_kwargs(), zero_mask=zero_mask, G_active=self.E_loc, world=c.world,
                    peer_bases=c.heap.peer_bases if c.S else None, shadow_of=ws.owned_shadow if c.S else None,
                    shadow_g_off=sh.g_off, me=c.rank)
        sh.w8_dirty = True

    def failure_rate_ref(self) -> float:
        return self.cfg.failure_rate if (self.training and self.ctx is None) else 0.0

    def _expert_params(self, e_local: int, dtype=torch.float32):
        if self.ctx is None and torch.is_grad_enabled() and self.training:
            leaves = self._ref_leaves.get(e_local)
            if leaves is None:
                leaves = {n: self.shard.views[n][e_local].detach().requires_grad_(True) for n in self.shard.layout.names}
                self._ref_leaves[e_local] = leaves
            return leaves
        return {n: self.shard.views[n][e_local].to(dtype) for n in self.shard.layout.names}

    def apply_expert_gradients_ref(self):
        sh, cfg = self.shard, self.cfg
        if self._ref_rows is None:
            return
        rows, zero_mask = self._ref_rows, 0
        with torch.no_grad():
            for le, leaves in self._ref_leaves.items():
                for n, leaf in leaves.items():
                    if cfg.accumulate:
                        if leaf.grad is not None:
                            sh.grads[n][le].add_(leaf.grad)
                    elif leaf.grad is not None:
                        sh.grads[n][le].copy_(leaf.grad)
                    else:
                        sh.grads[n][le].zero_()
                    leaf.grad = None
            if cfg.accumulate:
                sh.pending_rows += rows.to(sh.pending_rows.dtype)
                sh.pending_steps += (sh.pending_rows > 0).to(sh.pending_steps.dtype)
                thr_rows, thr_steps = cfg.update_thresholds()
                due = (sh.pending_rows > 0) & ((sh.pending_rows >= thr_rows) | (sh.pending_steps >= thr_steps))
                keep = (~due).to(sh.pending_rows.dtype)
                sh.pending_rows.mul_(keep)
                sh.pending_steps.mul_(keep)
                rows, zero_mask = due.to(rows.dtype), (1 << len(sh.layout.names)) - 1
            sh.step += (rows > 0).to(sh.step.dtype)
            K.adam_step_ref(sh.p, sh.g, sh.m, sh.v, sh.vmax, sh.seg_sizes, self.E_loc, step=sh.step,
                            group_rows=rows, **cfg.adam_kwargs(), zero_mask=zero_mask)
        sh.sync_bf16()
        self._ref_rows = None
        self._ref_leaves = {}

    def _forward_ref(self, x, logits, emulate_bf16: bool = False):
        cfg = self.cfg
        fail_mask = self.ref_fail_mask
        if fail_mask is None and self.failure_rate_ref() > 0:
            fail_mask = torch.rand(x.shape[0], cfg.num_experts, device=x.device) < cfg.failure_rate
        idx, w_sel = K.gate_topk_ref(logits.detach(), self.grid_size, cfg.k,
                                     alive=self.ctx.alive if self.ctx is not None else getattr(self, "alive_ref", None),
                                     fail_mask=fail_mask)
        scores = K.product_key_scores(logits, self.grid_size)
        safe_idx = idx.clamp(min=0)
        sel = torch.gather(scores, 1, safe_idx).masked_fill(idx < 0, float("-inf"))
        weights = torch.softmax(sel, dim=-1)
        weights = torch.where(idx >= 0, weights, torch.zeros_like(weights))
        xf = x.float()
        out = torch.zeros(x.shape[0], cfg.hidden, dtype=torch.float32, device=x.device)
        rnd = (lambda t: t.to(torch.bfloat16).float()) if emulate_bf16 else (lambda t: t)
        if self.training:
            rows = torch.bincount(idx[idx >= 0].flatten() - self.first_expert, minlength=self.E_loc)
            self._ref_rows = rows if self._ref_rows is None else self._ref_rows + rows
        for e in idx[idx >= 0].unique().tolist():
            le = e - self.first_expert
            p = self._expert_params(le)
            if emulate_bf16:
                p = {n: (rnd(v) if n.startswith("w") else v) for n, v in p.items()}
            tok, slot = torch.nonzero(idx == e, as_tuple=True)
            ye = self._expert_ref(p, rnd(xf[tok]), rnd)
            out = out.index_put((tok,), ye * weights[tok, slot].unsqueeze(-1), accumulate=True)
        if self.training and self.router_on:
            alive = self.ctx.alive if self.ctx is not None else getattr(self, "alive_ref", None)
            counts = torch.bincount(idx[idx >= 0].flatten(), minlength=cfg.num_experts)
            l_aux, l_z = K.router_loss_ref(logits, self.grid_size, counts, alive=alive)
            with torch.no_grad():
                self.router_loss.copy_(torch.stack([l_aux, l_z]).detach())
            if torch.is_grad_enabled() and logits.requires_grad:
                aux = self.router_grad_scale * (self.router_aux_coef * l_aux + self.router_z_coef * l_z)
                out = _AddRouterLoss.apply(out, aux)
        return out.to(x.dtype)

    def _expert_ref(self, p, xe, rnd):
        cfg = self.cfg
        if cfg.expert == "swiglu":
            n = rnd(F.rms_norm(xe, (cfg.hidden,), p["g"], GATED_EPS))
            hg, hu = rnd(F.linear(n, p["w13"])).chunk(2, dim=-1)
            a = rnd(F.silu(hg) * hu)
            return rnd(F.linear(a, p["w2"]) + xe)
        h1 = rnd(F.linear(xe, p["w1"], p["b1"]))
        a1 = rnd(F.relu(F.layer_norm(h1, (cfg.inner,), p["g1"], p["be1"])))
        h2 = rnd(F.linear(a1, p["w2"], p["b2"]))
        a2 = rnd(F.relu(F.layer_norm(h2, (cfg.inner,), p["g2"], p["be2"])))
        return rnd(F.linear(a2, p["w3"], p["b3"]) + xe)


class DMoEClassifier(nn.Module):
    def __init__(self, cfg: DMoEConfig, ctx: Optional[EngineContext] = None, device=None):
        super().__init__()
        self.cfg = cfg
        self.stem = nn.Linear(cfg.in_features, cfg.hidden)
        self.blocks = nn.ModuleList([FusedDMoE(cfg, ctx, layer_index=i, device=device) for i in range(cfg.num_layers)])
        self.norm = nn.LayerNorm(cfg.hidden)
        self.head = nn.Linear(cfg.hidden, cfg.num_classes)

    def forward(self, x):
        on_gpu = self.blocks[0].ctx is not None
        if on_gpu:
            h = F.linear(x.to(torch.bfloat16), self.stem.weight.to(torch.bfloat16), self.stem.bias.to(torch.bfloat16))
        else:
            h = self.stem(x)
        for block in self.blocks:
            h = block(h)
        h = self.norm(h.float())
        return self.head(h)

    def non_expert_parameters(self):
        return list(self.parameters())
```

Before: 12890.

## Store fp32 master weights as bf16 hi plane plus low-bits plane in fused wgrad-Adam

Adds a split representation of the fp32 master weights: a bf16 high plane that doubles as the bf16 compute copy, and a 16-bit low plane. A tie bit packed into the sign of v makes the split reconstruct the exact fp32 value. The fused wgrad+Adam kernel now loads and stores the two planes through TMA instead of the fp32 master, and drops the separate bf16 write, which cuts state bytes per weight. In exchange it adds encode/decode kernels, extra bit manipulation in the update loop, and invasive changes to the Python state views (raw_views, v_raw, lo_views).

```diff
diff --git a/learning-at-home_b200/csrc/adam.cu b/learning-at-home_b200/csrc/adam.cu
--- a/learning-at-home_b200/csrc/adam.cu
+++ b/learning-at-home_b200/csrc/adam.cu
@@ -122,6 +122,43 @@
         q.x = pack_bf16x2(p.x, p.y);
         q.y = pack_bf16x2(p.z, p.w);
         *reinterpret_cast<uint2*>(dst + i) = q;
+    }
+}
+
+__global__ void split_encode_kernel(const float* __restrict__ p, bf16* __restrict__ hi, uint16_t* __restrict__ lo,
+                                    float* __restrict__ v, long long n) {
+    const long long stride = static_cast<long long>(gridDim.x) * blockDim.x * 4;
+    for (long long i = (static_cast<long long>(blockIdx.x) * blockDim.x + threadIdx.x) * 4; i < n; i += stride) {
+        const float4 w = *reinterpret_cast<const float4*>(p + i);
+        float4 s = *reinterpret_cast<const float4*>(v + i);
+        uint2 h, l;
+        h.x = pack_bf16x2(w.x, w.y);
+        h.y = pack_bf16x2(w.z, w.w);
+        l.x = (__float_as_uint(w.x) & 0xffffu) | (__float_as_uint(w.y) << 16);
+        l.y = (__float_as_uint(w.z) & 0xffffu) | (__float_as_uint(w.w) << 16);
+        s.x = with_tie_bit(without_tie_bit(s.x), split_tie_up(w.x));
+        s.y = with_tie_bit(without_tie_bit(s.y), split_tie_up(w.y));
+        s.z = with_tie_bit(without_tie_bit(s.z), split_tie_up(w.z));
+        s.w = with_tie_bit(without_tie_bit(s.w), split_tie_up(w.w));
+        *reinterpret_cast<uint2*>(hi + i) = h;
+        *reinterpret_cast<uint2*>(lo + i) = l;
+        *reinterpret_cast<float4*>(v + i) = s;
+    }
+}
+
+__global__ void split_decode_kernel(const bf16* __restrict__ hi, const uint16_t* __restrict__ lo,
+                                    const float* __restrict__ v, float* __restrict__ p, long long n) {
+    const long long stride = static_cast<long long>(gridDim.x) * blockDim.x * 4;
+    for (long long i = (static_cast<long long>(blockIdx.x) * blockDim.x + threadIdx.x) * 4; i < n; i += stride) {
+        const uint2 h = *reinterpret_cast<const uint2*>(hi + i);
+        const uint2 l = *reinterpret_cast<const uint2*>(lo + i);
+        const float4 s = *reinterpret_cast<const float4*>(v + i);
+        float4 w;
+        w.x = split_decode(h.x & 0xffffu, l.x & 0xffffu, __float_as_uint(s.x) >> 31);
+        w.y = split_decode(h.x >> 16, l.x >> 16, __float_as_uint(s.y) >> 31);
+        w.z = split_decode(h.y & 0xffffu, l.y & 0xffffu, __float_as_uint(s.z) >> 31);
+        w.w = split_decode(h.y >> 16, l.y >> 16, __float_as_uint(s.w) >> 31);
+        *reinterpret_cast<float4*>(p + i) = w;
     }
 }
 
@@ -210,4 +247,16 @@
     return -(int)cudaGetLastError();
 }
 
-}
+int lah_split_master(float* p, void* hi, void* lo, float* v, long long n, int encode, cudaStream_t st) {
+    if (n % 4) return -2;
+    if (n <= 0) return 0;
+    long long blocks = (n / 4 + 255) / 256;
+    if (blocks > 132 * 16) blocks = 132 * 16;
+    if (encode)
+        split_encode_kernel<<<(int)blocks, 256, 0, st>>>(p, (bf16*)hi, (uint16_t*)lo, v, n);
+    else
+        split_decode_kernel<<<(int)blocks, 256, 0, st>>>((const bf16*)hi, (const uint16_t*)lo, v, p, n);
+    return -(int)cudaGetLastError();
+}
+
+}
diff --git a/learning-at-home_b200/csrc/sm90.cuh b/learning-at-home_b200/csrc/sm90.cuh
--- a/learning-at-home_b200/csrc/sm90.cuh
+++ b/learning-at-home_b200/csrc/sm90.cuh
@@ -296,6 +296,16 @@
     __nv_bfloat162 v = *reinterpret_cast<__nv_bfloat162*>(&u);
     return __bfloat1622float2(v);
 }
+__device__ __forceinline__ float split_decode(uint32_t hi, uint32_t lo, bool tie_up) {
+    const uint32_t up = (lo > 0x8000u || (lo == 0x8000u && tie_up)) ? 1u : 0u;
+    return __uint_as_float(((hi - up) << 16) | lo);
+}
+__device__ __forceinline__ uint32_t split_tie_up(float p) {
+    const uint32_t b = __float_as_uint(p);
+    return ((b & 0xffffu) == 0x8000u && (b & 0x10000u)) ? 0x80000000u : 0u;
+}
+__device__ __forceinline__ float with_tie_bit(float v, uint32_t tie) { return __uint_as_float(__float_as_uint(v) | tie); }
+__device__ __forceinline__ float without_tie_bit(float v) { return __uint_as_float(__float_as_uint(v) & 0x7fffffffu); }
 __device__ __forceinline__ float warp_sum(float v) {
 #pragma unroll
     for (int o = 16; o > 0; o >>= 1) v += __shfl_xor_sync(0xffffffffu, v, o);
diff --git a/learning-at-home_b200/csrc/small_m.cu b/learning-at-home_b200/csrc/small_m.cu
--- a/learning-at-home_b200/csrc/small_m.cu
+++ b/learning-at-home_b200/csrc/small_m.cu
@@ -291,25 +291,40 @@
     int g, mt, nt;
 };
 
+template <bool SPLIT>
 struct StateMaps {
-    CUtensorMap a[4];
+    CUtensorMap a[SPLIT ? 5 : 4];
 };
-
-__device__ __forceinline__ void state_chunk_tma(const StateMaps& tm, int n_arr, uint8_t* ss, uint64_t* bar, int col0, int srow,
-                                                int c) {
-    for (int a = 0; a < n_arr; ++a)
+constexpr int PLANE_COLS = 64;
+constexpr int PLANE_BYTES = ARR_BYTES / 2;
+static_assert(PLANE_BYTES == (BN_MAX / PLANE_COLS) * SUB_BYTES, "a plane box has the rows and bytes of an fp32 box");
+
+template <bool SPLIT>
+__device__ __forceinline__ void state_chunk_tma(const StateMaps<SPLIT>& tm, int n_arr, uint8_t* ss, uint64_t* bar, int col0,
+                                                int srow, int c) {
+    if constexpr (SPLIT) {
+        for (int a = 0; a < 2; ++a)
+#pragma unroll
+            for (int q = 0; q < BN_MAX / PLANE_COLS; ++q) {
+                uint8_t* s = ss + a * PLANE_BYTES + q * SUB_BYTES;
+                if (bar) tma_load_3d(s, &tm.a[a], bar, col0 + q * PLANE_COLS, BAND_ROWS * c, srow / 16);
+                else tma_store_3d(&tm.a[a], s, col0 + q * PLANE_COLS, BAND_ROWS * c, srow / 16);
+            }
+    }
+    for (int a = SPLIT ? 1 : 0; a < n_arr; ++a)
 #pragma unroll
         for (int q = 0; q < BN_MAX / SUB_COLS; ++q) {
             uint8_t* s = ss + a * ARR_BYTES + q * SUB_BYTES;
-            if (bar) tma_load_3d(s, &tm.a[a], bar, col0 + q * SUB_COLS, BAND_ROWS * c, srow / 16);
-            else tma_store_3d(&tm.a[a], s, col0 + q * SUB_COLS, BAND_ROWS * c, srow / 16);
-        }
-}
-
-template <int WD, bool DEV_LR>
+            const CUtensorMap* m = &tm.a[SPLIT ? a + 1 : a];
+            if (bar) tma_load_3d(s, m, bar, col0 + q * SUB_COLS, BAND_ROWS * c, srow / 16);
+            else tma_store_3d(m, s, col0 + q * SUB_COLS, BAND_ROWS * c, srow / 16);
+        }
+}
+
+template <int WD, bool DEV_LR, bool SPLIT>
 __global__ void __launch_bounds__(NUM_THREADS, 1)
 wgrad_adam_kernel(const Params p, const __grid_constant__ CUtensorMap tmDY, const __grid_constant__ CUtensorMap tmX,
-                  const __grid_constant__ StateMaps tmS, const float* __restrict__ lr_dev) {
+                  const __grid_constant__ StateMaps<SPLIT> tmS, const float* __restrict__ lr_dev) {
     extern __shared__ uint8_t smem_raw[];
     uint8_t* smem = reinterpret_cast<uint8_t*>((reinterpret_cast<uintptr_t>(smem_raw) + 1023) & ~uintptr_t(1023));
     uint8_t* st_smem = smem + ST_OFFSET;
@@ -329,7 +344,7 @@
     if (warp == 8 && lane == 0) {
         tma_prefetch_desc(&tmDY);
         tma_prefetch_desc(&tmX);
-        for (int a = 0; a < n_arr; ++a) tma_prefetch_desc(&tmS.a[a]);
+        for (int a = 0; a < n_arr + (SPLIT ? 1 : 0); ++a) tma_prefetch_desc(&tmS.a[a]);
         for (int i = 0; i < OP_STAGES; ++i) {
             mbar_init(&op_full[i], 1);
             mbar_init(&op_empty[i], 8);
@@ -494,7 +509,19 @@
                 float2* sm = reinterpret_cast<float2*>(ss + ARR_BYTES + so);
                 float2* sv = reinterpret_cast<float2*>(ss + 2 * ARR_BYTES + so);
                 float2* svm = reinterpret_cast<float2*>(ss + 3 * ARR_BYTES + so);
-                float2 pw = *sp, m = *sm, v = *sv;
+                const int po = (j >> 3) * SUB_BYTES + R * 128 + (((j & 7) ^ (R & 7)) << 4) + 4 * (lane & 3);
+                uint32_t* shi = reinterpret_cast<uint32_t*>(ss + po);
+                uint32_t* slo = reinterpret_cast<uint32_t*>(ss + PLANE_BYTES + po);
+                float2 pw, m = *sm, v = *sv;
+                if constexpr (SPLIT) {
+                    const uint32_t hw = *shi, lw = *slo;
+                    pw.x = split_decode(hw & 0xffffu, lw & 0xffffu, __float_as_uint(v.x) >> 31);
+                    pw.y = split_decode(hw >> 16, lw >> 16, __float_as_uint(v.y) >> 31);
+                    v.x = without_tie_bit(v.x);
+                    v.y = without_tie_bit(v.y);
+                } else {
+                    pw = *sp;
+                }
                 float2 vm = p.amsgrad ? *svm : make_float2(0.f, 0.f);
                 float* pp = &pw.x; float* mp = &m.x; float* vp = &v.x; float* vmp = &vm.x;
 #pragma unroll
@@ -514,11 +541,18 @@
                     }
                     pp[e] -= step_size * (mp[e] / denom);
                 }
-                *sp = pw;
+                if constexpr (SPLIT) {
+                    *shi = pack_bf16x2(pw.x, pw.y);
+                    *slo = (__float_as_uint(pw.x) & 0xffffu) | (__float_as_uint(pw.y) << 16);
+                    v.x = with_tie_bit(v.x, split_tie_up(pw.x));
+                    v.y = with_tie_bit(v.y, split_tie_up(pw.y));
+                } else {
+                    *sp = pw;
+                }
                 *sm = m;
                 *sv = v;
                 if (p.amsgrad) *svm = vm;
-                *reinterpret_cast<uint32_t*>(p.p_bf16 + o_row + 8 * j) = pack_bf16x2(pw.x, pw.y);
+                if constexpr (!SPLIT) *reinterpret_cast<uint32_t*>(p.p_bf16 + o_row + 8 * j) = pack_bf16x2(pw.x, pw.y);
             }
             fence_proxy_async_smem();
             named_bar_sync(1, 256);
@@ -620,32 +654,41 @@
 
 }
 
-template <int WD, bool DEV_LR>
-static int launch_wgrad_adam(const wa::Params& a, const CUtensorMap& tmDY, const CUtensorMap& tmX, const wa::StateMaps& tmS,
-                             const float* lr_dev, int ctas, cudaStream_t st) {
-    if (int e = set_max_dynamic_smem<wa::wgrad_adam_kernel<WD, DEV_LR>>(wa::SMEM_TOTAL)) return e;
-    wa::wgrad_adam_kernel<WD, DEV_LR><<<ctas, NUM_THREADS, wa::SMEM_TOTAL, st>>>(a, tmDY, tmX, tmS, lr_dev);
+template <int WD, bool DEV_LR, bool SPLIT>
+static int launch_wgrad_adam(const wa::Params& a, const CUtensorMap& tmDY, const CUtensorMap& tmX,
+                             const wa::StateMaps<SPLIT>& tmS, const float* lr_dev, int ctas, cudaStream_t st) {
+    if (int e = set_max_dynamic_smem<wa::wgrad_adam_kernel<WD, DEV_LR, SPLIT>>(wa::SMEM_TOTAL)) return e;
+    wa::wgrad_adam_kernel<WD, DEV_LR, SPLIT><<<ctas, NUM_THREADS, wa::SMEM_TOTAL, st>>>(a, tmDY, tmX, tmS, lr_dev);
     return -(int)cudaGetLastError();
 }
 
-extern "C" {
-
-int lah_wgrad_adam(const void* dy, long long lddy, const void* x, long long ldx, int total_rows, int G, int N, int K,
-                   const int* group_off, const int* group_rows, const int* skip, const int* step, float* p, float* m,
-                   float* v, float* vmax, void* p_bf16, float lr, const float* lr_dev, float beta1, float beta2, float eps,
-                   int amsgrad, float weight_decay, float decay, int decoupled, int max_ctas, cudaStream_t st) {
+template <bool SPLIT>
+static int wgrad_adam(const void* dy, long long lddy, const void* x, long long ldx, int total_rows, int G, int N, int K,
+                      const int* group_off, const int* group_rows, const int* skip, const int* step, void* p, void* lo,
+                      float* m, float* v, float* vmax, void* p_bf16, float lr, const float* lr_dev, float beta1, float beta2,
+                      float eps, int amsgrad, float weight_decay, float decay, int decoupled, int max_ctas, cudaStream_t st) {
     if ((N % BM) || (K % BN_MAX) || (lddy % 8) || (ldx % 8) || 1ll * G * N > INT_MAX) return -2;
     if (decoupled && weight_decay != 0.f) return -2;
     if (amsgrad && !vmax) return -2;
     CUtensorMap tmDY, tmX;
-    wa::StateMaps tmS;
+    wa::StateMaps<SPLIT> tmS;
     {
-        float* arrs[4] = {p, m, v, amsgrad ? vmax : p};
+        void* arrs[5] = {p, m, v, amsgrad ? vmax : (float*)m, nullptr};
+        if (SPLIT) {
+            arrs[1] = lo; arrs[2] = m; arrs[3] = v; arrs[4] = amsgrad ? vmax : m;
+        }
         uint64_t dims[3] = {(uint64_t)K, 16, (uint64_t)G * N / 16};
         uint64_t str[2] = {(uint64_t)K * 4, (uint64_t)K * 64};
         uint32_t box[3] = {wa::SUB_COLS, wa::BAND_ROWS, BM / 16};
-        for (int a = 0; a < 4; ++a) {
-            int r = make_tmap(&tmS.a[a], CU_TENSOR_MAP_DATA_TYPE_FLOAT32, 3, arrs[a], dims, str, box);
+        for (int a = 0; a < (SPLIT ? 5 : 4); ++a) {
+            int r;
+            if (SPLIT && a < 2) {
+                uint64_t pstr[2] = {(uint64_t)K * 2, (uint64_t)K * 32};
+                uint32_t pbox[3] = {wa::PLANE_COLS, wa::BAND_ROWS, BM / 16};
+                r = make_tmap(&tmS.a[a], CU_TENSOR_MAP_DATA_TYPE_BFLOAT16, 3, arrs[a], dims, pstr, pbox);
+            } else {
+                r = make_tmap(&tmS.a[a], CU_TENSOR_MAP_DATA_TYPE_FLOAT32, 3, arrs[a], dims, str, box);
+            }
             if (r) return r;
         }
     }
@@ -665,7 +708,7 @@
     }
     wa::Params a;
     a.G = G; a.N = N; a.K = K; a.group_off = group_off; a.group_rows = group_rows; a.skip = skip; a.step = step;
-    a.p = p; a.m = m; a.v = v; a.vmax = vmax; a.p_bf16 = (bf16*)p_bf16; a.lr = lr; a.beta1 = beta1; a.beta2 = beta2; a.eps = eps; a.amsgrad = amsgrad;
+    a.p = SPLIT ? nullptr : (float*)p; a.m = m; a.v = v; a.vmax = vmax; a.p_bf16 = (bf16*)p_bf16; a.lr = lr; a.beta1 = beta1; a.beta2 = beta2; a.eps = eps; a.amsgrad = amsgrad;
     a.wd = decoupled ? decay : weight_decay;
     a.tile_counter = tile_counter() ? tile_counter() + 16 : nullptr;
     a.poison = g_poison;
@@ -675,13 +718,33 @@
     if (cudaMemsetAsync(a.tile_counter, 0, sizeof(int), st) != cudaSuccess) return -4;
     const int ctas = persistent_grid(total, max_ctas);
     if (lr_dev) {
-        if (decoupled) return launch_wgrad_adam<wa::WD_DECOUPLED, true>(a, tmDY, tmX, tmS, lr_dev, ctas, st);
-        if (weight_decay != 0.f) return launch_wgrad_adam<wa::WD_L2, true>(a, tmDY, tmX, tmS, lr_dev, ctas, st);
-        return launch_wgrad_adam<wa::WD_NONE, true>(a, tmDY, tmX, tmS, lr_dev, ctas, st);
-    }
-    if (decoupled) return launch_wgrad_adam<wa::WD_DECOUPLED, false>(a, tmDY, tmX, tmS, nullptr, ctas, st);
-    if (weight_decay != 0.f) return launch_wgrad_adam<wa::WD_L2, false>(a, tmDY, tmX, tmS, nullptr, ctas, st);
-    return launch_wgrad_adam<wa::WD_NONE, false>(a, tmDY, tmX, tmS, nullptr, ctas, st);
-}
-
-}
+        if (decoupled) return launch_wgrad_adam<wa::WD_DECOUPLED, true, SPLIT>(a, tmDY, tmX, tmS, lr_dev, ctas, st);
+        if (weight_decay != 0.f) return launch_wgrad_adam<wa::WD_L2, true, SPLIT>(a, tmDY, tmX, tmS, lr_dev, ctas, st);
+        return launch_wgrad_adam<wa::WD_NONE, true, SPLIT>(a, tmDY, tmX, tmS, lr_dev, ctas, st);
+    }
+    if (decoupled) return launch_wgrad_adam<wa::WD_DECOUPLED, false, SPLIT>(a, tmDY, tmX, tmS, nullptr, ctas, st);
+    if (weight_decay != 0.f) return launch_wgrad_adam<wa::WD_L2, false, SPLIT>(a, tmDY, tmX, tmS, nullptr, ctas, st);
+    return launch_wgrad_adam<wa::WD_NONE, false, SPLIT>(a, tmDY, tmX, tmS, nullptr, ctas, st);
+}
+
+extern "C" {
+
+int lah_wgrad_adam(const void* dy, long long lddy, const void* x, long long ldx, int total_rows, int G, int N, int K,
+                   const int* group_off, const int* group_rows, const int* skip, const int* step, float* p, float* m,
+                   float* v, float* vmax, void* p_bf16, float lr, const float* lr_dev, float beta1, float beta2, float eps,
+                   int amsgrad, float weight_decay, float decay, int decoupled, int max_ctas, cudaStream_t st) {
+    return wgrad_adam<false>(dy, lddy, x, ldx, total_rows, G, N, K, group_off, group_rows, skip, step, p, nullptr, m, v,
+                             vmax, p_bf16, lr, lr_dev, beta1, beta2, eps, amsgrad, weight_decay, decay, decoupled, max_ctas,
+                             st);
+}
+
+int lah_wgrad_adam_split(const void* dy, long long lddy, const void* x, long long ldx, int total_rows, int G, int N, int K,
+                         const int* group_off, const int* group_rows, const int* skip, const int* step, void* hi, void* lo,
+                         float* m, float* v, float* vmax, float lr, const float* lr_dev, float beta1, float beta2, float eps,
+                         int amsgrad, float weight_decay, float decay, int decoupled, int max_ctas, cudaStream_t st) {
+    if (!hi || !lo) return -2;
+    return wgrad_adam<true>(dy, lddy, x, ldx, total_rows, G, N, K, group_off, group_rows, skip, step, hi, lo, m, v, vmax,
+                            nullptr, lr, lr_dev, beta1, beta2, eps, amsgrad, weight_decay, decay, decoupled, max_ctas, st);
+}
+
+}
diff --git a/learning-at-home_b200/ops/kernels.py b/learning-at-home_b200/ops/kernels.py
--- a/learning-at-home_b200/ops/kernels.py
+++ b/learning-at-home_b200/ops/kernels.py
@@ -36,6 +36,7 @@
         "lah_step_begin": [I, L, P],
         "lah_swapab_linear": [P, L, I, P, I, I, I, I, P, L, P, P, P, P, L, P, I, I, P, I, P],
         "lah_wgrad_adam": [P, L, P, L, I, I, I, I, P, P, P, P, P, P, P, P, P, Fl, P, Fl, Fl, Fl, I, Fl, Fl, I, I, P],
+        "lah_wgrad_adam_split": [P, L, P, L, I, I, I, I, P, P, P, P, P, P, P, P, P, Fl, P, Fl, Fl, Fl, I, Fl, Fl, I, I, P],
         "lah_ln_relu_fwd_q": [P, P, P, P, P, P, P, I, I, I, P, P, P],
         "lah_set_peers": [P, I, I],
         "lah_set_wait_counter": [P],
@@ -53,6 +54,7 @@
                           I, P],
         "lah_bump_steps": [P, P, I, P],
         "lah_cast_bf16": [P, P, L, P],
+        "lah_split_master": [P, P, P, P, L, I, P],
         "lah_attention_fwd": [P, P, P, L, I, I, I, c_ull, I, Fl, P, P],
         "lah_attention_bwd": [P, P, P, P, P, P, P, L, I, I, I, c_ull, I, Fl, P, P],
         "lah_attention_fwd_causal": [P, P, P, L, I, I, I, c_ull, I, Fl, P],
@@ -771,20 +773,30 @@
 
 
 def wgrad_adam(dy, x, group_off, group_rows, *, p, m, v, vmax, p_bf16, step, skip=None, lr=1e-3, betas=(0.9, 0.999),
-               eps=1e-8, amsgrad=True, weight_decay=0.0, decoupled=False, max_ctas=0, lr_dev=None):
-    G, N, Kd = p.shape
-    assert dy.shape[1] == N and x.shape[1] == Kd and dy.shape[0] == x.shape[0] and p.is_contiguous()
-    assert dy.dtype == torch.bfloat16 and x.dtype == torch.bfloat16 and p.dtype == torch.float32
+               eps=1e-8, amsgrad=True, weight_decay=0.0, decoupled=False, max_ctas=0, lr_dev=None, p_lo=None):
+    G, N, Kd = (p if p_lo is None else p_lo).shape
+    assert dy.shape[1] == N and x.shape[1] == Kd and dy.shape[0] == x.shape[0]
+    assert dy.dtype == torch.bfloat16 and x.dtype == torch.bfloat16
+    if p_lo is None:
+        assert p.is_contiguous() and p.dtype == torch.float32
+    else:
+        assert p is None and p_lo.dtype == torch.int16 and p_bf16.dtype == torch.bfloat16
+        assert p_lo.is_contiguous() and p_bf16.is_contiguous() and p_bf16.shape[1:] == p_lo.shape[1:]
     if amsgrad and vmax is None:
         raise ValueError("wgrad_adam: amsgrad needs a vmax tensor (vmax=None only with amsgrad=False)")
     if lr_dev is not None:
         _check_lr_dev(lr_dev)
     l2, decay = weight_decay_args(lr, weight_decay, decoupled)
-    native.check(_lib().lah_wgrad_adam(ptr(dy), dy.stride(0), ptr(x), x.stride(0), dy.shape[0], G, N, Kd, ptr(group_off),
-                                       ptr(group_rows), ptr(skip), ptr(step), ptr(p), ptr(m), ptr(v), ptr(vmax), ptr(p_bf16),
-                                       lr, ptr(lr_dev), betas[0], betas[1], eps, int(amsgrad), l2, decay,
-                                       int(bool(decoupled and weight_decay)), int(max_ctas), stream_ptr()),
-                 "lah_wgrad_adam")
+    common = (ptr(dy), dy.stride(0), ptr(x), x.stride(0), dy.shape[0], G, N, Kd, ptr(group_off), ptr(group_rows),
+              ptr(skip), ptr(step))
+    tail = (lr, ptr(lr_dev), betas[0], betas[1], eps, int(amsgrad), l2, decay, int(bool(decoupled and weight_decay)),
+            int(max_ctas), stream_ptr())
+    if p_lo is None:
+        native.check(_lib().lah_wgrad_adam(*common, ptr(p), ptr(m), ptr(v), ptr(vmax), ptr(p_bf16), *tail),
+                     "lah_wgrad_adam")
+    else:
+        native.check(_lib().lah_wgrad_adam_split(*common, ptr(p_bf16), ptr(p_lo), ptr(m), ptr(v), ptr(vmax), *tail),
+                     "lah_wgrad_adam_split")
     native.count_launch()
 
 
@@ -796,6 +808,26 @@
 def cast_bf16(src, dst):
     assert src.dtype == torch.float32 and dst.dtype == torch.bfloat16 and src.numel() == dst.numel()
     native.check(_lib().lah_cast_bf16(ptr(src), ptr(dst), src.numel(), stream_ptr()), "lah_cast_bf16")
+    native.count_launch()
+
+
+def _check_split(p, hi, lo, v):
+    n = p.numel()
+    assert p.dtype == torch.float32 and hi.dtype == torch.bfloat16 and lo.dtype == torch.int16 and v.dtype == torch.float32
+    assert hi.numel() == n and lo.numel() == n and v.numel() == n
+    assert all(t.is_contiguous() and t.is_cuda for t in (p, hi, lo, v))
+
+
+def split_encode(p, hi, lo, v):
+    _check_split(p, hi, lo, v)
+    native.check(_lib().lah_split_master(ptr(p), ptr(hi), ptr(lo), ptr(v), p.numel(), 1, stream_ptr()), "lah_split_master")
+    native.count_launch()
+
+
+def split_decode(hi, lo, v, out):
+    _check_split(out, hi, lo, v)
+    native.check(_lib().lah_split_master(ptr(out), ptr(hi), ptr(lo), ptr(v), out.numel(), 0, stream_ptr()),
+                 "lah_split_master")
     native.count_launch()
 
 
diff --git a/learning-at-home_b200/parallel/engine.py b/learning-at-home_b200/parallel/engine.py
--- a/learning-at-home_b200/parallel/engine.py
+++ b/learning-at-home_b200/parallel/engine.py
@@ -337,21 +337,28 @@
         f32 = dict(dtype=torch.float32, device=device)
         self.p_off = self.g_off = self.pbf16_off = -1
         if ctx is not None and ctx.S > 0:
-            self.p, self.p_off = ctx.heap.alloc((total,), torch.float32)
+            self.p_raw, self.p_off = ctx.heap.alloc((total,), torch.float32)
             self.g, self.g_off = ctx.heap.alloc((total,), torch.float32)
             self.p_bf16, self.pbf16_off = ctx.heap.alloc((total,), torch.bfloat16)
-            self.p.zero_(), self.g.zero_(), self.p_bf16.zero_()
-        else:
-            self.p = torch.zeros(total, **f32)
+            self.p_raw.zero_(), self.g.zero_(), self.p_bf16.zero_()
+        else:
+            self.p_raw = torch.zeros(total, **f32)
             self.g = torch.zeros(total, **f32)
             self.p_bf16 = torch.zeros(total, dtype=torch.bfloat16, device=device)
         self.m = torch.zeros(total, **f32)
-        self.v = torch.zeros(total, **f32)
+        self.v_raw = torch.zeros(total, **f32)
         self.vmax = torch.zeros(total, **f32) if cfg.amsgrad else None
         self.step = torch.zeros(E_loc, dtype=torch.int32, device=device)
-        self.views, self.grads, self.bf16, self.m_views, self.v_views = (
-            K.segment_views(flat, shapes, slots) for flat in (self.p, self.g, self.p_bf16, self.m, self.v))
+        self._shapes = shapes
+        self.raw_views, self.grads, self.bf16, self.m_views, self.v_raw_views = (
+            K.segment_views(flat, shapes, slots) for flat in (self.p_raw, self.g, self.p_bf16, self.m, self.v_raw))
         self.vmax_views = K.segment_views(self.vmax, shapes, slots) if self.vmax is not None else {}
+        self.split = ctx is not None and ctx.small
+        self.matrices = [n for s, n in enumerate(self.layout.names) if not (self.layout.small_mask >> s) & 1]
+        self.lo_views = {}
+        if self.split:
+            self.lo_views = {n: torch.zeros(self.raw_views[n].shape, dtype=torch.int16, device=device)
+                             for n in self.matrices}
         self.pending_rows = torch.zeros(E_loc, dtype=torch.int32, device=device)
         self.pending_steps = torch.zeros(E_loc, dtype=torch.int32, device=device)
         self.fire = torch.zeros(E_loc, dtype=torch.int32, device=device)
@@ -365,18 +372,19 @@
     @torch.no_grad()
     def reset_parameters(self, layer_index: int = 0):
         cfg = self.cfg
-        dev = self.p.device
+        dev = self.p_raw.device
+        views = self.raw_views
         for le in range(self.E_loc):
             gen = torch.Generator(device=dev)
             gen.manual_seed(cfg.seed * 1000003 + layer_index * 10007 + self.first_expert + le)
             for n in self.layout.names:
-                t = self.views[n][le]
+                t = views[n][le]
                 if n.startswith("be"):
                     t.zero_()
                 elif n.startswith("g"):
                     t.fill_(1.0)
                 else:
-                    fan_in = self.views["w" + n[1:]].shape[-1]
+                    fan_in = views["w" + n[1:]].shape[-1]
                     bound = 1.0 / math.sqrt(fan_in)
                     t.uniform_(-bound, bound, generator=gen)
         self.sync_bf16()
@@ -390,10 +398,31 @@
 
     def sync_bf16(self):
         self.w8_dirty = True
-        if self.p.is_cuda:
-            K.cast_bf16(self.p, self.p_bf16)
-        else:
-            self.p_bf16.copy_(self.p)
+        if self.p_raw.is_cuda:
+            K.cast_bf16(self.p_raw, self.p_bf16)
+        else:
+            self.p_bf16.copy_(self.p_raw)
+        for n in (self.matrices if self.split else ()):
+            K.split_encode(self.raw_views[n], self.bf16[n], self.lo_views[n], self.v_raw_views[n])
+
+    @property
+    def p(self) -> torch.Tensor:
+        for n in (self.matrices if self.split else ()):
+            K.split_decode(self.bf16[n], self.lo_views[n], self.v_raw_views[n], out=self.raw_views[n])
+        return self.p_raw
+
+    @property
+    def views(self) -> Dict[str, torch.Tensor]:
+        self.p
+        return self.raw_views
+
+    @property
+    def v(self) -> torch.Tensor:
+        return self.v_raw.abs() if self.split else self.v_raw
+
+    @property
+    def v_views(self) -> Dict[str, torch.Tensor]:
+        return K.segment_views(self.v, self._shapes, self.slots) if self.split else self.v_raw_views
 
     def _expert_tensors(self, views, le: int) -> Dict[str, torch.Tensor]:
         return self.layout.module_state({n: views[n][le] for n in self.layout.names})
@@ -416,18 +445,20 @@
 
     def load_expert_state_dict(self, le: int, state: Dict[str, torch.Tensor], prefix: str = "expert."):
         with torch.no_grad():
+            views = self.views
             for n, t in self.layout.segment_state(state, prefix).items():
-                self.views[n][le].copy_(t)
+                views[n][le].copy_(t)
         self.sync_bf16()
 
     def load_expert_optimizer_state(self, le: int, opt_state: Dict):
         with torch.no_grad():
+            self.p
             for i, k in enumerate(self.layout.params):
                 entry = opt_state["state"].get(i)
                 if entry is None:
                     continue
                 n, block, parts = self.layout.slices[k]
-                for name, views in (("exp_avg", self.m_views), ("exp_avg_sq", self.v_views),
+                for name, views in (("exp_avg", self.m_views), ("exp_avg_sq", self.v_raw_views),
                                     ("max_exp_avg_sq", self.vmax_views if self.vmax is not None else None)):
                     if views is None or name not in entry:
                         continue
@@ -435,6 +466,8 @@
                     dst = dst.chunk(parts, 0)[block] if parts > 1 else dst
                     dst.copy_(entry[name].reshape(dst.shape))
                 self.step[le] = int(entry["step"])
+            if self.split:
+                self.sync_bf16()
 
 
 class LayerWorkspace:
@@ -629,19 +662,19 @@
             self._expert_gated_fwd(wait, epoch)
         elif c.small:
             go, gr_, T = ws.group_off, ws.group_rows, c.tile_rows
-            K.swapab_linear(ws.xd, sh.bf16["w1"], go, gr_, out=ws.h1, bias=sh.views["b1"], wait=wait)
-            K.ln_relu_fwd(ws.h1, sh.views["g1"], sh.views["be1"], tg, out=ws.a1, mean=ws.mean1, rstd=ws.rstd1, tile_rows=T)
-            K.swapab_linear(ws.a1, sh.bf16["w2"], go, gr_, out=ws.h2, bias=sh.views["b2"])
-            K.ln_relu_fwd(ws.h2, sh.views["g2"], sh.views["be2"], tg, out=ws.a2, mean=ws.mean2, rstd=ws.rstd2, tile_rows=T)
-            K.swapab_linear(ws.a2, sh.bf16["w3"], go, gr_, out=ws.yo, bias=sh.views["b3"], residual=ws.xd)
+            K.swapab_linear(ws.xd, sh.bf16["w1"], go, gr_, out=ws.h1, bias=sh.raw_views["b1"], wait=wait)
+            K.ln_relu_fwd(ws.h1, sh.raw_views["g1"], sh.raw_views["be1"], tg, out=ws.a1, mean=ws.mean1, rstd=ws.rstd1, tile_rows=T)
+            K.swapab_linear(ws.a1, sh.bf16["w2"], go, gr_, out=ws.h2, bias=sh.raw_views["b2"])
+            K.ln_relu_fwd(ws.h2, sh.raw_views["g2"], sh.raw_views["be2"], tg, out=ws.a2, mean=ws.mean2, rstd=ws.rstd2, tile_rows=T)
+            K.swapab_linear(ws.a2, sh.bf16["w3"], go, gr_, out=ws.yo, bias=sh.raw_views["b3"], residual=ws.xd)
         elif cfg.expert_dtype == "fp8":
             self._expert_ffn_fp8(wait, epoch)
         else:
-            gemm.grouped_linear(ws.xd, sh.bf16["w1"], tile_group=tg, bias=sh.views["b1"], out=ws.h1, wait=wait)
-            K.ln_relu_fwd(ws.h1, sh.views["g1"], sh.views["be1"], tg, out=ws.a1, mean=ws.mean1, rstd=ws.rstd1)
-            gemm.grouped_linear(ws.a1, sh.bf16["w2"], tile_group=tg, bias=sh.views["b2"], out=ws.h2)
-            K.ln_relu_fwd(ws.h2, sh.views["g2"], sh.views["be2"], tg, out=ws.a2, mean=ws.mean2, rstd=ws.rstd2)
-            gemm.grouped_linear(ws.a2, sh.bf16["w3"], tile_group=tg, bias=sh.views["b3"], residual=ws.xd, out=ws.yo)
+            gemm.grouped_linear(ws.xd, sh.bf16["w1"], tile_group=tg, bias=sh.raw_views["b1"], out=ws.h1, wait=wait)
+            K.ln_relu_fwd(ws.h1, sh.raw_views["g1"], sh.raw_views["be1"], tg, out=ws.a1, mean=ws.mean1, rstd=ws.rstd1)
+            gemm.grouped_linear(ws.a1, sh.bf16["w2"], tile_group=tg, bias=sh.raw_views["b2"], out=ws.h2)
+            K.ln_relu_fwd(ws.h2, sh.raw_views["g2"], sh.raw_views["be2"], tg, out=ws.a2, mean=ws.mean2, rstd=ws.rstd2)
+            gemm.grouped_linear(ws.a2, sh.bf16["w3"], tile_group=tg, bias=sh.raw_views["b3"], residual=ws.xd, out=ws.yo)
         c.timer.mark("expert_ffn_fwd")
         y = torch.empty(B, cfg.hidden, dtype=torch.bfloat16, device=x.device)
         K.combine_rows(ws.yo_off, idx, pair_row, w, y, k, c.E_loc, flags_off=c.flags_off, slot=K.SLOT_OUTPUT, epoch=epoch,
@@ -654,7 +687,7 @@
         tg, T = ws.tile_group, c.tile_rows
         if wait is not None:
             K.signal_wait(c.flags_off, K.SLOT_DISPATCH, epoch, c.status, signal=False, wait=True)
-        K.rms_norm_fwd(ws.xd, sh.views["g"], GATED_EPS, out=ws.n, rstd=ws.rstd, tile_group=tg, tile_rows=T)
+        K.rms_norm_fwd(ws.xd, sh.raw_views["g"], GATED_EPS, out=ws.n, rstd=ws.rstd, tile_group=tg, tile_rows=T)
         if c.small:
             go, gr_ = ws.group_off, ws.group_rows
             K.swapab_linear(ws.n, sh.bf16["w13"], go, gr_, out=ws.h)
@@ -673,11 +706,11 @@
             K.signal_wait(c.flags_off, K.SLOT_DISPATCH, epoch, c.status, signal=False, wait=True)
         w8 = sh.fp8_weights()
         fp8.quantize(ws.xd, tile_group=tg, out=ws.xq)
-        fp8.grouped_linear_fp8(ws.xq, w8["w1"], tile_group=tg, bias=sh.views["b1"], out=ws.h1)
-        K.ln_relu_fwd(ws.h1, sh.views["g1"], sh.views["be1"], tg, out=ws.a1, mean=ws.mean1, rstd=ws.rstd1, quant=ws.aq)
-        fp8.grouped_linear_fp8(ws.aq, w8["w2"], tile_group=tg, bias=sh.views["b2"], out=ws.h2)
-        K.ln_relu_fwd(ws.h2, sh.views["g2"], sh.views["be2"], tg, out=ws.a2, mean=ws.mean2, rstd=ws.rstd2, quant=ws.aq)
-        fp8.grouped_linear_fp8(ws.aq, w8["w3"], tile_group=tg, bias=sh.views["b3"], residual=ws.xd, out=ws.yo)
+        fp8.grouped_linear_fp8(ws.xq, w8["w1"], tile_group=tg, bias=sh.raw_views["b1"], out=ws.h1)
+        K.ln_relu_fwd(ws.h1, sh.raw_views["g1"], sh.raw_views["be1"], tg, out=ws.a1, mean=ws.mean1, rstd=ws.rstd1, quant=ws.aq)
+        fp8.grouped_linear_fp8(ws.aq, w8["w2"], tile_group=tg, bias=sh.raw_views["b2"], out=ws.h2)
+        K.ln_relu_fwd(ws.h2, sh.raw_views["g2"], sh.raw_views["be2"], tg, out=ws.a2, mean=ws.mean2, rstd=ws.rstd2, quant=ws.aq)
+        fp8.grouped_linear_fp8(ws.aq, w8["w3"], tile_group=tg, bias=sh.raw_views["b3"], residual=ws.xd, out=ws.yo)
 
     def _backward_cuda(self, gy, B, logits=None):
         c, ws, sh, cfg = self.ctx, self.ws, self.shard, self.cfg
@@ -716,17 +749,17 @@
             K.swiglu_bwd(c.da, ws.h, out=c.dh)
             gemm.grouped_wgrad(c.dh, ws.n, go, G, out=gr["w13"], accumulate=cfg.accumulate)
             gemm.grouped_linear(c.dh, sh.bf16["w13"], tile_group=tg, w_is_kn=True, out=c.dn)
-            K.rms_norm_bwd(c.dn, ws.xd, ws.rstd, sh.views["g"], dx=c.dxd, dgamma=gr["g"], dres=c.gyd,
+            K.rms_norm_bwd(c.dn, ws.xd, ws.rstd, sh.raw_views["g"], dx=c.dxd, dgamma=gr["g"], dres=c.gyd,
                            tile_rows=c.tile_rows, tile_group=tg)
         else:
             K.grouped_colsum(c.gyd, tg, out=gr["b3"])
             gemm.grouped_wgrad(c.gyd, ws.a2, go, G, out=gr["w3"], accumulate=cfg.accumulate)
             gemm.grouped_linear(c.gyd, sh.bf16["w3"], tile_group=tg, w_is_kn=True, out=c.da)
-            K.ln_relu_bwd(c.da, ws.h2, ws.mean2, ws.rstd2, sh.views["g2"], sh.views["be2"], tg, dh=c.dh, dgamma=gr["g2"],
+            K.ln_relu_bwd(c.da, ws.h2, ws.mean2, ws.rstd2, sh.raw_views["g2"], sh.raw_views["be2"], tg, dh=c.dh, dgamma=gr["g2"],
                           dbeta=gr["be2"], dbias=gr["b2"])
             gemm.grouped_wgrad(c.dh, ws.a1, go, G, out=gr["w2"], accumulate=cfg.accumulate)
             gemm.grouped_linear(c.dh, sh.bf16["w2"], tile_group=tg, w_is_kn=True, out=c.da)
-            K.ln_relu_bwd(c.da, ws.h1, ws.mean1, ws.rstd1, sh.views["g1"], sh.views["be1"], tg, dh=c.dh, dgamma=gr["g1"],
+            K.ln_relu_bwd(c.da, ws.h1, ws.mean1, ws.rstd1, sh.raw_views["g1"], sh.raw_views["be1"], tg, dh=c.dh, dgamma=gr["g1"],
                           dbeta=gr["be1"], dbias=gr["b1"])
             gemm.grouped_wgrad(c.dh, ws.xd, go, G, out=gr["w1"], accumulate=cfg.accumulate)
             gemm.grouped_linear(c.dh, sh.bf16["w1"], tile_group=tg, w_is_kn=True, residual=c.gyd, out=c.dxd)
@@ -750,8 +783,11 @@
         side, chain_ctas = c.opt_stream, c.chain_ctas
 
         def wgrad(name, dy, x):
-            kw = dict(p=sh.views[name][:self.E_loc], m=sh.m_views[name][:self.E_loc], v=sh.v_views[name][:self.E_loc],
-                      vmax=sh.vmax_views[name][:self.E_loc] if cfg.amsgrad else None, p_bf16=sh.bf16[name], step=sh.step, **opt)
+            E = self.E_loc
+            kw = dict(p=None, p_lo=sh.lo_views[name][:E], p_bf16=sh.bf16[name][:E]) if sh.split else \
+                dict(p=sh.raw_views[name][:E], p_bf16=sh.bf16[name])
+            kw.update(m=sh.m_views[name][:E], v=sh.v_raw_views[name][:E],
+                      vmax=sh.vmax_views[name][:E] if cfg.amsgrad else None, step=sh.step, **opt)
             if side is None:
                 K.wgrad_adam(dy, x, go, rows, **kw)
                 return
@@ -769,23 +805,23 @@
             K.swiglu_bwd(c.da, ws.h, out=dh13)
             K.swapab_linear(dh13, sh.bf16["w13"], go, rows, out=c.dn, w_is_kn=True, max_ctas=chain_ctas)
             wgrad("w13", dh13, ws.n)
-            K.rms_norm_bwd(c.dn, ws.xd, ws.rstd, sh.views["g"], dx=c.dxd, dgamma=gr["g"], dres=gyd, tile_rows=T,
+            K.rms_norm_bwd(c.dn, ws.xd, ws.rstd, sh.raw_views["g"], dx=c.dxd, dgamma=gr["g"], dres=gyd, tile_rows=T,
                            tile_group=tg)
         else:
             dh2, dh1 = ws.dh2, ws.dh1
             K.grouped_colsum(gyd, tg, out=gr["b3"], tile_rows=T)
             K.swapab_linear(gyd, sh.bf16["w3"], go, rows, out=c.da, w_is_kn=True, max_ctas=chain_ctas)
             wgrad("w3", gyd, ws.a2)
-            K.ln_relu_bwd(c.da, ws.h2, ws.mean2, ws.rstd2, sh.views["g2"], sh.views["be2"], tg, dh=dh2, dgamma=gr["g2"],
+            K.ln_relu_bwd(c.da, ws.h2, ws.mean2, ws.rstd2, sh.raw_views["g2"], sh.raw_views["be2"], tg, dh=dh2, dgamma=gr["g2"],
                           dbeta=gr["be2"], dbias=gr["b2"], tile_rows=T)
             K.swapab_linear(dh2, sh.bf16["w2"], go, rows, out=c.da, w_is_kn=True, max_ctas=chain_ctas)
             wgrad("w2", dh2, ws.a1)
-            K.ln_relu_bwd(c.da, ws.h1, ws.mean1, ws.rstd1, sh.views["g1"], sh.views["be1"], tg, dh=dh1, dgamma=gr["g1"],
+            K.ln_relu_bwd(c.da, ws.h1, ws.mean1, ws.rstd1, sh.raw_views["g1"], sh.raw_views["be1"], tg, dh=dh1, dgamma=gr["g1"],
                           dbeta=gr["be1"], dbias=gr["b1"], tile_rows=T)
             K.swapab_linear(dh1, sh.bf16["w1"], go, rows, out=c.dxd, w_is_kn=True, residual=gyd, max_ctas=chain_ctas)
             wgrad("w1", dh1, ws.xd)
         small = sh.layout.small_mask
-        K.adam_step(sh.p, sh.g, sh.m, sh.v, sh.vmax, sh.p_bf16, sh.seg_sizes, sh.slots, step=sh.step,
+        K.adam_step(sh.p_raw, sh.g, sh.m, sh.v_raw, sh.vmax, sh.p_bf16, sh.seg_sizes, sh.slots, step=sh.step,
                     group_rows=ws.step_rows, zero_mask=small, G_active=self.E_loc, seg_mask=small, **opt)
         sh.w8_dirty = True
 
@@ -802,7 +838,7 @@
             sh.pending_steps.mul_(1 - sh.fire)
             rows, zero_mask = sh.fire, (1 << len(sh.layout.names)) - 1
         K.bump_steps(sh.step, rows)
-        K.adam_step(sh.p, sh.g, sh.m, sh.v, sh.vmax, sh.p_bf16, sh.seg_sizes, sh.slots, step=sh.step,
+        K.adam_step(sh.p_raw, sh.g, sh.m, sh.v_raw, sh.vmax, sh.p_bf16, sh.seg_sizes, sh.slots, step=sh.step,
                     group_rows=rows, **c.adam_kwargs(), zero_mask=zero_mask, G_active=self.E_loc, world=c.world,
                     peer_bases=c.heap.peer_bases if c.S else None, shadow_of=ws.owned_shadow if c.S else None,
                     shadow_g_off=sh.g_off, me=c.rank)
@@ -846,7 +882,7 @@
                 sh.pending_steps.mul_(keep)
                 rows, zero_mask = due.to(rows.dtype), (1 << len(sh.layout.names)) - 1
             sh.step += (rows > 0).to(sh.step.dtype)
-            K.adam_step_ref(sh.p, sh.g, sh.m, sh.v, sh.vmax, sh.seg_sizes, self.E_loc, step=sh.step,
+            K.adam_step_ref(sh.p_raw, sh.g, sh.m, sh.v_raw, sh.vmax, sh.seg_sizes, self.E_loc, step=sh.step,
                             group_rows=rows, **cfg.adam_kwargs(), zero_mask=zero_mask)
         sh.sync_bf16()
         self._ref_rows = None
```

Measured after the change: 13580 (median of 6 runs). +5.4%, better.
